# EAST-J/Dynhor

Hardware: AMD Instinct MI355X
Metric: training rays/sec (higher is better)
Workload: dtype f32; 1 GPU; custom_shoes-shaped synthetic seq, 512x512, 2048 rays x (64+64) samples per rank, NeuS SDF(8x256, skip 4, softplus100) + colour(4x256) MLP, full training iteration; family=neus, frames=64, rays_per_rank=2048, samples_per_ray=128, parallelism=dp1, loss=rgb L1 + 0.1 eikonal + 0.1 mask BCE + 0.05 mono-normal

## Files before the change

dynhor_amd/_lib.py:

```python
import ctypes
import os

import torch

_HERE = os.path.dirname(os.path.abspath(__file__))
LIB_PATH = os.path.join(_HERE, "libdynhor_hip.so")
_LIB = None

_vp, _i64, _i32, _f32 = ctypes.c_void_p, ctypes.c_int64, ctypes.c_int, ctypes.c_float

SIGNATURES = {
    "dh_version": (_i32, []),
    "dh_strerror": (ctypes.c_char_p, [_i32]),
    "dh_set_arithmetic": (_i32, [_i32]),
    "dh_get_arithmetic": (_i32, []),
    "dh_hash_set_scatter_mode": (_i32, [_i32]),
    "dh_num_params": (_i64, []),
    "dh_packed_floats": (_i64, []),
    "dh_param_layout": (_i32, [_i32, _i32, ctypes.POINTER(_i64), ctypes.POINTER(_i64), ctypes.POINTER(_i64),
                               ctypes.POINTER(_i32), ctypes.POINTER(_i32)]),
    "dh_packed_section": (_i32, [_i32, ctypes.POINTER(_i64), ctypes.POINTER(_i64)]),
    "dh_pack_weights": (_i32, [_vp, _vp, _vp]),
    "dh_pack_weights_ex": (_i32, [_i32, _vp, _vp, _vp]),
    "dh_sdf_nograd": (_i32, [_vp, _vp, _i64, _vp, _vp]),
    "dh_workspace_floats": (_i32, [_i64, ctypes.POINTER(_i64), ctypes.POINTER(_i64), ctypes.POINTER(_i64)]),
    "dh_range_words": (_i32, [ctypes.POINTER(_i64), ctypes.POINTER(_i64), ctypes.POINTER(_f32)]),
    "dh_mlp_forward": (_i32, [_vp, _vp, _vp, _i32, _i64, _vp, _vp, _vp, _vp, _vp]),
    "dh_sdf_forward": (_i32, [_vp, _vp, _i64, _vp, _vp, _vp]),
    "dh_sdf_gradient": (_i32, [_vp, _vp, _i64, _vp, _vp, _i32, _vp]),
    "dh_color_forward": (_i32, [_vp, _vp, _vp, _i32, _vp, _i64, _vp, _vp, _i32, _vp]),
    "dh_color_backward": (_i32, [_vp, _vp, _vp, _i64, _vp, _vp, _vp]),
    "dh_sdf_tangent": (_i32, [_vp, _vp, _vp, _i64, _vp, _vp]),
    "dh_sdf_backward": (_i32, [_vp, _vp, _i64, _vp, _vp]),
    "dh_color_backward_rays": (_i32, [_vp, _vp, _vp, _vp, _i32, _i64, _vp, _vp, _vp, _vp, _vp]),
    "dh_sdf_backward_rays": (_i32, [_vp, _vp, _vp, _vp, _i64, _vp, _vp, _vp]),
    "dh_weight_grads_gemm": (_i32, [_i64, _vp, _vp]),
    "dh_weight_grads_fold": (_i32, [_vp, _vp, _i64, _vp, _vp, _vp]),
    "dh_mlp_backward": (_i32, [_vp, _vp, _vp, _i64] + [_vp] * 7),
    "dh_sdf_nograd_ex": (_i32, [_i32, _vp, _vp, _i64, _vp, _vp]),
    "dh_mlp_forward_ex": (_i32, [_i32, _vp, _vp, _vp, _i32, _i64, _vp, _vp, _vp, _vp, _vp]),
    "dh_sdf_forward_ex": (_i32, [_i32, _vp, _vp, _i64, _vp, _vp, _vp]),
    "dh_sdf_gradient_ex": (_i32, [_i32, _vp, _vp, _i64, _vp, _vp, _i32, _vp]),
    "dh_color_forward_ex": (_i32, [_i32, _vp, _vp, _vp, _i32, _vp, _i64, _vp, _vp, _i32, _vp]),
    "dh_color_backward_ex": (_i32, [_i32, _vp, _vp, _vp, _i64, _vp, _vp, _vp]),
    "dh_sdf_tangent_ex": (_i32, [_i32, _vp, _vp, _vp, _i64, _vp, _vp]),
    "dh_sdf_backward_ex": (_i32, [_i32, _vp, _vp, _i64, _vp, _vp]),
    "dh_color_backward_rays_ex": (_i32, [_i32, _vp, _vp, _vp, _vp, _i32, _i64, _vp, _vp, _vp, _vp, _vp]),
    "dh_sdf_backward_rays_ex": (_i32, [_i32, _vp, _vp, _vp, _vp, _i64, _vp, _vp, _vp]),
    "dh_weight_grads_gemm_ex": (_i32, [_i32, _i64, _vp, _vp]),
    "dh_mlp_backward_ex": (_i32, [_i32, _vp, _vp, _vp, _i64] + [_vp] * 7),
    "dh_adam_step": (_i32, [_vp, _vp, _vp, _vp, _i64, _f32, _f32, _f32, _f32, _i64, _f32, _vp]),
    "dh_hashgrid_entries": (_i64, []),
    "dh_hashgrid_level": (_i32, [_i32, ctypes.POINTER(_f32), ctypes.POINTER(ctypes.c_uint32), ctypes.POINTER(ctypes.c_uint32),
                                 ctypes.POINTER(ctypes.c_uint32)]),
    "dh_hashgrid_encode": (_i32, [_vp, _vp, _i64, _vp, _vp]),
    "dh_hashgrid_encode_backward": (_i32, [_vp, _vp, _i64, _vp, _vp]),
    "dh_hash_num_params": (_i64, []),
    "dh_hash_packed_floats": (_i64, []),
    "dh_hash_param_layout": (_i32, [_i32, _i32, ctypes.POINTER(_i64), ctypes.POINTER(_i64), ctypes.POINTER(_i64),
                                    ctypes.POINTER(_i32), ctypes.POINTER(_i32)]),
    "dh_hash_pack_weights": (_i32, [_vp, _vp, _vp]),
    "dh_hash_workspace_floats": (_i32, [_i64, ctypes.POINTER(_i64), ctypes.POINTER(_i64)]),
    "dh_hash_sdf_nograd": (_i32, [_vp, _vp, _vp, _i64, _f32, _vp, _vp]),
    "dh_hash_geo_forward": (_i32, [_vp, _vp, _vp, _i64, _f32, _f32, _vp, _i32, _vp, _vp, _vp, _vp, _vp]),
    "dh_hash_color_forward": (_i32, [_vp, _vp, _vp, _vp, _i32, _i64, _vp, _vp, _vp]),
    "dh_hash_color_backward": (_i32, [_vp, _vp, _vp, _vp, _vp, _i32, _i64, _vp, _vp, _vp, _vp, _vp]),
    "dh_hash_geo_backward": (_i32, [_vp, _vp, _vp, _vp, _vp, _vp, _i64, _f32, _f32, _vp, _vp, _vp]),
    "dh_hash_weight_grads": (_i32, [_vp, _vp, _i64, _vp, _vp, _vp, _vp]),
    "dh_hash_weight_grads_parts": (_i32, [_vp, _vp, _i64, _vp, _vp, _vp, _i32, _vp]),
    "dh_gen_rays": (_i32, [_vp] * 6 + [_i32, _i32, _i32, _i32, _vp, _vp, _i64, _vp, _vp, _vp, _vp]),
    "dh_coarse_samples": (_i32, [_vp] * 5 + [_i64, _i32, _vp, _vp, _vp]),
    "dh_upsample_step": (_i32, [_vp] * 4 + [_i64, _i32, _i32, _f32, _vp, _vp, _vp]),
    "dh_merge_samples": (_i32, [_vp] * 4 + [_i64, _i32, _i32, _vp, _vp, _vp]),
    "dh_midpoints": (_i32, [_vp] * 3 + [_i64, _i32, _f32, _vp, _vp]),
    "dh_render_scan_fwd": (_i32, [_vp] * 7 + [_f32, _f32, _vp, _i64, _i32] + [_vp] * 9),
    "dh_render_scan_bwd": (_i32, [_vp] * 7 + [_f32, _f32, _vp, _i64, _i32] + [_vp] * 11),
    "dh_render_scan_bwd_rays": (_i32, [_vp] * 7 + [_f32, _f32, _vp, _i64, _i32] + [_vp] * 12),
    "dh_march_count": (_i32, [_vp] * 6 + [_i32, _f32, _f32, _f32, _i32, _i64, _vp, _vp]),
# ... 85 lines not shown


def roctx():
    global _ROCTX
    if _ROCTX is False:
        _ROCTX = None
        for name in ("librocprofiler-sdk-roctx.so", "libroctx64.so"):
            try:
                L = ctypes.CDLL(name)
                L.roctxRangePushA.argtypes = [ctypes.c_char_p]
                L.roctxRangePushA.restype = ctypes.c_int
                L.roctxRangePop.restype = ctypes.c_int
                _ROCTX = L
                break
            except (OSError, AttributeError):
                continue
    return _ROCTX


def check(status: int):
    if status != 0:
        raise DynhorHipError(f"dynhor_hip status {status}: {lib().dh_strerror(status).decode()}")


def ptr(t: torch.Tensor):
    assert t.is_cuda and t.is_contiguous(), "device-resident contiguous tensor required"
    return ctypes.c_void_p(t.data_ptr())


def stream():
    return ctypes.c_void_p(torch.cuda.current_stream().cuda_stream)


def param_layout(net: int, layer: int):
    b, g, v = _i64(), _i64(), _i64()
    o, i = _i32(), _i32()
    check(lib().dh_param_layout(net, layer, ctypes.byref(b), ctypes.byref(g), ctypes.byref(v),
                                ctypes.byref(o), ctypes.byref(i)))
    return b.value, g.value, v.value, o.value, i.value


def packed_section(section: int):
    o, n = _i64(), _i64()
    check(lib().dh_packed_section(int(section), ctypes.byref(o), ctypes.byref(n)))
    return o.value, n.value


def range_words():
    a, t, lim = _i64(), _i64(), _f32()
    check(lib().dh_range_words(ctypes.byref(a), ctypes.byref(t), ctypes.byref(lim)))
    return a.value, t.value, lim.value


def workspace_floats(npts: int):
    i, f, t = _i64(), _i64(), _i64()
    check(lib().dh_workspace_floats(npts, ctypes.byref(i), ctypes.byref(f), ctypes.byref(t)))
    return i.value, f.value, t.value
```

dynhor_amd/csrc/api.hip:

```cpp
#include "../../include/dynhor_hip.h"
#include "kernels.h"
#include "hash_layout.h"
#include "layout.h"
#include "workspace.h"

using namespace dh;

namespace dh {
static int g_arith = DH_ARITH_SPLIT_F16;
static int g_hash_scatter = 0;
int hash_scatter_mode() { return __atomic_load_n(&g_hash_scatter, __ATOMIC_RELAXED); }
}

namespace {
inline bool misaligned16(const void* p) { return (reinterpret_cast<uintptr_t>(p) & 15u) != 0; }
inline bool bad_arith(int a) { return a != DH_ARITH_SPLIT_BF16 && a != DH_ARITH_FP32_MFMA && a != DH_ARITH_SPLIT_F16; }
inline bool bad_arith_form(int a) {
    const int form = a & ~0xff;
    return bad_arith(a & 0xff) || (form != 0 && form != DH_CHAIN_FORM_TILE && form != DH_CHAIN_FORM_PAIR) ||
           (form != 0 && (a & 0xff) != DH_ARITH_SPLIT_F16);
}
inline int cur_arith() { return __atomic_load_n(&dh::g_arith, __ATOMIC_RELAXED); }
#ifndef DH_GRID_DIV
#define DH_GRID_DIV 1
// ... 37 lines not shown
        case 0: *offset_floats = PACKT.stream; *n_floats = PACKT_STREAM_FLOATS; break;
        case 1: *offset_floats = PACKT.bias10; *n_floats = 10 * 256; break;
        case 2: *offset_floats = PACKH.stream; *n_floats = PACKTH_STREAM_FLOATS; break;
        case 3: *offset_floats = PACKH.bias11; *n_floats = 11 * 256; break;
        case 4: *offset_floats = PACKH.wabs; *n_floats = 16; break;
        default: return DH_ERR_BAD_ARG;
    }
    return DH_OK;
}

int dh_param_layout(int net, int layer, int64_t* bias_off, int64_t* g_off, int64_t* v_off, int* out_dim, int* in_dim) {
    if (!bias_off || !g_off || !v_off || !out_dim || !in_dim) return DH_ERR_BAD_ARG;
    if (net == 0) {
        if (layer < 0 || layer >= N_SDF) return DH_ERR_BAD_ARG;
        const LinOff o = sdf_off(layer);
        *bias_off = o.bias; *g_off = o.g; *v_off = o.v; *out_dim = SDF_DIMS[layer].out; *in_dim = SDF_DIMS[layer].in;
    } else if (net == 1) {
        *bias_off = *g_off = *v_off = VARIANCE_OFF; *out_dim = 1; *in_dim = 1;
    } else if (net == 2) {
        if (layer < 0 || layer >= N_COL) return DH_ERR_BAD_ARG;
        const LinOff o = col_off(layer);
        *bias_off = o.bias; *g_off = o.g; *v_off = o.v; *out_dim = COL_DIMS[layer].out; *in_dim = COL_DIMS[layer].in;
    } else {
        return DH_ERR_BAD_ARG;
    }
    return DH_OK;
}

int dh_pack_weights(const float* params, float* packed, void* stream) {
    if (!params || !packed || misaligned16(packed)) return DH_ERR_BAD_ARG;
    return launch_pack_weights(params, packed, 7, static_cast<hipStream_t>(stream));
}
int dh_pack_weights_ex(int arithmetic, const float* params, float* packed, void* stream) {
    if (!params || !packed || misaligned16(packed) || bad_arith(arithmetic)) return DH_ERR_BAD_ARG;
    return launch_pack_weights(params, packed, 1 << arithmetic, static_cast<hipStream_t>(stream));
}

int dh_sdf_nograd_ex(int arithmetic, const float* packed, const float* pts, int64_t npts, float* sdf, void* stream) {
    if (npts < 0 || bad_arith(arithmetic)) return DH_ERR_BAD_ARG;
    if (npts == 0) return DH_OK;
    if (!packed || !pts || !sdf || misaligned16(packed)) return DH_ERR_BAD_ARG;
    return launch_sdf_nograd(packed, pts, npts, sdf, DEFAULT_GRID, arithmetic, static_cast<hipStream_t>(stream));
}

int dh_workspace_floats(int64_t npts, int64_t* infer_floats, int64_t* fwd_floats, int64_t* total_floats) {
    if (npts < 0 || !infer_floats || !fwd_floats || !total_floats) return DH_ERR_BAD_ARG;
    const Workspace w = carve_workspace(nullptr, npts);
    *infer_floats = w.infer_floats;
    *fwd_floats = w.fwd_floats;
    *total_floats = w.total_floats;
    return DH_OK;
}

int dh_range_words(int64_t* act_max_off, int64_t* tag_off, float* limit) {
    if (!act_max_off || !tag_off || !limit) return DH_ERR_BAD_ARG;
    *act_max_off = (int64_t)ABSMAX_ACT * ABSMAX_STRIDE;
    *tag_off = (int64_t)ABSMAX_TAG * ABSMAX_STRIDE;
    *limit = H2_RANGE / H2_XS;
    return DH_OK;
}

int dh_sdf_forward_ex(int arithmetic, const float* packed, const float* pts, int64_t npts, float* ws, float* sdf, void* stream) {
    if (bad_arith(arithmetic)) return DH_ERR_BAD_ARG;
    if (npts <= 0) return npts == 0 ? DH_OK : DH_ERR_BAD_ARG;
    if (!packed || !pts || !ws || !sdf || misaligned16(packed) || misaligned16(ws)) return DH_ERR_BAD_ARG;
    const Workspace w = carve_workspace(ws, npts);
    return launch_sdf_fwd_train(packed, pts, npts, sdf, w.feat, w.act, w.eaux, w.absmax, DEFAULT_GRID, arithmetic, static_cast<hipStream_t>(stream));
}

int dh_sdf_gradient_ex(int arithmetic, const float* packed, const float* pts, int64_t npts, float* ws, float* normals, int save,
                       void* stream) {
    if (bad_arith_form(arithmetic)) return DH_ERR_BAD_ARG;
    if (npts <= 0) return npts == 0 ? DH_OK : DH_ERR_BAD_ARG;
    if (!packed || !pts || !ws || !normals || misaligned16(packed) || misaligned16(ws)) return DH_ERR_BAD_ARG;
    const Workspace w = carve_workspace(ws, npts);
    if (save < 0 || save > 2) return DH_ERR_BAD_ARG;
    return launch_sdf_grad(packed, pts, npts, w.act, w.asave, normals, save, w.gesave, w.absmax, DEFAULT_GRID, arithmetic,
                           static_cast<hipStream_t>(stream));
}

int dh_color_forward_ex(int arithmetic, const float* packed, const float* pts, const float* dirs, int n_per_ray, const float* normals,
                        int64_t npts, float* ws, float* color, int save, void* stream) {
    if (npts < 0 || n_per_ray <= 0 || bad_arith_form(arithmetic)) return DH_ERR_BAD_ARG;
    if (npts == 0) return DH_OK;
    if (!packed || !pts || !dirs || !normals || !ws || !color || misaligned16(packed) || misaligned16(ws)) return DH_ERR_BAD_ARG;
    const Workspace w = carve_workspace(ws, npts);
    return launch_color_fwd(packed, pts, dirs, n_per_ray, normals, w.feat, npts, color, w.cact, w.caux, save, w.absmax, DEFAULT_GRID,
                            arithmetic, static_cast<hipStream_t>(stream));
}

int dh_mlp_forward_ex(int arithmetic, const float* packed, const float* pts, const float* dirs, int n_per_ray, int64_t npts, float* ws,
                      float* sdf, float* normals, float* color, void* stream) {
    int rc = dh_sdf_forward_ex(arithmetic, packed, pts, npts, ws, sdf, stream);
    if (rc) return rc;
    rc = dh_sdf_gradient_ex(arithmetic, packed, pts, npts, ws, normals, 1, stream);
    if (rc) return rc;
    return dh_color_forward_ex(arithmetic, packed, pts, dirs, n_per_ray, normals, npts, ws, color, 1, stream);
}

int dh_color_backward_ex(int arithmetic, const float* packed, const float* colors, const float* d_colors, int64_t npts, float* ws,
                         float* d_normals, void* stream) {
    if (npts <= 0 || bad_arith_form(arithmetic)) return DH_ERR_BAD_ARG;
    if (!packed || !colors || !d_colors || !ws || !d_normals || misaligned16(packed) || misaligned16(ws)) return DH_ERR_BAD_ARG;
    const Workspace w = carve_workspace(ws, npts);
    return launch_color_bwd(packed, colors, d_colors, npts, w.cact, w.czbar, w.featbar, d_normals, w.tpart, w.absmax, DEFAULT_GRID,
                            arithmetic, static_cast<hipStream_t>(stream));
}

int dh_sdf_tangent_ex(int arithmetic, const float* packed, const float* pts, const float* d_normals, int64_t npts, float* ws,
                      void* stream) {
    if (npts <= 0 || bad_arith(arithmetic)) return DH_ERR_BAD_ARG;
    if (!packed || !pts || !d_normals || !ws || misaligned16(packed) || misaligned16(ws)) return DH_ERR_BAD_ARG;
    const Workspace w = carve_workspace(ws, npts);
    return launch_sdf_tangent(packed, pts, d_normals, npts, w.act, w.asave, w.t0aux, w.tsave, w.rsave, w.tpart, w.absmax, DEFAULT_GRID,
                              arithmetic, static_cast<hipStream_t>(stream));
}

int dh_sdf_backward_ex(int arithmetic, const float* packed, const float* d_sdf, int64_t npts, float* ws, void* stream) {
    if (npts <= 0 || bad_arith(arithmetic)) return DH_ERR_BAD_ARG;
    if (!packed || !d_sdf || !ws || misaligned16(packed) || misaligned16(ws)) return DH_ERR_BAD_ARG;
    const Workspace w = carve_workspace(ws, npts);
    return launch_sdf_bwd(packed, d_sdf, npts, w.act, w.rsave, w.featbar, w.zbar, w.tpart, w.absmax, DEFAULT_GRID, arithmetic,
                          static_cast<hipStream_t>(stream));
}

int dh_color_backward_rays_ex(int arithmetic, const float* packed, const float* colors, const float* d_colors, const float* dirs,
                              int n_per_ray, int64_t npts, float* ws, float* d_normals, float* d_pts, float* d_dirs_pts, void* stream) {
    if (npts <= 0 || n_per_ray <= 0 || bad_arith(arithmetic)) return DH_ERR_BAD_ARG;
    if (!packed || !colors || !d_colors || !dirs || !ws || !d_normals || !d_pts || !d_dirs_pts || misaligned16(packed) || misaligned16(ws))
        return DH_ERR_BAD_ARG;
    const Workspace w = carve_workspace(ws, npts);
    return launch_color_bwd_rays(packed, colors, d_colors, dirs, n_per_ray, npts, w.cact, w.czbar, w.featbar, d_normals, w.tpart,
                                 d_pts, d_dirs_pts, w.absmax, DEFAULT_GRID, arithmetic, static_cast<hipStream_t>(stream));
}

int dh_sdf_backward_rays_ex(int arithmetic, const float* packed, const float* d_sdf, const float* pts, const float* d_normals,
                            int64_t npts, float* ws, float* d_pts, void* stream) {
    if (npts <= 0 || bad_arith(arithmetic)) return DH_ERR_BAD_ARG;
    if (!packed || !d_sdf || !pts || !d_normals || !ws || !d_pts || misaligned16(packed) || misaligned16(ws)) return DH_ERR_BAD_ARG;
    const Workspace w = carve_workspace(ws, npts);
    return launch_sdf_bwd_rays(packed, d_sdf, pts, d_normals, npts, w.act, w.rsave, w.featbar, w.gesave, w.zbar, w.tpart, d_pts,
                               w.absmax, DEFAULT_GRID, arithmetic, static_cast<hipStream_t>(stream));
}

int dh_weight_grads_gemm_ex(int arithmetic, int64_t npts, float* ws, void* stream) {
    if (npts <= 0 || bad_arith(arithmetic)) return DH_ERR_BAD_ARG;
    if (!ws || misaligned16(ws)) return DH_ERR_BAD_ARG;
    const Workspace w = carve_workspace(ws, npts);
    return launch_weight_grads_gemm(w, w.slabs, DW_G, arithmetic, static_cast<hipStream_t>(stream));
}

int dh_weight_grads_fold(const float* packed, const float* params, int64_t npts, float* ws, float* grad_flat, void* stream) {
    if (npts <= 0) return DH_ERR_BAD_ARG;
    if (!packed || !params || !ws || !grad_flat || misaligned16(packed) || misaligned16(ws)) return DH_ERR_BAD_ARG;
    const Workspace w = carve_workspace(ws, npts);
    return launch_weight_grads_fold(w, w.slabs, w.tred, DW_G, DW_NS, params, packed, grad_flat, static_cast<hipStream_t>(stream));
}

int dh_mlp_backward_ex(int arithmetic, const float* packed, const float* params, const float* pts, int64_t npts, float* ws,
                       const float* colors, const float* d_sdf, float* d_normals, const float* d_colors, float* grad_flat,
                       void* stream) {
    int rc = dh_color_backward_ex(arithmetic, packed, colors, d_colors, npts, ws, d_normals, stream);
    if (rc) return rc;
    rc = dh_sdf_tangent_ex(arithmetic, packed, pts, d_normals, npts, ws, stream);
    if (rc) return rc;
    rc = dh_sdf_backward_ex(arithmetic, packed, d_sdf, npts, ws, stream);
    if (rc) return rc;
    rc = dh_weight_grads_gemm_ex(arithmetic, npts, ws, stream);
    if (rc) return rc;
    return dh_weight_grads_fold(packed, params, npts, ws, grad_flat, stream);
}

int dh_sdf_nograd(const float* packed, const float* pts, int64_t npts, float* sdf, void* stream) {
    return dh_sdf_nograd_ex(cur_arith(), packed, pts, npts, sdf, stream);
}
int dh_sdf_forward(const float* packed, const float* pts, int64_t npts, float* ws, float* sdf, void* stream) {
    return dh_sdf_forward_ex(cur_arith(), packed, pts, npts, ws, sdf, stream);
}
int dh_sdf_gradient(const float* packed, const float* pts, int64_t npts, float* ws, float* normals, int save, void* stream) {
    return dh_sdf_gradient_ex(cur_arith(), packed, pts, npts, ws, normals, save, stream);
}
int dh_color_forward(const float* packed, const float* pts, const float* dirs, int n_per_ray, const float* normals,
                     int64_t npts, float* ws, float* color, int save, void* stream) {
    return dh_color_forward_ex(cur_arith(), packed, pts, dirs, n_per_ray, normals, npts, ws, color, save, stream);
}
// ... 529 lines not shown
```

dynhor_amd/csrc/chain_pair.hip:

```cpp
#include "tile.h"
#include "kernels.h"
#include "mlp_common.h"
#include "tile16h.h"
#include "pair16h.h"
#include "workspace.h"

namespace dh {

struct HScratchP { float sred[4]; float sred2[4]; float lmax[12]; };
struct ColHPtrs;
struct ColPPtrs {
    const u32x4* main0;
    const u32x4* aux;
    const float* bias0;
    const float* w4;
    const float* b4;
    const unsigned* wabs;
};
constexpr int64_t COL_MAIN_STRIDE = (PACKH.col_fwd_main[1] - PACKH.col_fwd_main[0]) / 4;
constexpr int64_t COL_BIAS_STRIDE = PACK.col_bias[1] - PACK.col_bias[0];
static_assert(PACKH.col_fwd_main[2] - PACKH.col_fwd_main[1] == PACKH.col_fwd_main[1] - PACKH.col_fwd_main[0] &&
              PACKH.col_fwd_main[3] - PACKH.col_fwd_main[2] == PACKH.col_fwd_main[1] - PACKH.col_fwd_main[0] &&
              (PACKH.col_fwd_main[1] - PACKH.col_fwd_main[0]) % 4 == 0, "colour forward weights: one stride");
static_assert(PACK.col_bias[2] - PACK.col_bias[1] == COL_BIAS_STRIDE && PACK.col_bias[3] - PACK.col_bias[2] == COL_BIAS_STRIDE, "colour biases: one stride");
static inline ColPPtrs make_colp_ptrs(const float* packed) {
    ColPPtrs C;
    C.main0 = reinterpret_cast<const u32x4*>(packed + PACKH.col_fwd_main[0]);
    C.aux = reinterpret_cast<const u32x4*>(packed + PACKH.col_fwd_aux0);
    C.bias0 = packed + PACK.col_bias[0];
    C.w4 = packed + PACK.col_w4;
    C.b4 = packed + PACK.col_b4;
    C.wabs = reinterpret_cast<const unsigned*>(packed + PACKH.wabs) + N_SDF;
    return C;
}

template <bool SAVE>
struct ColFwdEpi : PEpi<ColFwdEpi<SAVE>, 3, 4> {
    f32x16 (&acc)[MT][2];
    HScratchP& hs;
    float* lmax;
    const int wave, lane, tid;
    const float inv, b0, b1;
    const rsrc_t st;
    const int loff;
    __device__ __forceinline__ ColFwdEpi(f32x16 (&acc_)[MT][2], _Float16* img_, HScratchP& hs_, float* lmax_, int wave_, int lane_, int tid_,
                                         float inv_, float b0_, float b1_, rsrc_t st_, int loff_, bool)
        : acc(acc_), hs(hs_), lmax(lmax_), wave(wave_), lane(lane_), tid(tid_), inv(inv_), b0(b0_), b1(b1_), st(st_), loff(loff_) {
        this->handoff_init(img_, wave_, lane_);
    }
    template <int G, int SUB>
    __device__ __forceinline__ void elem() {
        constexpr int m = G / 8, t = (G / 4) % 2, r4 = G % 4;
        const float b = t ? b1 : b0;
        if constexpr (SUB == 0 || SUB == 1) {
            constexpr int r = 4 * r4 + 2 * SUB;
            acc[m][t][r] = fmaxf(fmaf(acc[m][t][r], inv, b), 0.f);
            acc[m][t][r + 1] = fmaxf(fmaf(acc[m][t][r + 1], inv, b), 0.f);
        } else {
            if constexpr (SAVE) {
                f32x4 v;
                v[0] = acc[m][t][4 * r4 + 0]; v[1] = acc[m][t][4 * r4 + 1]; v[2] = acc[m][t][4 * r4 + 2]; v[3] = acc[m][t][4 * r4 + 3];
                tile_st(st, loff, G, v);
            }
            this->m0 = fmaxf(this->m0, fmaxf(fabsf(acc[m][t][4 * r4 + 0]), fabsf(acc[m][t][4 * r4 + 1])));
            this->m1 = fmaxf(this->m1, fmaxf(fabsf(acc[m][t][4 * r4 + 2]), fabsf(acc[m][t][4 * r4 + 3])));
        }
    }
    __device__ __forceinline__ void publish(float wm) { tile_max_publish(hs.sred, wave, lane, wm); }
    __device__ __forceinline__ float read_tile_max() { return tile_max_read(hs.sred); }
    __device__ __forceinline__ void on_tile_max(float m) { if (tid == 0 && lmax) *lmax = fmaxf(*lmax, m); }
};

__device__ __forceinline__ void row_dot256x3_hp(const _Float16* img, const float* sw4, int tid, float (&out)[3]) {
    constexpr int TPP_ = 256 / TM, SEG = 256 / TPP_;
    const int p = tid / TPP_, part = tid % TPP_;
    const f16x8* xh = reinterpret_cast<const f16x8*>(img + p * LDH + part * SEG);
    const f16x8* xl = reinterpret_cast<const f16x8*>(img + PLANE_H + p * LDH + part * SEG);
    float s[3] = {0.f, 0.f, 0.f};
    DH_UNROLL for (int i = 0; i < SEG / 8; ++i) {
        const f16x8 h = xh[i], l = xl[i];
        float x[8];
        DH_UNROLL for (int k = 0; k < 8; ++k) x[k] = (float)h[k] + (float)l[k];
        DH_UNROLL for (int j = 0; j < 3; ++j) {
            const f32x4* wr = reinterpret_cast<const f32x4*>(sw4 + j * 256 + part * SEG);
            const f32x4 b0 = wr[2 * i], b1 = wr[2 * i + 1];
            DH_UNROLL for (int k = 0; k < 4; ++k) s[j] = fmaf(x[k], b0[k], s[j]);
            DH_UNROLL for (int k = 0; k < 4; ++k) s[j] = fmaf(x[4 + k], b1[k], s[j]);
        }
    }
    DH_UNROLL for (int j = 0; j < 3; ++j) {
        DH_UNROLL for (int off = 1; off < TPP_; off <<= 1) s[j] += __shfl_xor(s[j], off);
        out[j] = s[j];
    }
}

__device__ __forceinline__ TileScale pair_handoff_exposed(const f32x16 (&acc)[MT][2], _Float16* img, HScratchP& hs, float* lmax, int tid,
                                                          int wave, int lane, const float* extra_lds) {
    tile_max_publish(hs.sred, wave, lane, acc_absmax(acc));
    __syncthreads();
    const float m = tile_max_read(hs.sred);
    if (tid == 0 && lmax) *lmax = fmaxf(*lmax, m);
    const TileScale ts = scale_for_max(fmaxf(m, *extra_lds));
    acc_to_lds_split(acc, img, wave, lane, ts.S);
    __syncthreads();
    return ts;
}

template <bool SAVE>
__global__ __launch_bounds__(256, 1) void color_fwd_p_kernel(ColPPtrs C, const float* __restrict__ pts, const float* __restrict__ dirs,
                                                            int n_per_ray, const float* __restrict__ normals,
                                                            const float* __restrict__ feat, int64_t npts, float* __restrict__ color,
                                                            float* __restrict__ cact, float* __restrict__ caux,
                                                            unsigned* __restrict__ absmax) {
    __shared__ __attribute__((aligned(16))) _Float16 simg[2][IMG_H];
    __shared__ __attribute__((aligned(16))) float saux[2][TM * LDA];
    __shared__ HScratchP hs;
    __shared__ float sfb[64];
    const int tid = threadIdx.x, wave = tid >> 6, lane = tid & 63;
    const int loff = tile_loff(wave, lane);
    const int64_t ntiles = (npts + TM - 1) / TM, npairs = (ntiles + 1) / 2;
    if (tid < 12) hs.lmax[tid] = 0.f;
    float winv0 = winv_from_bits(C.wabs[0]), winv1 = winv_from_bits(C.wabs[1]), winv2 = winv_from_bits(C.wabs[2]), winv3 = winv_from_bits(C.wabs[3]);
    float bs[4][2];
    DH_UNROLL for (int l = 0; l < 4; ++l)
        DH_UNROLL for (int t = 0; t < 2; ++t) bs[l][t] = C.bias0[l * COL_BIAS_STRIDE + acc_col(wave, t, lane)];
    PW<P_NKC> W;
    _Float16* imgA = simg[0];
    _Float16* imgB = simg[1];
    int pit = 0;
    for (int64_t pr = blockIdx.x; pr < npairs; pr += gridDim.x, ++pit) {
        const bool son = pit == 2;
        (void)son;
        PSTAMP(son, 0);
        const int64_t tileA = 2 * pr;
        const bool okB = tileA + 1 < ntiles;
        const int64_t tileB = okB ? tileA + 1 : tileA;
        f32x16 accA[MT][2], accB[MT][2];
        acc_load_native_b(accA, tile_rsrc(feat + tileA * TILE_F), loff);
        acc_load_native_b(accB, tile_rsrc(feat + tileB * TILE_F), loff);
        {
            const int which = tid >> 7, half = (tid >> 6) & 1, p = tid & 63;
            const int64_t t0 = (which ? tileB : tileA) * TM;
            const int64_t gp = t0 + p;
            auto single_ray = [&](int64_t first) {
                const int64_t last = first + TM - 1 < npts ? first + TM - 1 : npts - 1;
                return first / n_per_ray == last / n_per_ray;
            };
            const bool oneA = single_ray(tileA * TM), oneB = single_ray(tileB * TM);
            const bool one_ray = which ? oneB : oneA;
            float* row = saux[which] + p * LDA;
            float* emb = sfb + which * 32;
            if (one_ray && half == 0 && lane < 12) {
                const int c = lane % 3, k = lane / 3;
                float sn, co; sincosf(dirs[(t0 / n_per_ray) * 3 + c] * (float)(1 << k), &sn, &co);
                emb[6 * k + c] = sn;
                emb[6 * k + 3 + c] = co;
            }
            float mx = 1.f;
            if (gp < npts) {
                const int64_t ray = gp / n_per_ray;
                DH_UNROLL for (int c = 0; c < 3; ++c) {
                    const float d = dirs[ray * 3 + c];
                    if (!one_ray) {
                        DH_UNROLL for (int kk = 0; kk < 2; ++kk) {
                            const int k = 2 * half + kk;
                            float sn, co; sincosf(d * (float)(1 << k), &sn, &co);
// ... 2 lines not shown
                        }
                    }
                    if (half == 0) {
                        const float x = pts[gp * 3 + c], nn = normals[gp * 3 + c];
                        row[c] = x;
                        row[3 + c] = d;
                        row[30 + c] = nn;
                        mx = fmaxf(mx, fmaxf(fabsf(x), fmaxf(fabsf(d), fabsf(nn))));
                    }
                }
            } else {
                DH_UNROLL for (int c = 0; c < 3; ++c) {
                    DH_UNROLL for (int kk = 0; kk < 2; ++kk) { row[6 + 6 * (2 * half + kk) + c] = 0.f; row[6 + 6 * (2 * half + kk) + 3 + c] = 0.f; }
                    if (half == 0) { row[c] = 0.f; row[3 + c] = 0.f; row[30 + c] = 0.f; }
                }
            }
            if (half == 0) {
                DH_UNROLL for (int c = CAUX; c < LDA; ++c) row[c] = 0.f;
                mx = wave_max(mx);
                if (lane == 0) hs.sred2[which] = mx;
            }
            if (oneA || oneB) {
                pair_barrier();
                if (one_ray && gp < npts) { DH_UNROLL for (int j = 0; j < 12; ++j) row[6 + 12 * half + j] = emb[12 * half + j]; }
            }
        }
        PSTAMP(son, 88);
        TileScale tsA = pair_handoff_exposed(accA, imgA, hs, SAVE ? &hs.lmax[4] : nullptr, tid, wave, lane, &hs.sred2[0]);
        PSTAMP(son, 89);
        TileScale tsB = pair_handoff_exposed(accB, imgB, hs, SAVE ? &hs.lmax[4] : nullptr, tid, wave, lane, &hs.sred2[1]);
        PSTAMP(son, 90);
        if (SAVE && tid == 0) hs.lmax[5] = fmaxf(hs.lmax[5], fmaxf(hs.sred2[0], hs.sred2[1]));
        if (SAVE) {
            aux_lds_to_native(saux[0], caux + tileA * AUXT_F, wave, lane);
            if (okB) aux_lds_to_native(saux[1], caux + tileB * AUXT_F, wave, lane);
        }
        PSTAMP(son, 91);
        pw_load_all(W, C.main0, wave, lane);
        PSTAMP(son, 1);
        _Pragma("unroll 1") for (int l = 0; l < 4; ++l) {
            const float wl = l == 0 ? winv0 : l == 1 ? winv1 : l == 2 ? winv2 : winv3;
            const float wp = l == 1 ? winv0 : l == 2 ? winv1 : winv2;
            const float c0 = l == 0 ? bs[0][0] : l == 1 ? bs[1][0] : l == 2 ? bs[2][0] : bs[3][0];
            const float c1 = l == 0 ? bs[0][1] : l == 1 ? bs[1][1] : l == 2 ? bs[2][1] : bs[3][1];
            const float p0 = l == 1 ? bs[0][0] : l == 2 ? bs[1][0] : bs[2][0];
            const float p1 = l == 1 ? bs[0][1] : l == 2 ? bs[1][1] : bs[2][1];
            acc_zero(accA);
            if (l == 0) {
                PNoEpi e;
                pair_phase<false>(accA, imgA, W, C.main0, C.main0, wave, lane, e);
                gemm_rows_aux_h(accA, saux[0], C.aux, wave, lane, tsA.S);
            } else {
                ColFwdEpi<SAVE> e(accB, imgB, hs, SAVE ? &hs.lmax[l - 1] : nullptr, wave, lane, tid, tsB.inv * wp, p0, p1,
                                  tile_rsrc_if(cact + ((int64_t)(l - 1) * ntiles + tileB) * TILE_F, okB), loff, okB);
                if (son && l == 2) e.stamp = 18;
                pair_phase<false>(accA, imgA, W, C.main0 + (int64_t)l * COL_MAIN_STRIDE, C.main0, wave, lane, e);
                tsB.S = e.S; tsB.inv = e.inv_S;
            }
            PSTAMP(son, 2 + 4 * l);
            pair_barrier();
            PSTAMP(son, 3 + 4 * l);
            acc_zero(accB);
            {
                ColFwdEpi<SAVE> e(accA, imgA, hs, SAVE ? &hs.lmax[l] : nullptr, wave, lane, tid, tsA.inv * wl, c0, c1,
                                  tile_rsrc(cact + ((int64_t)l * ntiles + tileA) * TILE_F), loff, true);
                if (son && l == 2) e.stamp = 52;
                pair_phase<true>(accB, imgB, W, C.main0 + (int64_t)l * COL_MAIN_STRIDE, C.main0 + (int64_t)(l < 3 ? l + 1 : 3) * COL_MAIN_STRIDE, wave, lane, e, l < 3);
                if (l == 0) gemm_rows_aux_h(accB, saux[1], C.aux, wave, lane, tsB.S);
                tsA.S = e.S; tsA.inv = e.inv_S;
            }
            PSTAMP(son, 4 + 4 * l);
            pair_barrier();
            PSTAMP(son, 5 + 4 * l);
        }
        const float w4a = C.w4[tid], w4b = C.w4[256 + tid], w4c = C.w4[512 + tid];
        {
            ColFwdEpi<SAVE> e(accB, imgB, hs, SAVE ? &hs.lmax[3] : nullptr, wave, lane, tid, tsB.inv * winv3, bs[3][0], bs[3][1],
                              tile_rsrc_if(cact + ((int64_t)3 * ntiles + tileB) * TILE_F, okB), loff, okB);
            pair_epi_alone_from<0>(e);
            tsB.S = e.S; tsB.inv = e.inv_S;
        }
        float* sw4 = saux[0];
        sw4[tid] = w4a; sw4[256 + tid] = w4b; sw4[512 + tid] = w4c;
        pair_barrier();
        PSTAMP(son, 86);
        DH_UNROLL for (int which = 0; which < 2; ++which) {
            const int64_t gp = (which ? tileB : tileA) * TM + tid / TPP;
            const float sinv = which ? tsB.inv : tsA.inv;
            float dots[3];
            row_dot256x3_hp(which ? imgB : imgA, sw4, tid, dots);
            DH_UNROLL for (int j = 0; j < 3; ++j) {
                const float raw = fmaf(dots[j], sinv, C.b4[j]);
                if (tid % TPP == 0 && gp < npts && (which == 0 || okB)) color[gp * 3 + j] = 1.f / (1.f + __expf(-raw));
            }
        }
        pair_barrier();
        PSTAMP(son, 87);
    }
    if (SAVE && absmax) {
        if (tid < 4) post_class_max(absmax, ABSMAX_CACT + tid, hs.lmax[tid]);
        if (tid == 4) post_class_max(absmax, ABSMAX_FEAT, hs.lmax[4]);
        if (tid == 5) post_class_max(absmax, ABSMAX_CAUX, hs.lmax[5]);
    }
}

struct SdfGradPPtrs {
    const u32x4 *rev1, *rev2, *rev3, *rev4, *rev5, *rev6, *rev7;
    const u32x4 *revaux0, *revaux4;
    const float* w8row0;
    const unsigned* wabs;
};
static inline SdfGradPPtrs make_sdfgradp_ptrs(const float* packed) {
    SdfGradPPtrs P;
    auto rv = [&](int l) { return reinterpret_cast<const u32x4*>(packed + PACKH.sdf_rev_main[l]); };
    P.rev1 = rv(1); P.rev2 = rv(2); P.rev3 = rv(3); P.rev4 = rv(4); P.rev5 = rv(5); P.rev6 = rv(6); P.rev7 = rv(7);
    P.revaux0 = reinterpret_cast<const u32x4*>(packed + PACKH.sdf_rev_aux[0]);
    P.revaux4 = reinterpret_cast<const u32x4*>(packed + PACKH.sdf_rev_aux[4]);
    P.w8row0 = packed + PACK.sdf_w8row0;
    P.wabs = reinterpret_cast<const unsigned*>(packed + PACKH.wabs);
    return P;
}
template <bool SAVE>
struct SdfGradEpi : PEpi<SdfGradEpi<SAVE>, 5, 3> {
    static constexpr int RING = 5;
    f32x16 (&acc)[MT][2];
    HScratchP& hs;
    float* lmax;
    const int wave, lane, tid;
    const float inv;
    const rsrc_t hr, st;
    const int loff;
// ... 151 lines not shown
                        float* q = &saux[which][aux_row(wave, r, lane) * LDA + col];
                        *q = fmaf(g0[tt][r], inv, *q);
                    }
                }
            }
        }
        __syncthreads();
        if (tid < 2 * TM) {
            const int which = tid >> 6, p = tid & 63;
            const int64_t gp = (which ? tileB : tileA) * TM + p;
            if (gp < npts && (which == 0 || okB)) {
                const float* g = saux[which] + p * LDA;
                float n[3];
                DH_UNROLL for (int c = 0; c < 3; ++c) {
                    const float x = pts[gp * 3 + c];
                    float v = g[c];
                    DH_UNROLL for (int k = 0; k < 6; ++k) {
                        const float f = (float)(1 << k);
                        float sn, co; sincosf(x * f, &sn, &co);
                        v += f * (co * g[3 + 6 * k + c] - sn * g[3 + 6 * k + 3 + c]);
                    }
                    n[c] = v;
                }
                normals[gp * 3 + 0] = n[0]; normals[gp * 3 + 1] = n[1]; normals[gp * 3 + 2] = n[2];
                if (save == 2) { for (int c = 0; c < 40; ++c) gesave[gp * 40 + c] = c < EMB ? g[c] : 0.f; }
            }
        }
        __syncthreads();
        PSTAMP(son, 31);
    }
    if (SAVE && absmax && tid < 8) post_class_max(absmax, ABSMAX_ASAVE + tid, hs.lmax[tid]);
    if (absmax) {
        const float m = wave_max(watch_close(hmax));
        if (lane == 0) post_class_max(absmax, ABSMAX_ACT, m);
    }
}

enum : int { PTP_COL_B0 = 12, PTP_COL_W4 = 16, PTP_COL_B4 = 19 };
struct ColBwdPPtrs {
    const u32x4 *rev0, *rev1, *rev2, *rev3;
    const u32x4* revaux;
    const float* w4;
    const unsigned* wabs;
};
static inline ColBwdPPtrs make_colbwdp_ptrs(const float* packed) {
    ColBwdPPtrs C;
    auto rv = [&](int l) { return reinterpret_cast<const u32x4*>(packed + PACKH.col_rev_main[l]); };
    C.rev0 = rv(0); C.rev1 = rv(1); C.rev2 = rv(2); C.rev3 = rv(3);
    C.revaux = reinterpret_cast<const u32x4*>(packed + PACKH.col_rev_aux0);
    C.w4 = packed + PACK.col_w4;
    C.wabs = reinterpret_cast<const unsigned*>(packed + PACKH.wabs) + N_SDF;
    return C;
}
template <bool LAST>
struct ColBwdEpi : PEpi<ColBwdEpi<LAST>, 4, 3, !LAST> {
    static constexpr int RING = 5;
    f32x16 (&acc)[MT][2];
    HScratchP& hs;
    float* lmax;
    unsigned* tslot;
    float* csum;
    const int wave, lane, tid;
    const float inv;
    const rsrc_t hr, st;
    const int loff;
    const bool store;
    float cs0 = 0.f, cs1 = 0.f;
    f32x4 hq[RING];
    __device__ __forceinline__ ColBwdEpi(f32x16 (&acc_)[MT][2], _Float16* img_, HScratchP& hs_, float* lmax_, unsigned* tslot_, float* csum_,
                                         int wave_, int lane_, int tid_, float inv_, rsrc_t hr_, rsrc_t st_, int loff_, bool store_)
        : acc(acc_), hs(hs_), lmax(lmax_), tslot(tslot_), csum(csum_), wave(wave_), lane(lane_), tid(tid_), inv(inv_), hr(hr_),
          st(st_), loff(loff_), store(store_) {
        if constexpr (!LAST) {
            this->handoff_init(img_, wave_, lane_);
            DH_UNROLL for (int g = 0; g < RING; ++g) hq[g] = tile_ld(hr, loff, g);
        }
    }
    template <int G, int SUB>
    __device__ __forceinline__ void elem() {
        constexpr int m = G / 8, t = (G / 4) % 2, r4 = G % 4;
        if constexpr (SUB == 0 || SUB == 1) {
            constexpr int i = 2 * SUB, r = 4 * r4 + i;
            if constexpr (LAST) {
                acc[m][t][r] *= inv;
                acc[m][t][r + 1] *= inv;
            } else {
                const f32x4& h = hq[G % RING];
                acc[m][t][r] = h[i] > 0.f ? acc[m][t][r] * inv : 0.f;
                acc[m][t][r + 1] = h[i + 1] > 0.f ? acc[m][t][r + 1] * inv : 0.f;
            }
        } else if constexpr (SUB == 2) {
            f32x4 v;
            v[0] = acc[m][t][4 * r4 + 0]; v[1] = acc[m][t][4 * r4 + 1]; v[2] = acc[m][t][4 * r4 + 2]; v[3] = acc[m][t][4 * r4 + 3];
            tile_st(st, loff, G, v);
            if constexpr (!LAST && G + RING < 16) hq[G % RING] = tile_ld(hr, loff, G + RING);
            if constexpr (!LAST) {
                float& cs = t ? cs1 : cs0;
                cs += acc[m][t][4 * r4 + 0]; cs += acc[m][t][4 * r4 + 1]; cs += acc[m][t][4 * r4 + 2]; cs += acc[m][t][4 * r4 + 3];
            }
        } else {
            this->m0 = fmaxf(this->m0, fmaxf(fabsf(acc[m][t][4 * r4 + 0]), fabsf(acc[m][t][4 * r4 + 1])));
            this->m1 = fmaxf(this->m1, fmaxf(fabsf(acc[m][t][4 * r4 + 2]), fabsf(acc[m][t][4 * r4 + 3])));
        }
    }
    __device__ __forceinline__ void publish(float wm) {
        if constexpr (LAST) {
            tile_max_publish(hs.sred2, wave, lane, wm);
        } else {
            cs0 += __shfl_xor(cs0, 32); cs1 += __shfl_xor(cs1, 32);
            if (lane < 32 && store) { csum[64 * wave + lane] = cs0; csum[64 * wave + 32 + lane] = cs1; }
            tile_max_publish(hs.sred, wave, lane, wm);
        }
    }
    __device__ __forceinline__ float read_tile_max() { return tile_max_read(hs.sred); }
    __device__ __forceinline__ void on_tile_max(float m) {
        if (tid == 0) {
            *lmax = fmaxf(*lmax, m);
            if (store) *tslot = __builtin_bit_cast(unsigned, m);
        }
    }
};

#ifndef COLBWD_NREG
#define COLBWD_NREG 8
#endif
__global__ __launch_bounds__(256, 1) void color_bwd_p_kernel(ColBwdPPtrs C, const float* __restrict__ colors, const float* __restrict__ d_colors,
                                                            int64_t npts, const float* __restrict__ cact, float* __restrict__ czbar,
                                                            float* __restrict__ featbar, float* __restrict__ d_normals,
                                                            float* __restrict__ tpart, unsigned* __restrict__ absmax,
                                                            unsigned* __restrict__ tmax) {
    __shared__ __attribute__((aligned(16))) _Float16 simg[2][IMG_H];
    __shared__ __attribute__((aligned(16))) float scraw[2][TM * 4];
    __shared__ HScratchP hs;
    __shared__ float sfb[2][4];
    const int tid = threadIdx.x, wave = tid >> 6, lane = tid & 63;
    const int loff = tile_loff(wave, lane);
    const int64_t ntiles = (npts + TM - 1) / TM, npairs = (ntiles + 1) / 2;
    if (tid < 12) hs.lmax[tid] = 0.f;
    const float wi0 = winv_from_bits(C.wabs[0]), wi1 = winv_from_bits(C.wabs[1]), wi2 = winv_from_bits(C.wabs[2]), wi3 = winv_from_bits(C.wabs[3]);
    auto winv = [&](int l) { return l == 0 ? wi0 : l == 1 ? wi1 : l == 2 ? wi2 : wi3; };
    auto rev = [&](int l) { return l == 0 ? C.rev0 : l == 1 ? C.rev1 : l == 2 ? C.rev2 : C.rev3; };
    PW<COLBWD_NREG> W;
    _Float16* imgA = simg[0];
    _Float16* imgB = simg[1];
    for (int64_t pr = blockIdx.x; pr < npairs; pr += gridDim.x) {
        const int64_t tileA = 2 * pr;
        const bool okB = tileA + 1 < ntiles;
        const int64_t tileB = okB ? tileA + 1 : tileA;
        float* tpA = tpart + tileA * N_TILE_PART * 256;
        float* tpB = tpart + tileB * N_TILE_PART * 256;
        if (tid < 2 * TM) {
            const int which = tid >> 6, p = tid & 63;
            const int64_t gp = (which ? tileB : tileA) * TM + p;
            DH_UNROLL for (int j = 0; j < 3; ++j) {
                float v = 0.f;
                if (gp < npts) { const float c = colors[gp * 3 + j]; v = d_colors[gp * 3 + j] * c * (1.f - c); }
                scraw[which][p * 4 + j] = v;
            }
            scraw[which][p * 4 + 3] = 0.f;
        }
        __syncthreads();
        if (tid < 3 || (tid >= 64 && tid < 67)) {
            const int which = tid >> 6, j = tid & 63;
            float sum = 0.f;
            for (int r = 0; r < TM; ++r) sum += scraw[which][r * 4 + j];
            if (which == 0 || okB) (which ? tpB : tpA)[PTP_COL_B4 * 256 + j] = sum;
        }
        f32x16 accA[MT][2], accB[MT][2];
        TileScale tsA, tsB;
        DH_UNROLL for (int which = 0; which < 2; ++which) {
            f32x16 (&acc)[MT][2] = which ? accB : accA;
            const int64_t tile = which ? tileB : tileA;
            float* tp = which ? tpB : tpA;
            const bool on = which == 0 || okB;
            acc_load_native_b(acc, tile_rsrc(cact + ((int64_t)3 * ntiles + tile) * TILE_F), loff);
            {
                const int col0 = acc_col(wave, 0, lane), col1 = acc_col(wave, 1, lane);
                float w4[3][2];
                DH_UNROLL for (int j = 0; j < 3; ++j) { w4[j][0] = C.w4[j * 256 + col0]; w4[j][1] = C.w4[j * 256 + col1]; }
                float dw[3][2] = {{0.f, 0.f}, {0.f, 0.f}, {0.f, 0.f}};
                DH_UNROLL for (int m = 0; m < MT; ++m)
                    DH_UNROLL for (int r = 0; r < 16; ++r) {
                        const f32x4 cr = *reinterpret_cast<const f32x4*>(scraw[which] + acc_row(m, r, lane) * 4);
                        DH_UNROLL for (int t = 0; t < 2; ++t) {
                            const float h = acc[m][t][r];
                            DH_UNROLL for (int j = 0; j < 3; ++j) dw[j][t] = fmaf(cr[j], h, dw[j][t]);
                            const float hb = cr[0] * w4[0][t] + cr[1] * w4[1][t] + cr[2] * w4[2][t];
                            acc[m][t][r] = h > 0.f ? hb : 0.f;
                        }
                    }
                DH_UNROLL for (int j = 0; j < 3; ++j)
                    DH_UNROLL for (int t = 0; t < 2; ++t) {
                        float sum = dw[j][t];
                        sum += __shfl_xor(sum, 32);
                        if (lane < 32 && on) tp[(PTP_COL_W4 + j) * 256 + 64 * wave + 32 * t + lane] = sum;
                    }
            }
            if (on) {
                acc_store_native_b(acc, tile_rsrc(czbar + ((int64_t)3 * ntiles + tile) * TILE_F), loff);
                tile_colsum(acc, tp + (PTP_COL_B0 + 3) * 256, wave, lane);
            }
            tile_max_publish(hs.sred, wave, lane, acc_absmax(acc));
            __syncthreads();
            const float mx = tile_max_read(hs.sred);
            if (tid == 0) {
                hs.lmax[3] = fmaxf(hs.lmax[3], mx);
                if (on) tmax[(TMAX_CZBAR + 3) * ntiles + tile] = __builtin_bit_cast(unsigned, mx);
            }
            const TileScale ts = scale_for_max(mx);
            acc_to_lds_split(acc, which ? imgB : imgA, wave, lane, ts.S);
            __syncthreads();
            if (which) tsB = ts; else tsA = ts;
        }
        pw_load_all(W, C.rev3, wave, lane);
        _Pragma("unroll 1") for (int l = 3; l >= 1; --l) {
            acc_zero(accA);
            if (l == 3) {
                PNoEpi e;
                pair_phase<false>(accA, imgA, W, C.rev3, C.rev3, wave, lane, e);
            } else {
                ColBwdEpi<false> e(accB, imgB, hs, &hs.lmax[l], tmax + (TMAX_CZBAR + l) * ntiles + tileB, tpB + (PTP_COL_B0 + l) * 256, wave, lane, tid,
                                   tsB.inv * winv(l + 1), tile_rsrc(cact + ((int64_t)l * ntiles + tileB) * TILE_F),
                                   tile_rsrc_if(czbar + ((int64_t)l * ntiles + tileB) * TILE_F, okB), loff, okB);
                pair_phase<false>(accA, imgA, W, rev(l), C.rev3, wave, lane, e);
                tsB.S = e.S; tsB.inv = e.inv_S;
            }
            pair_barrier();
            acc_zero(accB);
            {
                ColBwdEpi<false> e(accA, imgA, hs, &hs.lmax[l - 1], tmax + (TMAX_CZBAR + l - 1) * ntiles + tileA, tpA + (PTP_COL_B0 + l - 1) * 256, wave,
                                   lane, tid, tsA.inv * winv(l), tile_rsrc(cact + ((int64_t)(l - 1) * ntiles + tileA) * TILE_F),
                                   tile_rsrc(czbar + ((int64_t)(l - 1) * ntiles + tileA) * TILE_F), loff, true);
                pair_phase<true>(accB, imgB, W, rev(l), rev(l - 1), wave, lane, e);
                tsA.S = e.S; tsA.inv = e.inv_S;
            }
            pair_barrier();
        }
        acc_zero(accA);
        {
            ColBwdEpi<false> e(accB, imgB, hs, &hs.lmax[0], tmax + TMAX_CZBAR * ntiles + tileB, tpB + PTP_COL_B0 * 256, wave, lane, tid,
                               tsB.inv * wi1, tile_rsrc(cact + tileB * TILE_F), tile_rsrc_if(czbar + tileB * TILE_F, okB), loff, okB);
            pair_phase<false>(accA, imgA, W, C.rev0, C.rev0, wave, lane, e);
            tsB.S = e.S; tsB.inv = e.inv_S;
        }
        pair_barrier();
        acc_zero(accB);
        {
            ColBwdEpi<true> e(accA, imgA, hs, nullptr, nullptr, nullptr, wave, lane, tid, tsA.inv * wi0, tile_rsrc(featbar + tileA * TILE_F),
                              tile_rsrc(featbar + tileA * TILE_F), loff, true);
            pair_phase<false>(accB, imgB, W, C.rev0, C.rev0, wave, lane, e);
            if (lane == 0) sfb[0][wave] = hs.sred2[wave];
        }
        pair_barrier();
        {
            ColBwdEpi<true> e(accB, imgB, hs, nullptr, nullptr, nullptr, wave, lane, tid, tsB.inv * wi0, tile_rsrc(featbar + tileB * TILE_F),
                              tile_rsrc_if(featbar + tileB * TILE_F, okB), loff, okB);
            pair_epi_alone_from<0>(e);
            if (lane == 0) sfb[1][wave] = hs.sred2[wave];
        }
        DH_UNROLL for (int which = 0; which < 2; ++which) {
            f32x16 a2[AUX_NTW];
            aux_zero(a2);
            gemm_auxout_hp(a2, which ? imgB : imgA, 16, C.revaux, wave, lane);
            const float inv0 = (which ? tsB.inv : tsA.inv) * wi0;
            DH_UNROLL for (int tt = 0; tt < AUX_NTW; ++tt) {
                const int col = aux_col(wave, tt, lane);
                if (col >= 30 && col < 33 && (which == 0 || okB)) {
                    DH_UNROLL for (int r = 0; r < 16; ++r) {
                        const int64_t gp = (which ? tileB : tileA) * TM + aux_row(wave, r, lane);
                        if (gp < npts) d_normals[gp * 3 + (col - 30)] += a2[tt][r] * inv0;
                    }
                }
            }
        }
        __syncthreads();
        if (tid < 2) {
            const float m = fmaxf(fmaxf(sfb[tid][0], sfb[tid][1]), fmaxf(sfb[tid][2], sfb[tid][3]));
            if (tid == 0 || okB) {
                atomicMax(reinterpret_cast<unsigned*>(&hs.lmax[4]), __builtin_bit_cast(unsigned, m));
                tmax[TMAX_FEATBAR * ntiles + (tid ? tileB : tileA)] = __builtin_bit_cast(unsigned, m);
            }
        }
        __syncthreads();
    }
    if (absmax) {
        if (tid < 4) post_class_max(absmax, ABSMAX_CZBAR + tid, hs.lmax[tid]);
        if (tid == 4) post_class_max(absmax, ABSMAX_FEATBAR, hs.lmax[4]);
    }
}

}
#ifdef DH_STAMPS
extern "C" int dh_dev_read_stamps_p(unsigned long long* host, long long n) {
    const long long total = (long long)(sizeof(dh::dh_pstamps) / sizeof(unsigned long long));
    if (n > total) n = total;
    return hipMemcpyFromSymbol(host, HIP_SYMBOL(dh::dh_pstamps), (size_t)n * sizeof(unsigned long long)) == hipSuccess ? 0 : -3;
}
#endif
namespace dh {
static inline int okp() { return hipGetLastError() == hipSuccess ? 0 : -3; }
static int pair_cus() {
    static int cache[16] = {};
    int dev = 0;
    if (hipGetDevice(&dev) != hipSuccess || dev < 0 || dev >= 16) return 0;
    if (cache[dev] == 0) {
        int cus = 0, lds = 0;
        if (hipDeviceGetAttribute(&cus, hipDeviceAttributeMultiprocessorCount, dev) != hipSuccess) cus = 0;
        if (hipDeviceGetAttribute(&lds, hipDeviceAttributeMaxSharedMemoryPerMultiprocessor, dev) != hipSuccess) lds = 0;
        cache[dev] = (lds >= PAIR_LDS_BYTES && cus > 0) ? cus : -1;
    }
    return cache[dev] > 0 ? cache[dev] : 0;
}
bool pair_form_available() { return pair_cus() > 0; }
int pair_form_cus() { return pair_cus(); }
int launch_color_fwd_p(const float* packed, const float* pts, const float* dirs, int n_per_ray, const float* normals,
                       const float* feat, int64_t npts, float* color, float* cact, float* caux, int save, unsigned* absmax,
                       hipStream_t stream) {
    const int cus = pair_cus();
    if (cus <= 0) return -2;
    const int64_t ntiles = (npts + TM - 1) / TM, npairs = (ntiles + 1) / 2;
    const int g = (int)(npairs < cus ? npairs : cus);
    if (save) hipLaunchKernelGGL(color_fwd_p_kernel<true>, dim3(g), dim3(256), 0, stream, make_colp_ptrs(packed), pts, dirs, n_per_ray, normals,
                                 feat, npts, color, cact, caux, absmax);
    else hipLaunchKernelGGL(color_fwd_p_kernel<false>, dim3(g), dim3(256), 0, stream, make_colp_ptrs(packed), pts, dirs, n_per_ray, normals,
                            feat, npts, color, cact, caux, absmax);
    return okp();
}

}

namespace dh {
int launch_sdf_grad_p(const float* packed, const float* pts, int64_t npts, const float* act, float* asave, float* normals, int save,
                      float* gesave, unsigned* absmax, hipStream_t stream) {
    const int cus = pair_cus();
    if (cus <= 0) return -2;
    const int64_t ntiles = (npts + TM - 1) / TM, npairs = (ntiles + 1) / 2;
    const int g = (int)(npairs < cus ? npairs : cus);
    if (save) hipLaunchKernelGGL(sdf_grad_p_kernel<true>, dim3(g), dim3(256), 0, stream, make_sdfgradp_ptrs(packed), pts, npts, act, asave,
                                 normals, save, gesave, absmax);
    else hipLaunchKernelGGL(sdf_grad_p_kernel<false>, dim3(g), dim3(256), 0, stream, make_sdfgradp_ptrs(packed), pts, npts, act, asave,
                            normals, save, gesave, absmax);
    return okp();
}
}

namespace dh {
int launch_color_bwd_p(const float* packed, const float* colors, const float* d_colors, int64_t npts, const float* cact, float* czbar,
                       float* featbar, float* d_normals, float* tpart, unsigned* absmax, unsigned* tmax, hipStream_t stream) {
    const int cus = pair_cus();
    if (cus <= 0) return -2;
    const int64_t ntiles = (npts + TM - 1) / TM, npairs = (ntiles + 1) / 2;
    const int g = (int)(npairs < cus ? npairs : cus);
    hipLaunchKernelGGL(color_bwd_p_kernel, dim3(g), dim3(256), 0, stream, make_colbwdp_ptrs(packed), colors, d_colors, npts, cact, czbar,
                       featbar, d_normals, tpart, absmax, tmax);
    return okp();
}
}
```

dynhor_amd/csrc/kernels.h:

```cpp
#pragma once
#include <hip/hip_runtime.h>
#include <stdint.h>
#include "layout.h"

namespace dh {

enum : int { ARITH_BF16 = 0, ARITH_FP32 = 1, ARITH_F16 = 2 };
int hash_scatter_mode();

int launch_pack_weights(const float* params, float* packed, int arith_mask, hipStream_t stream);

inline int ok() { return hipGetLastError() == hipSuccess ? 0 : -3; }
inline int grid_for(int64_t npts, int grid) {
    const int64_t ntiles = (npts + TM - 1) / TM;
    return (int)(ntiles < grid ? ntiles : grid);
}

int launch_sdf_nograd(const float* packed, const float* pts, int64_t npts, float* sdf, int grid, int arith, hipStream_t stream);
int launch_sdf_nograd_t(const float* packed, const float* pts, int64_t npts, float* sdf, bool h2, hipStream_t stream);
int launch_sdf_fwd_train_t(const float* packed, const float* pts, int64_t npts, float* sdf, float* feat, float* act, float* eaux,
                           unsigned* absmax, bool h2, hipStream_t stream);

int launch_sdf_fwd_train(const float* packed, const float* pts, int64_t npts, float* sdf, float* feat, float* act,
                         float* eaux, float* absmax, int grid, int arith, hipStream_t stream);
int launch_sdf_grad(const float* packed, const float* pts, int64_t npts, const float* act, float* asave, float* normals,
                    int save, float* gesave, float* absmax, int grid, int arith, hipStream_t stream);
int launch_color_fwd(const float* packed, const float* pts, const float* dirs, int n_per_ray, const float* normals,
                     const float* feat, int64_t npts, float* color, float* cact, float* caux, int save, float* absmax, int grid,
                     int arith, hipStream_t stream);
int launch_sdf_grad_h(const float* packed, const float* pts, int64_t npts, const float* act, float* asave, float* normals,
                      int save, float* gesave, unsigned* absmax, int grid, hipStream_t stream);
int launch_color_fwd_h(const float* packed, const float* pts, const float* dirs, int n_per_ray, const float* normals,
                       const float* feat, int64_t npts, float* color, float* cact, float* caux, int save, unsigned* absmax,
                       int grid, hipStream_t stream);
int launch_color_bwd_h(const float* packed, const float* colors, const float* d_colors, const float* dirs, int n_per_ray,
                       int64_t npts, const float* cact, float* czbar, float* featbar, float* d_normals, float* tpart,
                       float* d_pts, float* d_dirs_pts, unsigned* absmax, unsigned* tmax, int grid, hipStream_t st);
int launch_sdf_tangent_h(const float* packed, const float* pts, const float* d_normals, int64_t npts, const float* act,
                         const float* asave, float* t0aux, float* tsave, float* rsave, float* tpart, unsigned* absmax, unsigned* tmax,
                         int grid, hipStream_t st);
int launch_sdf_bwd_h(const float* packed, const float* d_sdf, const float* pts, const float* d_normals, int64_t npts,
                     const float* act, const float* rsave, const float* featbar, const float* gesave, float* zbar, float* tpart,
                     float* d_pts, unsigned* absmax, unsigned* tmax, int grid, hipStream_t st);

enum : int { CHAIN_FORM_AUTO = 0, CHAIN_FORM_TILE = 1, CHAIN_FORM_PAIR = 2 };
bool pair_form_available();
int pair_form_cus();
inline bool use_pair_form(int form, int64_t npts, bool auto_pair) {
    if (form == CHAIN_FORM_PAIR) return true;
    if (form == CHAIN_FORM_TILE || !auto_pair) return false;
    const int cus = pair_form_cus();
    return cus > 0 && (npts + TM - 1) / TM >= 2 * (int64_t)cus;
}
int launch_color_fwd_p(const float* packed, const float* pts, const float* dirs, int n_per_ray, const float* normals,
                       const float* feat, int64_t npts, float* color, float* cact, float* caux, int save, unsigned* absmax,
                       hipStream_t stream);

int launch_sdf_grad_p(const float* packed, const float* pts, int64_t npts, const float* act, float* asave, float* normals, int save,
                      float* gesave, unsigned* absmax, hipStream_t stream);

int launch_color_bwd_p(const float* packed, const float* colors, const float* d_colors, int64_t npts, const float* cact, float* czbar,
                       float* featbar, float* d_normals, float* tpart, unsigned* absmax, unsigned* tmax, hipStream_t stream);

int launch_gen_rays(const uint8_t* rgb, const int8_t* label, const uint8_t* normal, const float* R, const float* T,
                    const float* Kinv, int H, int W, int frame, const int64_t* px, const int64_t* py, int64_t B,
                    float* rays, float* near, float* far, hipStream_t st);
int launch_coarse_samples(const float* o, const float* d, const float* near, const float* far, const float* t_rand,
                          int64_t B, int n, float* z, float* pts, hipStream_t st);
int launch_upsample(const float* o, const float* d, const float* z, const float* sdf, int64_t B, int n, int n_new,
                    float inv_s, float* z_new, float* pts_new, hipStream_t st);
int launch_merge(const float* z, const float* z_new, const float* sdf, const float* sdf_new, int64_t B, int n, int n_new,
                 float* z_out, float* sdf_out, hipStream_t st);
int launch_midpoints(const float* o, const float* d, const float* z, int64_t B, int n, float sample_dist, float* pts,
                     hipStream_t st);
int launch_render_fwd(const float* o, const float* d, const float* z, const float* sdf, const float* normals,
                      const float* colors, const float* inv_s, float car, float sample_dist, const float* bg, int64_t B,
                      int n, float* weights, float* color, float* wsum, float* wmax, float* cdf, float* inside, float* eik,
                      float* nmap, const int64_t* seg_off, const int32_t* seg_cnt, hipStream_t st);
int launch_render_bwd(const float* o, const float* d, const float* z, const float* sdf, const float* normals,
                      const float* colors, const float* inv_s, float car, float sample_dist, const float* bg, int64_t B,
                      int n, const float* d_color, const float* d_wsum, const float* d_weights, const float* d_gradients,
                      const float* d_nmap, const float* eik_coef, float* d_sdf, float* d_normals, float* d_colors,
                      float* d_inv_s, float* d_rays_d, const int64_t* seg_off, const int32_t* seg_cnt, hipStream_t st);
int launch_march_count(const float* o, const float* d, const float* near, const float* far, const float* u, const uint8_t* occ,
                       int res, float radius, float step, float half_step, int max_samples, int64_t B, int32_t* cnt,
                       hipStream_t st);
int launch_march_emit(const float* o, const float* d, const float* near, const float* far, const float* u, const uint8_t* occ,
                      int res, float radius, float step, float half_step, int max_samples, int64_t B, const int64_t* off,
                      const int32_t* keep, float* t_start, float* pts, float* dirs_pts, int32_t* ray_idx, hipStream_t st);
int launch_loss(const float* color, const float* wsum, const float* nmap, const float* eik, const float* rays,
                const float* R, int64_t B, float igr_w, float mask_w, float normal_w, float* stats, float* d_color,
                float* d_wsum, float* d_nmap, float* eik_coef, hipStream_t st);

int launch_corr_loss(const float* rays_o, const float* rays_d, const float* z, const float* weights, const float* corr,
                     const float* R_all, const float* T_all, int n_frames, const float* K, int64_t B, int n, float sample_dist,
                     float delta_px, float corr_w, float* stats, float* residual_px, float* d_weights, float* pose_adj,
                     hipStream_t st);

int launch_color_bwd(const float* packed, const float* colors, const float* d_colors, int64_t npts, const float* cact,
                     float* czbar, float* featbar, float* d_normals, float* tpart, float* absmax, int grid, int arith, hipStream_t st);
int launch_color_bwd_rays(const float* packed, const float* colors, const float* d_colors, const float* dirs, int n_per_ray,
                          int64_t npts, const float* cact, float* czbar, float* featbar, float* d_normals, float* tpart,
                          float* d_pts, float* d_dirs_pts, float* absmax, int grid, int arith, hipStream_t st);
int launch_sdf_bwd_rays(const float* packed, const float* d_sdf, const float* pts, const float* d_normals, int64_t npts,
                        const float* act, const float* rsave, const float* featbar, const float* gesave, float* zbar,
                        float* tpart, float* d_pts, float* absmax, int grid, int arith, hipStream_t st);
int launch_sdf_tangent(const float* packed, const float* pts, const float* d_normals, int64_t npts, const float* act,
                       const float* asave, float* t0aux, float* tsave, float* rsave, float* tpart, float* absmax, int grid, int arith,
                       hipStream_t st);
int launch_sdf_bwd(const float* packed, const float* d_sdf, int64_t npts, const float* act, const float* rsave,
                   const float* featbar, float* zbar, float* tpart, float* absmax, int grid, int arith, hipStream_t st);
struct Workspace;
int launch_weight_grads_gemm(const Workspace& w, float* slabs, int G, int arith, hipStream_t st);
int launch_weight_grads_fold(const Workspace& w, float* slabs, float* tred, int G, int nS, const float* params,
                             const float* packed, float* grad, hipStream_t st);

int launch_adam(float* p, const float* g, float* m, float* v, int64_t n, float lr, float b1, float b2, float eps,
                int64_t step, float grad_scale, hipStream_t st);

int64_t hashgrid_entries();
int hashgrid_level(int l, float* scale, uint32_t* res, uint32_t* offset, uint32_t* dense);
int launch_hashgrid_fwd(const float* table, const float* x01, int64_t n, float* out, hipStream_t st);
int launch_hashgrid_bwd(const float* x01, const float* d_out, int64_t n, float* d_table, hipStream_t st);

int64_t hash_num_params();
int64_t hash_workspace_floats(int64_t n);
int launch_hash_pack(const float* params, float* hp, hipStream_t st);
int launch_hash_sdf_nograd(const float* params, const float* hp, const float* pts, int64_t n, float radius, float* sdf,
                           hipStream_t st);
int64_t hash_infer_workspace_floats(int64_t n);
int launch_hash_geo_fwd(const float* params, const float* hp, const float* pts, int64_t n, float radius, float eps,
                        float* ws, int save, float* sdf, float* feat, float* grad, const int64_t* n_act, hipStream_t st);
int launch_sh_color_fwd(const float* hp, const float* feat, const float* normals, const float* dirs, int n_per_ray,
                        int64_t n, float* color, const int64_t* n_act, hipStream_t st);
int launch_sh_color_bwd(const float* hp, const float* feat, const float* normals, const float* dirs, const float* d_color,
                        int n_per_ray, int64_t n, float* ws, float* d_feat, float* d_normals, const int64_t* n_act, hipStream_t st);
int launch_hash_geo_bwd(const float* params, const float* hp, const float* pts, const float* d_sdf, const float* d_feat,
                        const float* d_grad, int64_t n, float radius, float eps, float* ws, const int64_t* n_act, hipStream_t st);
int launch_hash_weight_grads(const float* params, const float* hp, int64_t n, float* ws, float* grad, const int64_t* n_act,
                             int parts, hipStream_t st);

int64_t nearest_sqdist_workspace(int64_t nq, int64_t nr);
int launch_nearest_sqdist(const float* q, int64_t nq, const float* ref, int64_t nr, float* d2, int32_t* idx, void* ws, hipStream_t st);

int64_t icp_correspond_workspace(int64_t n, int64_t m, int64_t h);
int launch_icp_correspond(const float* src, int64_t n, const float* tgt, int64_t m, const float* xf, int64_t h, float* d2, int32_t* idx,
                          void* ws, hipStream_t st);
int icp_moments_sums(int plane);
int64_t icp_moments_workspace(int64_t n, int64_t h, int plane);
int launch_icp_moments(const float* src, const float* tgt, const float* nrm, const float* xf, const int32_t* idx, const float* d2,
                       const float* thr, const float* osrc, const float* otgt, int64_t n, int64_t m, int64_t h, double* out, void* ws,
                       hipStream_t st);

int launch_label_dilate(const int8_t* label, int64_t n_frames, int H, int W, int radius, uint8_t* tmp, uint8_t* keep, hipStream_t st);
int launch_mesh_mask_votes(const float* verts, int64_t nv, const uint8_t* keep, const float* R, const float* T, const float* K,
// ... 31 lines not shown
```

dynhor_amd/csrc/kernels_mlp.hip:

```cpp
#include "tile.h"
#include "kernels.h"
#include "mlp_common.h"
#include "tile16.h"
#include "workspace.h"


namespace dh {

__global__ __launch_bounds__(256, 2) void sdf_nograd_kernel(SdfPtrs P, const float* __restrict__ pts, int64_t npts,
                                                             float* __restrict__ sdf_out) {
    __shared__ __attribute__((aligned(16))) float smain[TM * LDX];
    __shared__ __attribute__((aligned(16))) float saux[TM * LDA];
    const int tid = threadIdx.x, wave = tid >> 6, lane = tid & 63;
    const int64_t ntiles = (npts + TM - 1) / TM;
    for (int64_t tile = blockIdx.x; tile < ntiles; tile += gridDim.x) {
        embed_tile(pts, tile * TM, npts, saux, tid);
        __syncthreads();
        f32x16 acc[MT][2];
        BFrag pre = gemm_b_prefetch(P.fwd_main[1], wave, lane);
        for (int l = 0; l < 8; ++l) {
            acc_zero(acc);
            if (l > 0) gemm_rows(acc, smain, LDX, l == 4 ? 28 : 32, P.fwd_main[l], wave, lane, pre);
            if (l == 0 || l == 4) gemm_rows(acc, saux, LDA, 5, P.fwd_aux[l], wave, lane);
            pre = gemm_b_prefetch(P.fwd_main[l + 1], wave, lane);
// ... 64 lines not shown
            acc_map(acc, [&](int, int t, int, float h) { float s, em; softplus_deriv_from_h(h, s, em); return (t ? w1 : w0) * s; });
            if (save) acc_store_native(acc, asave + ((int64_t)7 * ntiles + tile) * TILE_F, wave, lane);
            acc_to_lds(acc, smain, wave, lane);
            __syncthreads();
        }
        typename Core::Pre pre = Core::prefetch(P.rev_main[7], wave, lane);
        for (int l = 7; l >= 1; --l) {
            acc_zero(acc);
            Core::rows(acc, smain, LDX, Core::K_MAIN, P.rev_main[l], wave, lane, pre);
            if (l > 1) pre = Core::prefetch(P.rev_main[l - 1], wave, lane);
            if (l == 4) Core::auxout(ge, smain, P.rev_aux[4], wave, lane);
            const f32x4* hp = reinterpret_cast<const f32x4*>(act + ((int64_t)(l - 1) * ntiles + tile) * TILE_F) + (size_t)wave * MT * 8 * 64 + lane;
            DH_UNROLL for (int m = 0; m < MT; ++m) {
                DH_UNROLL for (int t = 0; t < 2; ++t)
                    DH_UNROLL for (int r4 = 0; r4 < 4; ++r4) {
                        const f32x4 h = DH_TILE_LD(hp + ((m * 2 + t) * 4 + r4) * 64);
                        DH_UNROLL for (int rr = 0; rr < 4; ++rr) {
                            float s, em; softplus_deriv_from_h(h[rr], s, em);
                            acc[m][t][4 * r4 + rr] *= s;
                        }
                    }
                __builtin_amdgcn_sched_barrier(0);
            }
            if (save) acc_store_native(acc, asave + ((int64_t)(l - 1) * ntiles + tile) * TILE_F, wave, lane);
            __syncthreads();
            acc_to_lds(acc, smain, wave, lane);
            __syncthreads();
        }
        Core::auxout(ge, smain, P.rev_aux[0], wave, lane);
        aux_acc_to_lds(ge, saux, AUXW, wave, lane);
        __syncthreads();
        if (tid < TM) {
            const int64_t gp = tile * TM + tid;
            if (gp < npts) point_normal(saux + tid * LDA, pts, gp, normals, save, gesave);
        }
        __syncthreads();
    }
}
__global__ __launch_bounds__(256, 2) void sdf_grad_kernel(SdfPtrs P, const float* __restrict__ pts, int64_t npts,
                                                           const float* __restrict__ act, float* __restrict__ asave,
                                                           float* __restrict__ normals, int save, float* __restrict__ gesave) {
    sdf_grad_body<CoreF32>(P, pts, npts, act, asave, normals, save, gesave);
}
__global__ __launch_bounds__(256, 2) void sdf_grad_s_kernel(Sdf16Ptrs P, const float* __restrict__ pts, int64_t npts,
                                                           const float* __restrict__ act, float* __restrict__ asave,
                                                           float* __restrict__ normals, int save, float* __restrict__ gesave) {
    sdf_grad_body<CoreBf16>(P, pts, npts, act, asave, normals, save, gesave);
}


template <class Core>
__device__ __forceinline__ void color_fwd_body(const typename Core::Col& C, const float* pts, const float* dirs, int n_per_ray,
                                               const float* normals, const float* feat, int64_t npts, float* color, float* cact,
                                               float* caux, int save) {
    __shared__ __attribute__((aligned(16))) float smain[TM * LDX];
    __shared__ __attribute__((aligned(16))) float saux[TM * LDA];
    const int tid = threadIdx.x, wave = tid >> 6, lane = tid & 63;
    const int64_t ntiles = (npts + TM - 1) / TM;
    for (int64_t tile = blockIdx.x; tile < ntiles; tile += gridDim.x) {
        if (tid < TM) {
            const int64_t gp = tile * TM + tid;
            float* row = saux + tid * LDA;
            if (gp < npts) {
                const int64_t ray = gp / n_per_ray;
                DH_UNROLL for (int c = 0; c < 3; ++c) {
                    const float d = dirs[ray * 3 + c];
                    row[c] = pts[gp * 3 + c];
                    row[3 + c] = d;
                    DH_UNROLL for (int k = 0; k < 4; ++k) {
                        float s, co; sincosf(d * (float)(1 << k), &s, &co);
                        row[6 + 6 * k + c] = s;
                        row[6 + 6 * k + 3 + c] = co;
                    }
                    row[30 + c] = normals[gp * 3 + c];
                }
            } else {
                DH_UNROLL for (int c = 0; c < CAUX; ++c) row[c] = 0.f;
            }
            DH_UNROLL for (int c = CAUX; c < LDA; ++c) row[c] = 0.f;
        }
        f32x16 acc[MT][2];
        acc_load_native(acc, feat + tile * TILE_F, wave, lane);
        acc_to_lds(acc, smain, wave, lane);
        __syncthreads();
        if (save) aux_lds_to_native(saux, caux + tile * AUXT_F, wave, lane);
        typename Core::Pre pre = Core::prefetch(C.fwd_main[0], wave, lane);
        for (int l = 0; l < 4; ++l) {
            acc_zero(acc);
            Core::rows(acc, smain, LDX, Core::K_MAIN, C.fwd_main[l], wave, lane, pre);
            if (l == 0) Core::rows(acc, saux, LDA, Core::K_AUX, C.fwd_aux0, wave, lane);
            if (l < 3) pre = Core::prefetch(C.fwd_main[l + 1], wave, lane);
            const float b0 = C.bias[l][acc_col(wave, 0, lane)], b1 = C.bias[l][acc_col(wave, 1, lane)];
            acc_map(acc, [&](int, int t, int, float v) { return fmaxf(v + (t ? b1 : b0), 0.f); });
            if (save) acc_store_native(acc, cact + ((int64_t)l * ntiles + tile) * TILE_F, wave, lane);
            __syncthreads();
            acc_to_lds(acc, smain, wave, lane);
            __syncthreads();
        }
        const int64_t gp = tile * TM + tid / TPP;
        DH_UNROLL for (int j = 0; j < 3; ++j) {
            const float raw = row_dot256(smain, C.w4 + j * 256, tid) + C.b4[j];
            if (tid % TPP == 0 && gp < npts) color[gp * 3 + j] = 1.f / (1.f + __expf(-raw));
        }
        __syncthreads();
    }
}
__global__ __launch_bounds__(256, 2) void color_fwd_kernel(ColPtrs C, const float* __restrict__ pts, const float* __restrict__ dirs,
                                                            int n_per_ray, const float* __restrict__ normals,
                                                            const float* __restrict__ feat, int64_t npts,
                                                            float* __restrict__ color, float* __restrict__ cact,
                                                            float* __restrict__ caux, int save) {
    color_fwd_body<CoreF32>(C, pts, dirs, n_per_ray, normals, feat, npts, color, cact, caux, save);
}
__global__ __launch_bounds__(256, 2) void color_fwd_s_kernel(Col16Ptrs C, const float* __restrict__ pts, const float* __restrict__ dirs,
                                                            int n_per_ray, const float* __restrict__ normals,
                                                            const float* __restrict__ feat, int64_t npts,
                                                            float* __restrict__ color, float* __restrict__ cact,
                                                            float* __restrict__ caux, int save) {
    color_fwd_body<CoreBf16>(C, pts, dirs, n_per_ray, normals, feat, npts, color, cact, caux, save);
}

int launch_sdf_fwd_train(const float* packed, const float* pts, int64_t npts, float* sdf, float* feat, float* act,
                         float* eaux, float* absmax, int grid, int arith, hipStream_t stream) {
    if (absmax) (void)hipMemsetAsync(absmax, 0, ABSMAX_FLOATS * sizeof(float), stream);
    if (arith != ARITH_FP32) return launch_sdf_fwd_train_t(packed, pts, npts, sdf, feat, act, eaux, reinterpret_cast<unsigned*>(absmax),
                                                           arith == ARITH_F16, stream);
    hipLaunchKernelGGL(sdf_fwd_train_kernel, dim3(grid_for(npts, grid)), dim3(256), 0, stream, make_sdf_ptrs(packed), pts, npts, sdf, feat, act, eaux);
    return ok();
}
int launch_sdf_grad(const float* packed, const float* pts, int64_t npts, const float* act, float* asave, float* normals,
                    int save, float* gesave, float* absmax, int grid, int arith, hipStream_t stream) {
    const int form = arith >> 8;
    arith &= 0xff;
    if (arith == ARITH_F16) {
        if (use_pair_form(form, npts, false)) return launch_sdf_grad_p(packed, pts, npts, act, asave, normals, save, gesave, reinterpret_cast<unsigned*>(absmax), stream);
        return launch_sdf_grad_h(packed, pts, npts, act, asave, normals, save, gesave, reinterpret_cast<unsigned*>(absmax), grid, stream);
    }
    if (arith == ARITH_FP32) hipLaunchKernelGGL(sdf_grad_kernel, dim3(grid_for(npts, grid)), dim3(256), 0, stream, make_sdf_ptrs(packed), pts, npts, act, asave, normals, save, gesave);
    else hipLaunchKernelGGL(sdf_grad_s_kernel, dim3(grid_for(npts, grid)), dim3(256), 0, stream, make_sdf16_ptrs(packed), pts, npts, act, asave, normals, save, gesave);
    return ok();
}
int launch_color_fwd(const float* packed, const float* pts, const float* dirs, int n_per_ray, const float* normals,
                     const float* feat, int64_t npts, float* color, float* cact, float* caux, int save, float* absmax, int grid,
                     int arith, hipStream_t stream) {
    const int form = arith >> 8;
    arith &= 0xff;
    if (arith == ARITH_F16) {
        if (use_pair_form(form, npts, true)) return launch_color_fwd_p(packed, pts, dirs, n_per_ray, normals, feat, npts, color, cact, caux, save,
                                                                 reinterpret_cast<unsigned*>(absmax), stream);
        return launch_color_fwd_h(packed, pts, dirs, n_per_ray, normals, feat, npts, color, cact, caux, save,
                                  reinterpret_cast<unsigned*>(absmax), grid, stream);
    }
    const int g = grid_for(npts, grid);
    if (arith == ARITH_FP32) hipLaunchKernelGGL(color_fwd_kernel, dim3(g), dim3(256), 0, stream, make_col_ptrs(packed), pts, dirs, n_per_ray, normals,
                                                feat, npts, color, cact, caux, save);
    else hipLaunchKernelGGL(color_fwd_s_kernel, dim3(g), dim3(256), 0, stream, make_col16_ptrs(packed), pts, dirs, n_per_ray, normals,
                            feat, npts, color, cact, caux, save);
    return ok();
}

int launch_sdf_nograd(const float* packed, const float* pts, int64_t npts, float* sdf, int grid, int arith, hipStream_t stream) {
    if (npts <= 0) return 0;
    if (arith != ARITH_FP32) return launch_sdf_nograd_t(packed, pts, npts, sdf, arith == ARITH_F16, stream);
    hipLaunchKernelGGL(sdf_nograd_kernel, dim3(grid_for(npts, grid)), dim3(256), 0, stream, make_sdf_ptrs(packed), pts, npts, sdf);
    return ok();
}

}
```

dynhor_amd/csrc/kernels_mlp_bwd.hip:

```cpp
#include "tile.h"
#include "kernels.h"
#include "mlp_common.h"
#include "workspace.h"
#include "stamps.h"

DH_STAMP_READER(dh_dev_read_stamps_bwd)

namespace dh {

enum : int { TP_SDF_B0 = 0, TP_SDF_B8 = 8, TP_W8ROW0_T = 9, TP_W8ROW0_S = 10, TP_SCAL = 11, TP_COL_B0 = 12,
             TP_COL_W4 = 16, TP_COL_B4 = 19 };

template <class Core, bool RAYS>
__device__ __forceinline__ void color_bwd_body(const typename Core::Col& C, const float* colors, const float* d_colors, int64_t npts,
                                               const float* cact, float* czbar, float* featbar, float* d_normals, float* tpart,
                                               const float* dirs, int n_per_ray, float* d_pts, float* d_dirs_pts) {
    __shared__ __attribute__((aligned(16))) float smain[TM * LDX];
    __shared__ __attribute__((aligned(16))) float saux[TM * LDA];
    const int tid = threadIdx.x, wave = tid >> 6, lane = tid & 63;
    const int64_t ntiles = (npts + TM - 1) / TM;
    for (int64_t tile = blockIdx.x; tile < ntiles; tile += gridDim.x) {
        float* tp = tpart + tile * N_TILE_PART * 256;
        if (tid < TM) {
            const int64_t gp = tile * TM + tid;
            DH_UNROLL for (int j = 0; j < 3; ++j) {
                float v = 0.f;
                if (gp < npts) { const float c = colors[gp * 3 + j]; v = d_colors[gp * 3 + j] * c * (1.f - c); }
                saux[tid * 4 + j] = v;
            }
            saux[tid * 4 + 3] = 0.f;
        }
        __syncthreads();
        if (tid < 3) {
            float s = 0.f;
            for (int r = 0; r < TM; ++r) s += saux[r * 4 + tid];
            tp[TP_COL_B4 * 256 + tid] = s;
        }
        f32x16 acc[MT][2];
        acc_load_native(acc, cact + ((int64_t)3 * ntiles + tile) * TILE_F, wave, lane);
        {
            const int col0 = acc_col(wave, 0, lane), col1 = acc_col(wave, 1, lane);
            float w4[3][2];
            DH_UNROLL for (int j = 0; j < 3; ++j) { w4[j][0] = C.w4[j * 256 + col0]; w4[j][1] = C.w4[j * 256 + col1]; }
            float dw[3][2] = {{0.f, 0.f}, {0.f, 0.f}, {0.f, 0.f}};
            DH_UNROLL for (int m = 0; m < MT; ++m)
                DH_UNROLL for (int r = 0; r < 16; ++r) {
                    const f32x4 cr = *reinterpret_cast<const f32x4*>(saux + acc_row(m, r, lane) * 4);
                    DH_UNROLL for (int t = 0; t < 2; ++t) {
                        const float h = acc[m][t][r];
                        DH_UNROLL for (int j = 0; j < 3; ++j) dw[j][t] = fmaf(cr[j], h, dw[j][t]);
                        const float hb = cr[0] * w4[0][t] + cr[1] * w4[1][t] + cr[2] * w4[2][t];
                        acc[m][t][r] = h > 0.f ? hb : 0.f;
                    }
                }
            DH_UNROLL for (int j = 0; j < 3; ++j)
                DH_UNROLL for (int t = 0; t < 2; ++t) {
                    float s = dw[j][t];
                    s += __shfl_xor(s, 32);
                    if (lane < 32) tp[(TP_COL_W4 + j) * 256 + 64 * wave + 32 * t + lane] = s;
                }
        }
        acc_store_native(acc, czbar + ((int64_t)3 * ntiles + tile) * TILE_F, wave, lane);
        tile_colsum(acc, tp + (TP_COL_B0 + 3) * 256, wave, lane);
        acc_to_lds(acc, smain, wave, lane);
        __syncthreads();
        typename Core::Pre pre = Core::prefetch(C.rev_main[3], wave, lane);
        for (int l = 3; l >= 1; --l) {
            acc_zero(acc);
            Core::rows(acc, smain, LDX, Core::K_MAIN, C.rev_main[l], wave, lane, pre);
            pre = Core::prefetch(C.rev_main[l - 1], wave, lane);
            const f32x4* hp = reinterpret_cast<const f32x4*>(cact + ((int64_t)(l - 1) * ntiles + tile) * TILE_F) + (size_t)wave * MT * 8 * 64 + lane;
            DH_UNROLL for (int m = 0; m < MT; ++m) {
                DH_UNROLL for (int t = 0; t < 2; ++t)
                    DH_UNROLL for (int r4 = 0; r4 < 4; ++r4) {
                        const f32x4 h = DH_TILE_LD(hp + ((m * 2 + t) * 4 + r4) * 64);
                        DH_UNROLL for (int rr = 0; rr < 4; ++rr)
                            if (!(h[rr] > 0.f)) acc[m][t][4 * r4 + rr] = 0.f;
                    }
                __builtin_amdgcn_sched_barrier(0);
            }
            acc_store_native(acc, czbar + ((int64_t)(l - 1) * ntiles + tile) * TILE_F, wave, lane);
            tile_colsum(acc, tp + (TP_COL_B0 + l - 1) * 256, wave, lane);
            __syncthreads();
            acc_to_lds(acc, smain, wave, lane);
            __syncthreads();
        }
        acc_zero(acc);
        Core::rows(acc, smain, LDX, Core::K_MAIN, C.rev_main[0], wave, lane, pre);
        acc_store_native(acc, featbar + tile * TILE_F, wave, lane);
        f32x16 a2[AUX_NTW];
        aux_zero(a2);
        Core::auxout(a2, smain, C.rev_aux0, wave, lane);
        DH_UNROLL for (int tt = 0; tt < AUX_NTW; ++tt) {
            const int col = aux_col(wave, tt, lane);
            if (col >= 30 && col < 33) {
                DH_UNROLL for (int r = 0; r < 16; ++r) {
                    const int64_t gp = tile * TM + aux_row(wave, r, lane);
                    if (gp < npts) d_normals[gp * 3 + (col - 30)] += a2[tt][r];
                }
            }
        }
        if (RAYS) {
            __syncthreads();
            aux_acc_to_lds(a2, saux, CAUX, wave, lane);
            __syncthreads();
            if (tid < TM) {
                const int64_t gp = tile * TM + tid;
                if (gp < npts) point_view_adjoint(saux + tid * LDA, dirs, n_per_ray, gp, d_pts, d_dirs_pts);
            }
        }
        __syncthreads();
    }
}
template <bool RAYS>
__global__ __launch_bounds__(256, 2) void color_bwd_kernel(ColPtrs C, const float* __restrict__ colors,
                                                            const float* __restrict__ d_colors, int64_t npts,
                                                            const float* __restrict__ cact, float* __restrict__ czbar,
                                                            float* __restrict__ featbar, float* __restrict__ d_normals,
                                                            float* __restrict__ tpart, const float* __restrict__ dirs,
                                                            int n_per_ray, float* __restrict__ d_pts,
                                                            float* __restrict__ d_dirs_pts) {
    color_bwd_body<CoreF32, RAYS>(C, colors, d_colors, npts, cact, czbar, featbar, d_normals, tpart, dirs, n_per_ray, d_pts, d_dirs_pts);
}
template <bool RAYS>
__global__ __launch_bounds__(256, 2) void color_bwd_s_kernel(Col16Ptrs C, const float* __restrict__ colors,
                                                            const float* __restrict__ d_colors, int64_t npts,
                                                            const float* __restrict__ cact, float* __restrict__ czbar,
                                                            float* __restrict__ featbar, float* __restrict__ d_normals,
                                                            float* __restrict__ tpart, const float* __restrict__ dirs,
                                                            int n_per_ray, float* __restrict__ d_pts,
                                                            float* __restrict__ d_dirs_pts) {
    color_bwd_body<CoreBf16, RAYS>(C, colors, d_colors, npts, cact, czbar, featbar, d_normals, tpart, dirs, n_per_ray, d_pts, d_dirs_pts);
}


template <class Core>
__device__ __forceinline__ void sdf_tangent_body(const typename Core::Sdf& P, const float* pts, const float* d_normals, int64_t npts,
                                                 const float* act, const float* asave, float* t0aux, float* tsave, float* rsave,
                                                 float* tpart) {
    __shared__ __attribute__((aligned(16))) float smain[TM * LDX];
    __shared__ __attribute__((aligned(16))) float saux[TM * LDA];
    const int tid = threadIdx.x, wave = tid >> 6, lane = tid & 63;
    const int64_t ntiles = (npts + TM - 1) / TM;
    int it = 0;
    for (int64_t tile = blockIdx.x; tile < ntiles; tile += gridDim.x, ++it) {
        float* tp = tpart + tile * N_TILE_PART * 256;
        {
            const int p = tid & (TM - 1), part = tid / TM;
            const int64_t gp = tile * TM + p;
            float x[3] = {0.f, 0.f, 0.f}, nb[3] = {0.f, 0.f, 0.f};
            if (gp < npts) {
                DH_UNROLL for (int c = 0; c < 3; ++c) { x[c] = pts[gp * 3 + c]; nb[c] = d_normals[gp * 3 + c]; }
            }
            float* row = saux + p * LDA;
            if (part == 0) { row[0] = nb[0]; row[1] = nb[1]; row[2] = nb[2]; }
            if (part == 1) { for (int c = 39; c < LDA; ++c) row[c] = 0.f; }
            for (int k = part; k < 6; k += TPP) {
                const float f = (float)(1 << k);
                DH_UNROLL for (int c = 0; c < 3; ++c) {
                    float s, co;
                    sincosf(x[c] * f, &s, &co);
                    row[3 + 6 * k + c] = f * co * nb[c];
                    row[3 + 6 * k + 3 + c] = -f * s * nb[c];
                }
            }
        }
        __syncthreads();
        aux_lds_to_native(saux, t0aux + tile * AUXT_F, wave, lane);
        f32x16 acc[MT][2];
        typename Core::Pre pre = Core::prefetch(P.fwd_main[1], wave, lane);
        for (int l = 0; l < 8; ++l) {
            if constexpr (Core::STAMPS) DH_STAMP(it, l, 0);
            acc_zero(acc);
            if (l > 0) Core::rows(acc, smain, LDX, l == 4 ? Core::K_L4 : Core::K_MAIN, P.fwd_main[l], wave, lane, pre);
            if (l == 0 || l == 4) Core::rows(acc, saux, LDA, Core::K_AUX, P.fwd_aux[l], wave, lane);
            if (l < 7) pre = Core::prefetch(P.fwd_main[l + 1], wave, lane);
            if constexpr (Core::STAMPS) DH_STAMP(it, l, 1);
            const size_t woff = (size_t)wave * MT * 8 * 64 + lane;
            const f32x4* hp = reinterpret_cast<const f32x4*>(act + ((int64_t)l * ntiles + tile) * TILE_F) + woff;
            const f32x4* ap = reinterpret_cast<const f32x4*>(asave + ((int64_t)l * ntiles + tile) * TILE_F) + woff;
            f32x4* rp = reinterpret_cast<f32x4*>(rsave + ((int64_t)l * ntiles + tile) * TILE_F) + woff;
            DH_UNROLL for (int m = 0; m < MT; ++m) {
                DH_UNROLL for (int t = 0; t < 2; ++t)
                    DH_UNROLL for (int r4 = 0; r4 < 4; ++r4) {
                        const int idx = ((m * 2 + t) * 4 + r4) * 64;
// ... 101 lines not shown
            }
            if (l == 7) {
                ws0 += __shfl_xor(ws0, 32); ws1 += __shfl_xor(ws1, 32);
                if (lane < 32) {
                    tp[TP_W8ROW0_S * 256 + 64 * wave + lane] = ws0;
                    tp[TP_W8ROW0_S * 256 + 64 * wave + 32 + lane] = ws1;
                }
            }
            acc_store_native(acc, zbar + ((int64_t)l * ntiles + tile) * TILE_F, wave, lane);
            tile_colsum(acc, tp + (TP_SDF_B0 + l) * 256, wave, lane);
            if (l > 0) {
                __syncthreads();
                acc_to_lds(acc, smain, wave, lane);
                __syncthreads();
                if (RAYS && l == 4) Core::auxout(eb, smain, P.rev_aux[4], wave, lane);
                acc_zero(acc);
                Core::rows(acc, smain, LDX, Core::K_MAIN, P.rev_main[l], wave, lane, pre);
                if (l > 1) pre = Core::prefetch(P.rev_main[l - 1], wave, lane);
            } else if (RAYS) {
                __syncthreads();
                acc_to_lds(acc, smain, wave, lane);
                __syncthreads();
                Core::auxout(eb, smain, P.rev_aux[0], wave, lane);
                aux_acc_to_lds(eb, saux, AUXW, wave, lane);
                __syncthreads();
                if (tid < TM) {
                    const int64_t gp = tile * TM + tid;
                    if (gp < npts) point_sdf_adjoint(saux + tid * LDA, pts, d_normals, gesave, gp, d_pts);
                }
            }
        }
        __syncthreads();
    }
}
template <bool RAYS>
__global__ __launch_bounds__(256, 2) void sdf_bwd_kernel(SdfPtrs P, const float* __restrict__ d_sdf, int64_t npts,
                                                          const float* __restrict__ act, const float* __restrict__ rsave,
                                                          const float* __restrict__ featbar, float* __restrict__ zbar,
                                                          float* __restrict__ tpart, const float* __restrict__ pts,
                                                          const float* __restrict__ d_normals, const float* __restrict__ gesave,
                                                          float* __restrict__ d_pts) {
    sdf_bwd_body<CoreF32, RAYS>(P, d_sdf, npts, act, rsave, featbar, zbar, tpart, pts, d_normals, gesave, d_pts);
}
template <bool RAYS>
__global__ __launch_bounds__(256, 2) void sdf_bwd_s_kernel(Sdf16Ptrs P, const float* __restrict__ d_sdf, int64_t npts,
                                                          const float* __restrict__ act, const float* __restrict__ rsave,
                                                          const float* __restrict__ featbar, float* __restrict__ zbar,
                                                          float* __restrict__ tpart, const float* __restrict__ pts,
                                                          const float* __restrict__ d_normals, const float* __restrict__ gesave,
                                                          float* __restrict__ d_pts) {
    sdf_bwd_body<CoreBf16, RAYS>(P, d_sdf, npts, act, rsave, featbar, zbar, tpart, pts, d_normals, gesave, d_pts);
}

int launch_color_bwd(const float* packed, const float* colors, const float* d_colors, int64_t npts, const float* cact,
                     float* czbar, float* featbar, float* d_normals, float* tpart, float* absmax, int grid, int arith, hipStream_t st) {
    const int form = arith >> 8;
    arith &= 0xff;
    if (arith == ARITH_F16) {
        unsigned* am = reinterpret_cast<unsigned*>(absmax);
        if (use_pair_form(form, npts, false)) return launch_color_bwd_p(packed, colors, d_colors, npts, cact, czbar, featbar, d_normals, tpart, am,
                                                                 am + ABSMAX_FLOATS, st);
        return launch_color_bwd_h(packed, colors, d_colors, nullptr, 1, npts, cact, czbar, featbar, d_normals, tpart, nullptr, nullptr, am,
                                  am + ABSMAX_FLOATS, grid, st);
    }
    if (arith == ARITH_FP32) hipLaunchKernelGGL(color_bwd_kernel<false>, dim3(grid_for(npts, grid)), dim3(256), 0, st, make_col_ptrs(packed), colors,
                                                d_colors, npts, cact, czbar, featbar, d_normals, tpart, nullptr, 1, nullptr, nullptr);
    else hipLaunchKernelGGL(color_bwd_s_kernel<false>, dim3(grid_for(npts, grid)), dim3(256), 0, st, make_col16_ptrs(packed), colors,
                            d_colors, npts, cact, czbar, featbar, d_normals, tpart, nullptr, 1, nullptr, nullptr);
    return ok();
}
int launch_color_bwd_rays(const float* packed, const float* colors, const float* d_colors, const float* dirs, int n_per_ray,
                          int64_t npts, const float* cact, float* czbar, float* featbar, float* d_normals, float* tpart,
                          float* d_pts, float* d_dirs_pts, float* absmax, int grid, int arith, hipStream_t st) {
    if (arith == ARITH_F16) return launch_color_bwd_h(packed, colors, d_colors, dirs, n_per_ray, npts, cact, czbar, featbar, d_normals, tpart, d_pts,
                                                     d_dirs_pts, reinterpret_cast<unsigned*>(absmax), reinterpret_cast<unsigned*>(absmax) + ABSMAX_FLOATS, grid, st);
    if (arith == ARITH_FP32) hipLaunchKernelGGL(color_bwd_kernel<true>, dim3(grid_for(npts, grid)), dim3(256), 0, st, make_col_ptrs(packed), colors,
                                                d_colors, npts, cact, czbar, featbar, d_normals, tpart, dirs, n_per_ray, d_pts, d_dirs_pts);
    else hipLaunchKernelGGL(color_bwd_s_kernel<true>, dim3(grid_for(npts, grid)), dim3(256), 0, st, make_col16_ptrs(packed), colors,
                            d_colors, npts, cact, czbar, featbar, d_normals, tpart, dirs, n_per_ray, d_pts, d_dirs_pts);
    return ok();
}
int launch_sdf_tangent(const float* packed, const float* pts, const float* d_normals, int64_t npts, const float* act,
                       const float* asave, float* t0aux, float* tsave, float* rsave, float* tpart, float* absmax, int grid, int arith,
                       hipStream_t st) {
    if (arith == ARITH_F16) return launch_sdf_tangent_h(packed, pts, d_normals, npts, act, asave, t0aux, tsave, rsave, tpart,
                                                       reinterpret_cast<unsigned*>(absmax), reinterpret_cast<unsigned*>(absmax) + ABSMAX_FLOATS, grid, st);
    if (arith == ARITH_FP32) hipLaunchKernelGGL(sdf_tangent_kernel, dim3(grid_for(npts, grid)), dim3(256), 0, st, make_sdf_ptrs(packed), pts,
                                                d_normals, npts, act, asave, t0aux, tsave, rsave, tpart);
    else hipLaunchKernelGGL(sdf_tangent_s_kernel, dim3(grid_for(npts, grid)), dim3(256), 0, st, make_sdf16_ptrs(packed), pts, d_normals,
                            npts, act, asave, t0aux, tsave, rsave, tpart);
    return ok();
}
int launch_sdf_bwd(const float* packed, const float* d_sdf, int64_t npts, const float* act, const float* rsave,
                   const float* featbar, float* zbar, float* tpart, float* absmax, int grid, int arith, hipStream_t st) {
    if (arith == ARITH_F16) return launch_sdf_bwd_h(packed, d_sdf, nullptr, nullptr, npts, act, rsave, featbar, nullptr, zbar, tpart, nullptr,
                                                   reinterpret_cast<unsigned*>(absmax), reinterpret_cast<unsigned*>(absmax) + ABSMAX_FLOATS, grid, st);
    if (arith == ARITH_FP32) hipLaunchKernelGGL(sdf_bwd_kernel<false>, dim3(grid_for(npts, grid)), dim3(256), 0, st, make_sdf_ptrs(packed), d_sdf, npts,
                                                act, rsave, featbar, zbar, tpart, nullptr, nullptr, nullptr, nullptr);
    else hipLaunchKernelGGL(sdf_bwd_s_kernel<false>, dim3(grid_for(npts, grid)), dim3(256), 0, st, make_sdf16_ptrs(packed), d_sdf, npts,
                            act, rsave, featbar, zbar, tpart, nullptr, nullptr, nullptr, nullptr);
    return ok();
}
int launch_sdf_bwd_rays(const float* packed, const float* d_sdf, const float* pts, const float* d_normals, int64_t npts,
                        const float* act, const float* rsave, const float* featbar, const float* gesave, float* zbar,
                        float* tpart, float* d_pts, float* absmax, int grid, int arith, hipStream_t st) {
    if (arith == ARITH_F16) return launch_sdf_bwd_h(packed, d_sdf, pts, d_normals, npts, act, rsave, featbar, gesave, zbar, tpart, d_pts,
                                                   reinterpret_cast<unsigned*>(absmax), reinterpret_cast<unsigned*>(absmax) + ABSMAX_FLOATS, grid, st);
    if (arith == ARITH_FP32) hipLaunchKernelGGL(sdf_bwd_kernel<true>, dim3(grid_for(npts, grid)), dim3(256), 0, st, make_sdf_ptrs(packed), d_sdf, npts,
                                                act, rsave, featbar, zbar, tpart, pts, d_normals, gesave, d_pts);
    else hipLaunchKernelGGL(sdf_bwd_s_kernel<true>, dim3(grid_for(npts, grid)), dim3(256), 0, st, make_sdf16_ptrs(packed), d_sdf, npts, act,
                            rsave, featbar, zbar, tpart, pts, d_normals, gesave, d_pts);
    return ok();
}

}
```

dynhor_amd/csrc/kernels_mlp_h.hip:

```cpp
#include "tile.h"
#include "kernels.h"
#include "mlp_common.h"
#include "tile16h.h"
#include "workspace.h"
#include "stamps.h"

DH_STAMP_READER(dh_dev_read_stamps_h)

namespace dh {

#ifndef H2_LEAN2
#define H2_LEAN2 true
#endif

enum : int { TP_SDF_B0 = 0, TP_SDF_B8 = 8, TP_W8ROW0_T = 9, TP_W8ROW0_S = 10, TP_SCAL = 11, TP_COL_B0 = 12,
             TP_COL_W4 = 16, TP_COL_B4 = 19 };

struct SdfHPtrs {
    const u32x4* main[N_SDF];
    const u32x4* aux[N_SDF];
    const u32x4* rev[N_SDF];
    const u32x4* revaux[N_SDF];
    const float* bias[N_SDF];
    const float* w8row0;
// ... 55 lines not shown
        if (tslot) *tslot = __builtin_bit_cast(unsigned, m);
    }
    if (extra_lds) extra_max = fmaxf(extra_max, *extra_lds);
    const TileScale ts = scale_for_max(fmaxf(m, extra_max));
    acc_to_lds_split(acc, smain, wave, lane, ts.S);
    DH_STAMP(sit, slayer, 5);
    __syncthreads();
    DH_STAMP(sit, slayer, 6);
    return ts;
}

#ifdef DH_STAMPS
template <int KC>
__device__ __forceinline__ void gemm_stamped_steps(f32x16 (&acc)[MT][2], H2 (&a)[2][MT], H2 (&b)[4][2], const _Float16* xrow, rsrc_t wr, int woff, int it, int wave,
                                                   int lane, bool on) {
    if constexpr (KC < 16) {
        if (on) DH_STAMP(it, 5 + (KC >> 3), KC & 7);
        if constexpr (KC + 3 < 16) {
            DH_UNROLL for (int t = 0; t < 2; ++t)
                DH_UNROLL for (int p = 0; p < 2; ++p)
                    b[(KC + 3) & 3][t].p[p] = __builtin_amdgcn_raw_buffer_load_b128(wr, woff + (t * 2 + p) * 1024, (KC + 3) * (8 * 2 * 64 * 16), 0);
        }
        if constexpr (KC + 1 < 16) {
            DH_UNROLL for (int m = 0; m < MT; ++m)
                DH_UNROLL for (int p = 0; p < 2; ++p)
                    a[(KC + 1) & 1][m].p[p] = *reinterpret_cast<const u32x4*>(xrow + p * PLANE_H + m * 32 * LDH + (KC + 1) * 16);
        }
        __builtin_amdgcn_sched_barrier(0);
        mfma_only_h<0, 12>(acc, a[KC & 1], b[KC & 3]);
        __builtin_amdgcn_sched_barrier(0);
        gemm_stamped_steps<KC + 1>(acc, a, b, xrow, wr, woff, it, wave, lane, on);
    }
}
__device__ __forceinline__ void gemm_rows_stamped(f32x16 (&acc)[MT][2], const _Float16* img, const u32x4* __restrict__ wp, int wave, int lane, int it, bool on) {
    const _Float16* xrow = img + (lane & 31) * LDH + 8 * (lane >> 5);
    const rsrc_t wr = weight_rsrc(wp);
    const int woff = ((2 * wave) * 2 * 64 + lane) * 16;
    H2 a[2][MT], b[4][2];
    DH_UNROLL for (int kc = 0; kc < 3; ++kc)
        DH_UNROLL for (int t = 0; t < 2; ++t)
            DH_UNROLL for (int p = 0; p < 2; ++p)
                b[kc][t].p[p] = __builtin_amdgcn_raw_buffer_load_b128(wr, woff + (t * 2 + p) * 1024, kc * (8 * 2 * 64 * 16), 0);
    DH_UNROLL for (int m = 0; m < MT; ++m)
        DH_UNROLL for (int p = 0; p < 2; ++p) a[0][m].p[p] = *reinterpret_cast<const u32x4*>(xrow + p * PLANE_H + m * 32 * LDH);
    gemm_stamped_steps<0>(acc, a, b, xrow, wr, woff, it, wave, lane, on);
    if (on) DH_STAMP(it, 7, 0);
}
#endif

__global__ __launch_bounds__(256, 2) void color_fwd_h_kernel(ColHPtrs C, const float* __restrict__ pts, const float* __restrict__ dirs,
                                                            int n_per_ray, const float* __restrict__ normals,
                                                            const float* __restrict__ feat, int64_t npts,
                                                            float* __restrict__ color, float* __restrict__ cact,
                                                            float* __restrict__ caux, int save, unsigned* __restrict__ absmax) {
    __shared__ __attribute__((aligned(16))) _Float16 smain[IMG_H];
    __shared__ __attribute__((aligned(16))) float saux[TM * LDA];
    __shared__ HScratch hs;
    const int tid = threadIdx.x, wave = tid >> 6, lane = tid & 63;
    const int loff = tile_loff(wave, lane);
    const int64_t ntiles = (npts + TM - 1) / TM;
    hs_init(hs, tid);
    float winv[4];
    DH_UNROLL for (int l = 0; l < 4; ++l) winv[l] = winv_from_bits(C.wabs[l]);
    int it = 0;
    for (int64_t tile = blockIdx.x; tile < ntiles; tile += gridDim.x, ++it) {
        (void)it;
        if (tid < TM) {
            const int64_t gp = tile * TM + tid;
            float* row = saux + tid * LDA;
            float mx = 1.f;
            const int64_t first = tile * TM, last = first + TM - 1 < npts ? first + TM - 1 : npts - 1;
            const bool one_ray = first / n_per_ray == last / n_per_ray;
            float esin = 0.f, ecos = 0.f;
            if (one_ray && lane < 12) sincosf(dirs[(first / n_per_ray) * 3 + lane % 3] * (float)(1 << (lane / 3)), &esin, &ecos);
            if (gp < npts) {
                const int64_t ray = gp / n_per_ray;
                DH_UNROLL for (int c = 0; c < 3; ++c) {
                    const float d = dirs[ray * 3 + c], x = pts[gp * 3 + c], nn = normals[gp * 3 + c];
                    row[c] = x;
                    row[3 + c] = d;
                    DH_UNROLL for (int k = 0; k < 4; ++k) {
                        float s, co;
                        if (one_ray) {
                            s = __builtin_bit_cast(float, __builtin_amdgcn_readlane(__builtin_bit_cast(int, esin), 3 * k + c));
                            co = __builtin_bit_cast(float, __builtin_amdgcn_readlane(__builtin_bit_cast(int, ecos), 3 * k + c));
                        } else {
                            sincosf(d * (float)(1 << k), &s, &co);
                        }
                        row[6 + 6 * k + c] = s;
                        row[6 + 6 * k + 3 + c] = co;
                    }
                    row[30 + c] = nn;
                    mx = fmaxf(mx, fmaxf(fabsf(x), fmaxf(fabsf(d), fabsf(nn))));
                }
            } else {
                DH_UNROLL for (int c = 0; c < CAUX; ++c) row[c] = 0.f;
            }
            DH_UNROLL for (int c = CAUX; c < LDA; ++c) row[c] = 0.f;
            mx = wave_max(mx);
            if (lane == 0) hs.sred2[0] = mx;
        }
        f32x16 acc[MT][2];
        acc_load_native_b(acc, tile_rsrc(feat + tile * TILE_F), loff);
        TileScale ts = lds_handoff(acc, smain, hs, save ? &hs.lmax[4] : nullptr, tid, wave, lane, 0.f, &hs.sred2[0]);
        if (save && tid == 0) hs.lmax[5] = fmaxf(hs.lmax[5], hs.sred2[0]);
        if (save) aux_lds_to_native(saux, caux + tile * AUXT_F, wave, lane);
        for (int l = 0; l < 4; ++l) {
            DH_STAMP(it, l, 0);
            acc_zero(acc);
#ifdef DH_STAMPS
            gemm_rows_stamped(acc, smain, C.main[l], wave, lane, it, l == 1);
#else
            gemm_rows_hp(acc, smain, 16, C.main[l], wave, lane);
#endif
            const float inv = ts.inv * winv[l];
            if (l == 0) gemm_rows_aux_h(acc, saux, C.aux, wave, lane, ts.S);
            DH_STAMP(it, l, 1);
            const float b0 = C.bias[l][acc_col(wave, 0, lane)], b1 = C.bias[l][acc_col(wave, 1, lane)];
            acc_map(acc, [&](int, int t, int, float v) { return fmaxf(fmaf(v, inv, t ? b1 : b0), 0.f); });
            if (save) acc_store_native_b(acc, tile_rsrc(cact + ((int64_t)l * ntiles + tile) * TILE_F), loff);
            DH_STAMP(it, l, 2);
            ts = lds_handoff(acc, smain, hs, save ? &hs.lmax[l] : nullptr, tid, wave, lane, 0.f, nullptr, nullptr, it, l);
        }
        DH_STAMP(it, 4, 0);
        const int64_t gp = tile * TM + tid / TPP;
        DH_UNROLL for (int j = 0; j < 3; ++j) {
            const float raw = fmaf(row_dot256_hp(smain, C.w4 + j * 256, tid), ts.inv, C.b4[j]);
            if (tid % TPP == 0 && gp < npts) color[gp * 3 + j] = 1.f / (1.f + __expf(-raw));
        }
        __syncthreads();
    }
    if (save && absmax) {
        if (tid < 4) post_class_max(absmax, ABSMAX_CACT + tid, hs.lmax[tid]);
        if (tid == 4) post_class_max(absmax, ABSMAX_FEAT, hs.lmax[4]);
        if (tid == 5) post_class_max(absmax, ABSMAX_CAUX, hs.lmax[5]);
    }
}

__global__ __launch_bounds__(256, 2) void sdf_grad_h_kernel(SdfHPtrs P, const float* __restrict__ pts, int64_t npts,
                                                           const float* __restrict__ act, float* __restrict__ asave,
                                                           float* __restrict__ normals, int save, float* __restrict__ gesave,
                                                           unsigned* __restrict__ absmax) {
    __shared__ __attribute__((aligned(16))) _Float16 smain[IMG_H];
    __shared__ __attribute__((aligned(16))) float saux[TM * LDA];
    __shared__ HScratch hs;
    const int tid = threadIdx.x, wave = tid >> 6, lane = tid & 63;
    const int loff = tile_loff(wave, lane);
    const int64_t ntiles = (npts + TM - 1) / TM;
    hs_init(hs, tid);
    unsigned hmax = 0u;
    int it = 0;
    for (int64_t tile = blockIdx.x; tile < ntiles; tile += gridDim.x, ++it) {
        (void)it;
        f32x16 acc[MT][2];
        f32x16 ge[AUX_NTW];
        aux_zero(ge);
        TileScale ts;
        {
            const float w0 = P.w8row0[acc_col(wave, 0, lane)], w1 = P.w8row0[acc_col(wave, 1, lane)];
            acc_load_native_b(acc, tile_rsrc(act + ((int64_t)7 * ntiles + tile) * TILE_F), loff);
            DH_UNROLL for (int m = 0; m < MT; ++m) DH_UNROLL for (int t = 0; t < 2; ++t)
                DH_UNROLL for (int r = 0; r < 16; r += 2) hmax = watch_max3(hmax, acc[m][t][r], acc[m][t][r + 1]);
            acc_map(acc, [&](int, int t, int, float h) { float s, em; softplus_deriv_from_h(h, s, em); return (t ? w1 : w0) * s; });
            if (save) acc_store_native_b(acc, tile_rsrc(asave + ((int64_t)7 * ntiles + tile) * TILE_F), loff);
            ts = lds_handoff(acc, smain, hs, &hs.lmax[7], tid, wave, lane);
        }
        for (int l = 7; l >= 1; --l) {
            DH_STAMP(it, l, 0);
            acc_zero(acc);
            const rsrc_t hr = tile_rsrc(act + ((int64_t)(l - 1) * ntiles + tile) * TILE_F);
            Slab h0, h1;
            gemm_rows_hp<false>(acc, smain, 16, P.rev[l], wave, lane, [&] { slab_ld(h0, hr, loff, 0); });
            DH_STAMP(it, l, 1);
// ... 17 lines not shown
                    }
                __builtin_amdgcn_sched_barrier(0);
            }
            if (save) acc_store_native_b(acc, tile_rsrc(asave + ((int64_t)(l - 1) * ntiles + tile) * TILE_F), loff);
            DH_STAMP(it, l, 2);
            ts = lds_handoff(acc, smain, hs, &hs.lmax[l - 1], tid, wave, lane, 0.f, nullptr, nullptr, it, l);
        }
        DH_STAMP(it, 0, 0);
        {
            f32x16 g0[AUX_NTW];
            aux_zero(g0);
            gemm_auxout_hp(g0, smain, 16, P.revaux[0], wave, lane);
            const float inv = ts.inv * winv_from_bits(P.wabs[0]);
            DH_UNROLL for (int tt = 0; tt < AUX_NTW; ++tt) DH_UNROLL for (int r = 0; r < 16; ++r) ge[tt][r] = fmaf(g0[tt][r], inv, ge[tt][r]);
        }
        DH_UNROLL for (int tt = 0; tt < AUX_NTW; ++tt) {
            const int col = aux_col(wave, tt, lane);
            if (col < AUXW) {
                DH_UNROLL for (int r = 0; r < 16; ++r) saux[aux_row(wave, r, lane) * LDA + col] = ge[tt][r];
            }
        }
        __syncthreads();
        if (tid < TM) {
            const int64_t gp = tile * TM + tid;
            if (gp < npts) {
                const float* g = saux + tid * LDA;
                float n[3];
                DH_UNROLL for (int c = 0; c < 3; ++c) {
                    const float x = pts[gp * 3 + c];
                    float v = g[c];
                    DH_UNROLL for (int k = 0; k < 6; ++k) {
                        const float f = (float)(1 << k);
                        float s, co; sincosf(x * f, &s, &co);
                        v += f * (co * g[3 + 6 * k + c] - s * g[3 + 6 * k + 3 + c]);
                    }
                    n[c] = v;
                }
                normals[gp * 3 + 0] = n[0]; normals[gp * 3 + 1] = n[1]; normals[gp * 3 + 2] = n[2];
                if (save == 2) { for (int c = 0; c < 40; ++c) gesave[gp * 40 + c] = c < EMB ? g[c] : 0.f; }
            }
        }
        __syncthreads();
    }
    if (save && absmax && tid < 8) post_class_max(absmax, ABSMAX_ASAVE + tid, hs.lmax[tid]);
    if (absmax) {
        const float m = wave_max(watch_close(hmax));
        if (lane == 0) post_class_max(absmax, ABSMAX_ACT, m);
    }
}

template <bool RAYS>
__global__ __launch_bounds__(256, 2) void color_bwd_h_kernel(ColHPtrs C, const float* __restrict__ colors,
                                                            const float* __restrict__ d_colors, int64_t npts,
                                                            const float* __restrict__ cact, float* __restrict__ czbar,
                                                            float* __restrict__ featbar, float* __restrict__ d_normals,
                                                            float* __restrict__ tpart, const float* __restrict__ dirs,
                                                            int n_per_ray, float* __restrict__ d_pts,
                                                            float* __restrict__ d_dirs_pts, unsigned* __restrict__ absmax,
                                                            unsigned* __restrict__ tmax) {
    __shared__ __attribute__((aligned(16))) _Float16 smain[IMG_H];
    __shared__ __attribute__((aligned(16))) float saux[TM * LDA];
    __shared__ HScratch hs;
    const int tid = threadIdx.x, wave = tid >> 6, lane = tid & 63;
    const int loff = tile_loff(wave, lane);
    const int64_t ntiles = (npts + TM - 1) / TM;
    hs_init(hs, tid);
    for (int64_t tile = blockIdx.x; tile < ntiles; tile += gridDim.x) {
        float* tp = tpart + tile * N_TILE_PART * 256;
        if (tid < TM) {
            const int64_t gp = tile * TM + tid;
            DH_UNROLL for (int j = 0; j < 3; ++j) {
                float v = 0.f;
                if (gp < npts) { const float c = colors[gp * 3 + j]; v = d_colors[gp * 3 + j] * c * (1.f - c); }
                saux[tid * 4 + j] = v;
            }
            saux[tid * 4 + 3] = 0.f;
        }
        __syncthreads();
        if (tid < 3) {
            float s = 0.f;
            for (int r = 0; r < TM; ++r) s += saux[r * 4 + tid];
            tp[TP_COL_B4 * 256 + tid] = s;
        }
        f32x16 acc[MT][2];
        acc_load_native_b(acc, tile_rsrc(cact + ((int64_t)3 * ntiles + tile) * TILE_F), loff);
        {
            const int col0 = acc_col(wave, 0, lane), col1 = acc_col(wave, 1, lane);
            float w4[3][2];
            DH_UNROLL for (int j = 0; j < 3; ++j) { w4[j][0] = C.w4[j * 256 + col0]; w4[j][1] = C.w4[j * 256 + col1]; }
            float dw[3][2] = {{0.f, 0.f}, {0.f, 0.f}, {0.f, 0.f}};
            DH_UNROLL for (int m = 0; m < MT; ++m)
                DH_UNROLL for (int r = 0; r < 16; ++r) {
                    const f32x4 cr = *reinterpret_cast<const f32x4*>(saux + acc_row(m, r, lane) * 4);
                    DH_UNROLL for (int t = 0; t < 2; ++t) {
                        const float h = acc[m][t][r];
                        DH_UNROLL for (int j = 0; j < 3; ++j) dw[j][t] = fmaf(cr[j], h, dw[j][t]);
                        const float hb = cr[0] * w4[0][t] + cr[1] * w4[1][t] + cr[2] * w4[2][t];
                        acc[m][t][r] = h > 0.f ? hb : 0.f;
                    }
                }
            DH_UNROLL for (int j = 0; j < 3; ++j)
                DH_UNROLL for (int t = 0; t < 2; ++t) {
                    float s = dw[j][t];
                    s += __shfl_xor(s, 32);
                    if (lane < 32) tp[(TP_COL_W4 + j) * 256 + 64 * wave + 32 * t + lane] = s;
                }
        }
        acc_store_native_b(acc, tile_rsrc(czbar + ((int64_t)3 * ntiles + tile) * TILE_F), loff);
        tile_colsum(acc, tp + (TP_COL_B0 + 3) * 256, wave, lane);
        TileScale ts = lds_handoff(acc, smain, hs, &hs.lmax[3], tid, wave, lane, 0.f, nullptr, tmax + (TMAX_CZBAR + 3) * ntiles + tile);
        for (int l = 3; l >= 1; --l) {
            acc_zero(acc);
            const rsrc_t hr = tile_rsrc(cact + ((int64_t)(l - 1) * ntiles + tile) * TILE_F);
            Slab h0, h1;
            gemm_rows_hp<false>(acc, smain, 16, C.rev[l], wave, lane, [&] { slab_ld(h0, hr, loff, 0); });
            slab_ld(h1, hr, loff, 1);
            const float inv = ts.inv * winv_from_bits(C.wabs[l]);
            DH_UNROLL for (int m = 0; m < MT; ++m) {
                const Slab& hs_ = m ? h1 : h0;
                DH_UNROLL for (int t = 0; t < 2; ++t)
                    DH_UNROLL for (int r4 = 0; r4 < 4; ++r4) {
                        const f32x4 h = hs_.v[t * 4 + r4];
                        DH_UNROLL for (int rr = 0; rr < 4; ++rr)
                            acc[m][t][4 * r4 + rr] = h[rr] > 0.f ? acc[m][t][4 * r4 + rr] * inv : 0.f;
                    }
                __builtin_amdgcn_sched_barrier(0);
            }
            acc_store_native_b(acc, tile_rsrc(czbar + ((int64_t)(l - 1) * ntiles + tile) * TILE_F), loff);
            tile_colsum(acc, tp + (TP_COL_B0 + l - 1) * 256, wave, lane);
            ts = lds_handoff(acc, smain, hs, &hs.lmax[l - 1], tid, wave, lane, 0.f, nullptr, tmax + (TMAX_CZBAR + l - 1) * ntiles + tile);
        }
        const float inv0 = ts.inv * winv_from_bits(C.wabs[0]);
        acc_zero(acc);
        gemm_rows_hp(acc, smain, 16, C.rev[0], wave, lane);
        acc_map(acc, [&](int, int, int, float v) { return v * inv0; });
        acc_store_native_b(acc, tile_rsrc(featbar + tile * TILE_F), loff);
        tile_max_publish(hs.sred2, wave, lane, acc_absmax(acc));
        f32x16 a2[AUX_NTW];
        aux_zero(a2);
        gemm_auxout_hp(a2, smain, 16, C.revaux, wave, lane);
        DH_UNROLL for (int tt = 0; tt < AUX_NTW; ++tt) DH_UNROLL for (int r = 0; r < 16; ++r) a2[tt][r] *= inv0;
        DH_UNROLL for (int tt = 0; tt < AUX_NTW; ++tt) {
            const int col = aux_col(wave, tt, lane);
            if (col >= 30 && col < 33) {
                DH_UNROLL for (int r = 0; r < 16; ++r) {
                    const int64_t gp = tile * TM + aux_row(wave, r, lane);
                    if (gp < npts) d_normals[gp * 3 + (col - 30)] += a2[tt][r];
                }
            }
        }
        if (RAYS) {
            __syncthreads();
            DH_UNROLL for (int tt = 0; tt < AUX_NTW; ++tt) {
                const int col = aux_col(wave, tt, lane);
                if (col < CAUX) {
                    DH_UNROLL for (int r = 0; r < 16; ++r) saux[aux_row(wave, r, lane) * LDA + col] = a2[tt][r];
                }
            }
            __syncthreads();
            if (tid < TM) {
                const int64_t gp = tile * TM + tid;
                if (gp < npts) {
                    const float* row = saux + tid * LDA;
                    const int64_t ray = gp / n_per_ray;
                    DH_UNROLL for (int c = 0; c < 3; ++c) {
                        d_pts[gp * 3 + c] = row[c];
                        const float dv = dirs[ray * 3 + c];
                        float v = row[3 + c];
                        DH_UNROLL for (int kf = 0; kf < 4; ++kf) {
                            const float f = (float)(1 << kf);
                            float sn, co; sincosf(dv * f, &sn, &co);
                            v += f * (co * row[6 + 6 * kf + c] - sn * row[6 + 6 * kf + 3 + c]);
                        }
                        d_dirs_pts[gp * 3 + c] = v;
                    }
                }
            }
        }
        __syncthreads();
        if (tid == 0) {
            const float m = tile_max_read(hs.sred2);
            hs.lmax[4] = fmaxf(hs.lmax[4], m);
            tmax[TMAX_FEATBAR * ntiles + tile] = __builtin_bit_cast(unsigned, m);
        }
    }
    if (absmax) {
        if (tid < 4) post_class_max(absmax, ABSMAX_CZBAR + tid, hs.lmax[tid]);
        if (tid == 4) post_class_max(absmax, ABSMAX_FEATBAR, hs.lmax[4]);
    }
}

__global__ __launch_bounds__(256, 2) void sdf_tangent_h_kernel(SdfHPtrs P, const float* __restrict__ pts,
                                                              const float* __restrict__ d_normals, int64_t npts,
                                                              const float* __restrict__ act, const float* __restrict__ asave,
                                                              float* __restrict__ t0aux, float* __restrict__ tsave,
                                                              float* __restrict__ rsave, float* __restrict__ tpart,
                                                              unsigned* __restrict__ absmax, unsigned* __restrict__ tmax) {
    __shared__ __attribute__((aligned(16))) _Float16 smain[IMG_H];
    __shared__ __attribute__((aligned(16))) float saux[TM * LDA];
    __shared__ HScratch hs;
    const int tid = threadIdx.x, wave = tid >> 6, lane = tid & 63;
    const int loff = tile_loff(wave, lane);
    const int64_t ntiles = (npts + TM - 1) / TM;
    hs_init(hs, tid);
    for (int64_t tile = blockIdx.x; tile < ntiles; tile += gridDim.x) {
        float* tp = tpart + tile * N_TILE_PART * 256;
        {
            const int p = tid & (TM - 1), part = tid / TM;
            const int64_t gp = tile * TM + p;
// ... 154 lines not shown
                {
                    f32x16 e0[AUX_NTW];
                    aux_zero(e0);
                    gemm_auxout_hp(e0, smain, 16, P.revaux[0], wave, lane);
                    const float inv = ts.inv * winv_from_bits(P.wabs[0]);
                    DH_UNROLL for (int tt = 0; tt < AUX_NTW; ++tt) DH_UNROLL for (int r = 0; r < 16; ++r) eb[tt][r] = fmaf(e0[tt][r], inv, eb[tt][r]);
                }
                DH_UNROLL for (int tt = 0; tt < AUX_NTW; ++tt) {
                    const int col = aux_col(wave, tt, lane);
                    if (col < AUXW) {
                        DH_UNROLL for (int r = 0; r < 16; ++r) saux[aux_row(wave, r, lane) * LDA + col] = eb[tt][r];
                    }
                }
                __syncthreads();
                if (tid < TM) {
                    const int64_t gp = tile * TM + tid;
                    if (gp < npts) {
                        const float* e = saux + tid * LDA;
                        const float* ge = gesave + gp * 40;
                        DH_UNROLL for (int c = 0; c < 3; ++c) {
                            const float x = pts[gp * 3 + c], nb = d_normals[gp * 3 + c];
                            float v = e[c], dn = 0.f;
                            DH_UNROLL for (int k = 0; k < 6; ++k) {
                                const float f = (float)(1 << k);
                                float sn, co; sincosf(x * f, &sn, &co);
                                v += f * (co * e[3 + 6 * k + c] - sn * e[3 + 6 * k + 3 + c]);
                                dn -= f * f * (sn * ge[3 + 6 * k + c] + co * ge[3 + 6 * k + 3 + c]);
                            }
                            d_pts[gp * 3 + c] += v + nb * dn;
                        }
                    }
                }
            } else {
                tile_max_publish(hs.sred2, wave, lane, acc_absmax(acc));
            }
        }
        __syncthreads();
        if (!RAYS && tid == 0) {
            const float m = tile_max_read(hs.sred2);
            hs.lmax[0] = fmaxf(hs.lmax[0], m);
            tmax[TMAX_ZBAR * ntiles + tile] = __builtin_bit_cast(unsigned, m);
        }
    }
    if (absmax && tid < 8) post_class_max(absmax, ABSMAX_ZBAR + tid, hs.lmax[tid]);
}

int launch_sdf_grad_h(const float* packed, const float* pts, int64_t npts, const float* act, float* asave, float* normals,
                      int save, float* gesave, unsigned* absmax, int grid, hipStream_t stream) {
    hipLaunchKernelGGL(sdf_grad_h_kernel, dim3(grid_for(npts, grid)), dim3(256), 0, stream, make_sdfh_ptrs(packed), pts, npts, act,
                       asave, normals, save, gesave, absmax);
    return ok();
}
int launch_color_fwd_h(const float* packed, const float* pts, const float* dirs, int n_per_ray, const float* normals,
                       const float* feat, int64_t npts, float* color, float* cact, float* caux, int save, unsigned* absmax,
                       int grid, hipStream_t stream) {
    hipLaunchKernelGGL(color_fwd_h_kernel, dim3(grid_for(npts, grid)), dim3(256), 0, stream, make_colh_ptrs(packed), pts, dirs,
                       n_per_ray, normals, feat, npts, color, cact, caux, save, absmax);
    return ok();
}
int launch_color_bwd_h(const float* packed, const float* colors, const float* d_colors, const float* dirs, int n_per_ray,
                       int64_t npts, const float* cact, float* czbar, float* featbar, float* d_normals, float* tpart,
                       float* d_pts, float* d_dirs_pts, unsigned* absmax, unsigned* tmax, int grid, hipStream_t st) {
    if (d_pts) hipLaunchKernelGGL(color_bwd_h_kernel<true>, dim3(grid_for(npts, grid)), dim3(256), 0, st, make_colh_ptrs(packed), colors,
                                  d_colors, npts, cact, czbar, featbar, d_normals, tpart, dirs, n_per_ray, d_pts, d_dirs_pts, absmax, tmax);
    else hipLaunchKernelGGL(color_bwd_h_kernel<false>, dim3(grid_for(npts, grid)), dim3(256), 0, st, make_colh_ptrs(packed), colors,
                            d_colors, npts, cact, czbar, featbar, d_normals, tpart, nullptr, 1, nullptr, nullptr, absmax, tmax);
    return ok();
}
int launch_sdf_tangent_h(const float* packed, const float* pts, const float* d_normals, int64_t npts, const float* act,
                         const float* asave, float* t0aux, float* tsave, float* rsave, float* tpart, unsigned* absmax, unsigned* tmax,
                         int grid, hipStream_t st) {
    hipLaunchKernelGGL(sdf_tangent_h_kernel, dim3(grid_for(npts, grid)), dim3(256), 0, st, make_sdfh_ptrs(packed), pts, d_normals,
                       npts, act, asave, t0aux, tsave, rsave, tpart, absmax, tmax);
    return ok();
}
int launch_sdf_bwd_h(const float* packed, const float* d_sdf, const float* pts, const float* d_normals, int64_t npts,
                     const float* act, const float* rsave, const float* featbar, const float* gesave, float* zbar, float* tpart,
                     float* d_pts, unsigned* absmax, unsigned* tmax, int grid, hipStream_t st) {
    if (d_pts) hipLaunchKernelGGL(sdf_bwd_h_kernel<true>, dim3(grid_for(npts, grid)), dim3(256), 0, st, make_sdfh_ptrs(packed), d_sdf, npts,
                                  act, rsave, featbar, zbar, tpart, pts, d_normals, gesave, d_pts, absmax, tmax);
    else hipLaunchKernelGGL(sdf_bwd_h_kernel<false>, dim3(grid_for(npts, grid)), dim3(256), 0, st, make_sdfh_ptrs(packed), d_sdf, npts,
                            act, rsave, featbar, zbar, tpart, nullptr, nullptr, nullptr, nullptr, absmax, tmax);
    return ok();
}

}
```

dynhor_amd/csrc/tile.h:

```cpp
#pragma once
#include <hip/hip_runtime.h>
#include "layout.h"

namespace dh {

typedef float f32x16 __attribute__((ext_vector_type(16)));
typedef float f32x4 __attribute__((ext_vector_type(4)));

#define DH_UNROLL _Pragma("unroll")

__device__ __forceinline__ void acc_zero(f32x16 (&acc)[MT][2]) {
    DH_UNROLL for (int m = 0; m < MT; ++m)
        DH_UNROLL for (int t = 0; t < 2; ++t)
            DH_UNROLL for (int r = 0; r < 16; ++r) acc[m][t][r] = 0.f;
}

__device__ __forceinline__ void mfma_block(f32x16 (&acc)[MT][2], const f32x4 (&a)[MT], const f32x4 (&b)[2]) {
    DH_UNROLL for (int s = 0; s < 4; ++s)
        DH_UNROLL for (int m = 0; m < MT; ++m)
            DH_UNROLL for (int t = 0; t < 2; ++t)
                acc[m][t] = __builtin_amdgcn_mfma_f32_32x32x2f32(a[m][s], b[t][s], acc[m][t], 0, 0, 0);
}
struct BFrag { f32x4 b[2]; };
__device__ __forceinline__ BFrag gemm_b_prefetch(const f32x4* __restrict__ wp, const int wave, const int lane) {
// ... 12 lines not shown
    _Pragma("unroll 1") for (int kg = 0; kg < nkg; kg += 2) {
        const int k1 = (kg + 1 < nkg) ? kg + 1 : kg;
        DH_UNROLL for (int t = 0; t < 2; ++t) b1[t] = wl[(k1 * 8 + t) * 64];
        DH_UNROLL for (int m = 0; m < MT; ++m) a1[m] = *reinterpret_cast<const f32x4*>(xrow + m * 32 * ldx + k1 * 8);
        __builtin_amdgcn_sched_barrier(0);
        mfma_block(acc, a0, b0);
        __builtin_amdgcn_sched_barrier(0);
        if (kg + 1 < nkg) {
            const int k2 = (kg + 2 < nkg) ? kg + 2 : kg + 1;
            DH_UNROLL for (int t = 0; t < 2; ++t) b0[t] = wl[(k2 * 8 + t) * 64];
            DH_UNROLL for (int m = 0; m < MT; ++m) a0[m] = *reinterpret_cast<const f32x4*>(xrow + m * 32 * ldx + k2 * 8);
            __builtin_amdgcn_sched_barrier(0);
            mfma_block(acc, a1, b1);
            __builtin_amdgcn_sched_barrier(0);
        }
    }
}
__device__ __forceinline__ void gemm_rows(f32x16 (&acc)[MT][2], const float* xs, const int ldx, const int nkg,
                                          const f32x4* __restrict__ wp, const int wave, const int lane) {
    gemm_rows(acc, xs, ldx, nkg, wp, wave, lane, gemm_b_prefetch(wp, wave, lane));
}

constexpr int AUX_WPM = 4 / MT;
constexpr int AUX_NTW = 2 / AUX_WPM;
__device__ __forceinline__ int aux_mtile(int wave) { return wave / AUX_WPM; }
__device__ __forceinline__ int aux_ntile(int wave, int tt) { return (wave % AUX_WPM) * AUX_NTW + tt; }
__device__ __forceinline__ void gemm_auxout(f32x16 (&acc2)[AUX_NTW], const float* xs, const int nkg,
                                            const f32x4* __restrict__ wp, const int wave, const int lane) {
    const float* xrow = xs + (32 * aux_mtile(wave) + (lane & 31)) * LDX + 4 * (lane >> 5);
    const f32x4* wl = wp + aux_ntile(wave, 0) * 64 + lane;
    f32x4 a = *reinterpret_cast<const f32x4*>(xrow);
    f32x4 b[AUX_NTW];
    DH_UNROLL for (int t = 0; t < AUX_NTW; ++t) b[t] = wl[t * 64];
    _Pragma("unroll 2") for (int kg = 0; kg < nkg; ++kg) {
        const int kn = (kg + 1 < nkg) ? kg + 1 : kg;
        f32x4 an = *reinterpret_cast<const f32x4*>(xrow + kn * 8);
        f32x4 bn[AUX_NTW];
        DH_UNROLL for (int t = 0; t < AUX_NTW; ++t) bn[t] = wl[(kn * 2 + t) * 64];
        __builtin_amdgcn_sched_barrier(0);
        DH_UNROLL for (int s = 0; s < 4; ++s)
            DH_UNROLL for (int t = 0; t < AUX_NTW; ++t)
                acc2[t] = __builtin_amdgcn_mfma_f32_32x32x2f32(a[s], b[t][s], acc2[t], 0, 0, 0);
        __builtin_amdgcn_sched_barrier(0);
        a = an;
        DH_UNROLL for (int t = 0; t < AUX_NTW; ++t) b[t] = bn[t];
    }
}
__device__ __forceinline__ void aux_zero(f32x16 (&a2)[AUX_NTW]) {
    DH_UNROLL for (int t = 0; t < AUX_NTW; ++t) DH_UNROLL for (int r = 0; r < 16; ++r) a2[t][r] = 0.f;
}
__device__ __forceinline__ int aux_row(int wave, int r, int lane) { return 32 * aux_mtile(wave) + (r & 3) + 8 * (r >> 2) + 4 * (lane >> 5); }
__device__ __forceinline__ int aux_col(int wave, int tt, int lane) { return 32 * aux_ntile(wave, tt) + (lane & 31); }

__device__ __forceinline__ int acc_row(int m, int r, int lane) { return m * 32 + (r & 3) + 8 * (r >> 2) + 4 * (lane >> 5); }
__device__ __forceinline__ int acc_col(int wave, int t, int lane) { return 64 * wave + 32 * t + (lane & 31); }

__device__ __forceinline__ void acc_to_lds(const f32x16 (&acc)[MT][2], float* xs, int wave, int lane) {
    DH_UNROLL for (int m = 0; m < MT; ++m)
        DH_UNROLL for (int t = 0; t < 2; ++t) {
            float* base = xs + (m * 32 + 4 * (lane >> 5)) * LDX + acc_col(wave, t, lane);
            DH_UNROLL for (int r = 0; r < 16; ++r) base[((r & 3) + 8 * (r >> 2)) * LDX] = acc[m][t][r];
        }
}

#define DH_TILE_LD(ptr) __builtin_nontemporal_load(ptr)
#define DH_TILE_ST(ptr, v) __builtin_nontemporal_store(v, ptr)
__device__ __forceinline__ void acc_store_native(const f32x16 (&acc)[MT][2], float* __restrict__ tile, int wave, int lane) {
    f32x4* p = reinterpret_cast<f32x4*>(tile) + (size_t)wave * MT * 8 * 64 + lane;
    DH_UNROLL for (int m = 0; m < MT; ++m)
        DH_UNROLL for (int t = 0; t < 2; ++t)
            DH_UNROLL for (int r4 = 0; r4 < 4; ++r4) {
                f32x4 v;
                v[0] = acc[m][t][4 * r4 + 0]; v[1] = acc[m][t][4 * r4 + 1];
                v[2] = acc[m][t][4 * r4 + 2]; v[3] = acc[m][t][4 * r4 + 3];
                DH_TILE_ST(&p[((m * 2 + t) * 4 + r4) * 64], v);
            }
}
__device__ __forceinline__ void acc_load_native(f32x16 (&acc)[MT][2], const float* __restrict__ tile, int wave, int lane) {
    const f32x4* p = reinterpret_cast<const f32x4*>(tile) + (size_t)wave * MT * 8 * 64 + lane;
    DH_UNROLL for (int m = 0; m < MT; ++m)
        DH_UNROLL for (int t = 0; t < 2; ++t)
            DH_UNROLL for (int r4 = 0; r4 < 4; ++r4) {
                f32x4 v = DH_TILE_LD(&p[((m * 2 + t) * 4 + r4) * 64]);
                acc[m][t][4 * r4 + 0] = v[0]; acc[m][t][4 * r4 + 1] = v[1];
                acc[m][t][4 * r4 + 2] = v[2]; acc[m][t][4 * r4 + 3] = v[3];
            }
}

__device__ __forceinline__ void aux_store_native(const f32x16 (&a2)[AUX_NTW], float* __restrict__ tile, int wave, int lane) {
    f32x4* p = reinterpret_cast<f32x4*>(tile) + lane;
    DH_UNROLL for (int tt = 0; tt < AUX_NTW; ++tt)
        DH_UNROLL for (int r4 = 0; r4 < 4; ++r4) {
            f32x4 v;
            v[0] = a2[tt][4 * r4 + 0]; v[1] = a2[tt][4 * r4 + 1]; v[2] = a2[tt][4 * r4 + 2]; v[3] = a2[tt][4 * r4 + 3];
            p[((aux_mtile(wave) * 2 + aux_ntile(wave, tt)) * 4 + r4) * 64] = v;
        }
}
__device__ __forceinline__ void aux_lds_to_native(const float* aux, float* __restrict__ tile, int wave, int lane) {
    f32x16 a2[AUX_NTW];
    DH_UNROLL for (int tt = 0; tt < AUX_NTW; ++tt) {
        const int col = aux_col(wave, tt, lane);
        DH_UNROLL for (int r = 0; r < 16; ++r)
            a2[tt][r] = (col < AUXW) ? aux[aux_row(wave, r, lane) * LDA + col] : 0.f;
    }
    aux_store_native(a2, tile, wave, lane);
}

__device__ __forceinline__ float softplus100(float z) {
    const float e = __builtin_amdgcn_exp2f(-fabsf(z) * (SOFTPLUS_BETA * 1.44269504088896f));
    const float l = __builtin_amdgcn_logf(1.f + e);
    return fmaf(l, 0.69314718055995f / SOFTPLUS_BETA, fmaxf(z, 0.f));
}
__device__ __forceinline__ void softplus_deriv_from_h(float h, float& s, float& em) {
    em = __builtin_amdgcn_exp2f(h * (-SOFTPLUS_BETA * 1.44269504088896f));
    s = 1.f - em;
}

}
```

dynhor_amd/csrc/tile16h.h:

```cpp
#pragma once
#include "tile16.h"
#include "workspace.h"

namespace dh {

typedef _Float16 f16x8 __attribute__((ext_vector_type(8)));
typedef _Float16 f16x2v __attribute__((ext_vector_type(2)));
struct H2 { u32x4 p[2]; };
__device__ __forceinline__ unsigned pack_f16x2(f32x2 v) { return __builtin_bit_cast(unsigned, __builtin_convertvector(v, f16x2v)); }
__device__ __forceinline__ f32x2 resid_f16x2(f32x2 v, unsigned h) {
    f32x2 r;
#ifdef H2_VISIBLE_RESID
    const f16x2v hv = __builtin_bit_cast(f16x2v, h);
    r[0] = v[0] - (float)hv[0];
    r[1] = v[1] - (float)hv[1];
#else
    asm("v_fma_mix_f32 %0, -%1, 1.0, %2 op_sel_hi:[1,0,0]" : "=v"(r[0]) : "v"(h), "v"(v[0]));
    asm("v_fma_mix_f32 %0, -%1, 1.0, %2 op_sel:[1,0,0] op_sel_hi:[1,0,0]" : "=v"(r[1]) : "v"(h), "v"(v[1]));
#endif
    return r;
}
__device__ __forceinline__ f32x16 mfma_h(const u32x4& a, const u32x4& b, const f32x16& c) {
    return __builtin_amdgcn_mfma_f32_32x32x16_f16(__builtin_bit_cast(f16x8, a), __builtin_bit_cast(f16x8, b), c, 0, 0, 0);
}
// ... 107 lines not shown
        f32x2 x;
        x[0] = q < 2 ? raw.lo[m][2 * q] : raw.hi[m][2 * q - 4];
        x[1] = q < 2 ? raw.lo[m][2 * q + 1] : raw.hi[m][2 * q - 3];
        if constexpr (SC) { x[0] *= st.sc; x[1] *= st.sc; }
        a[m].p[0][q] = pack_f16x2(x);
        st.r[j] = x;
    } else if constexpr (s == 1) {
        st.r[j] = resid_f16x2(st.r[j], a[m].p[0][q]);
    } else {
        a[m].p[1][q] = pack_f16x2(st.r[j]);
    }
}

template <int I>
__device__ __forceinline__ void mfma_step_h(f32x16 (&acc)[MT][2], const H2 (&a)[MT], const H2 (&b)[2]) {
    constexpr int pa[3] = {0, 1, 0}, pb[3] = {1, 0, 0};
    constexpr int p = I / (2 * MT), mt = I % (2 * MT), m = mt / 2, t = mt % 2;
    acc[m][t] = mfma_h(a[m].p[pa[p]], b[t].p[pb[p]], acc[m][t]);
}
template <int I, int N>
__device__ __forceinline__ void mfma_only_h(f32x16 (&acc)[MT][2], const H2 (&ac)[MT], const H2 (&bc)[2]) {
    if constexpr (I < N) { mfma_step_h<I>(acc, ac, bc); mfma_only_h<I + 1, N>(acc, ac, bc); }
}

typedef __amdgpu_buffer_rsrc_t rsrc_t;
__device__ __forceinline__ rsrc_t tile_rsrc(const float* tile) {
    return __builtin_amdgcn_make_buffer_rsrc(const_cast<float*>(tile), 0, TILE_F * 4, 0x00020000);
}
__device__ __forceinline__ int tile_loff(int wave, int lane) { return (wave * MT * 8 * 64 + lane) * 16; }
__device__ __forceinline__ f32x4 tile_ld(rsrc_t r, int loff, int idx) {
    const int off = idx * 1024;
    return __builtin_bit_cast(f32x4, __builtin_amdgcn_raw_buffer_load_b128(r, loff + (off & 4095), off & ~4095, 2));
}
__device__ __forceinline__ void tile_st(rsrc_t r, int loff, int idx, const f32x4& v) {
    __builtin_amdgcn_raw_buffer_store_b128(__builtin_bit_cast(u32x4, v), r, loff + idx * 1024, 0, 2);
}
__device__ __forceinline__ void acc_store_native_b(const f32x16 (&acc)[MT][2], rsrc_t r, int loff) {
    DH_UNROLL for (int m = 0; m < MT; ++m)
        DH_UNROLL for (int t = 0; t < 2; ++t)
            DH_UNROLL for (int r4 = 0; r4 < 4; ++r4) {
                f32x4 v;
                v[0] = acc[m][t][4 * r4 + 0]; v[1] = acc[m][t][4 * r4 + 1]; v[2] = acc[m][t][4 * r4 + 2]; v[3] = acc[m][t][4 * r4 + 3];
                tile_st(r, loff, (m * 2 + t) * 4 + r4, v);
            }
}
__device__ __forceinline__ void acc_load_native_b(f32x16 (&acc)[MT][2], rsrc_t r, int loff) {
    DH_UNROLL for (int m = 0; m < MT; ++m)
        DH_UNROLL for (int t = 0; t < 2; ++t)
            DH_UNROLL for (int r4 = 0; r4 < 4; ++r4) {
                const f32x4 v = tile_ld(r, loff, (m * 2 + t) * 4 + r4);
                acc[m][t][4 * r4 + 0] = v[0]; acc[m][t][4 * r4 + 1] = v[1]; acc[m][t][4 * r4 + 2] = v[2]; acc[m][t][4 * r4 + 3] = v[3];
            }
}
struct Slab { f32x4 v[8]; };
__device__ __forceinline__ void slab_ld(Slab& s, rsrc_t r, int loff, int m) {
    DH_UNROLL for (int i = 0; i < 8; ++i) s.v[i] = tile_ld(r, loff, m * 8 + i);
}
__device__ __forceinline__ rsrc_t weight_rsrc(const u32x4* wp) {
    return __builtin_amdgcn_make_buffer_rsrc(const_cast<u32x4*>(wp), 0, 0x40000000, 0x00020000);
}

struct NoPre { __device__ __forceinline__ void operator()() const {} };
template <bool LEAN = false, class Pre = NoPre>
__device__ __forceinline__ void gemm_rows_hp(f32x16 (&acc)[MT][2], const _Float16* img, const int nkc,
                                             const u32x4* __restrict__ wp, const int wave, const int lane, Pre&& pre = Pre()) {
    static_assert(MT == 2, "");
    const _Float16* xrow = img + (lane & 31) * LDH + 8 * (lane >> 5);
    const rsrc_t wr = weight_rsrc(wp);
    const int woff = ((2 * wave) * 2 * 64 + lane) * 16;
    auto loadb = [&](H2 (&b)[2], int kc) {
        DH_UNROLL for (int t = 0; t < 2; ++t)
            DH_UNROLL for (int p = 0; p < 2; ++p)
                b[t].p[p] = __builtin_amdgcn_raw_buffer_load_b128(wr, woff + (t * 2 + p) * 1024, kc * (8 * 2 * 64 * 16), 0);
    };
    auto loada = [&](H2 (&a)[MT], int kc) {
        DH_UNROLL for (int m = 0; m < MT; ++m)
            DH_UNROLL for (int p = 0; p < 2; ++p)
                a[m].p[p] = *reinterpret_cast<const u32x4*>(xrow + p * PLANE_H + m * 32 * LDH + kc * 16);
    };
    H2 a0[MT], a1[MT];
    if constexpr (LEAN) {
        H2 b0[2], b1[2];
        loadb(b0, 0); loada(a0, 0);
        _Pragma("unroll 1") for (int kc = 0; kc < nkc; kc += 2) {
            loadb(b1, kc + 1); loada(a1, kc + 1);
            __builtin_amdgcn_sched_barrier(0);
            mfma_only_h<0, 12>(acc, a0, b0);
            __builtin_amdgcn_sched_barrier(0);
            if (kc + 2 < nkc) { loadb(b0, kc + 2); loada(a0, kc + 2); }
            else pre();
            __builtin_amdgcn_sched_barrier(0);
            mfma_only_h<0, 12>(acc, a1, b1);
            __builtin_amdgcn_sched_barrier(0);
        }
        return;
    }
    H2 bA[2], bB[2], bC[2], bD[2];
    auto step2 = [&](int c, H2 (&b0)[2], H2 (&b1)[2], H2 (&b2)[2], H2 (&b3)[2]) {
        loadb(b2, c + 2); loada(a1, c + 1);
        __builtin_amdgcn_sched_barrier(0);
        mfma_only_h<0, 12>(acc, a0, b0);
        __builtin_amdgcn_sched_barrier(0);
        loadb(b3, c + 3); loada(a0, c + 2);
        __builtin_amdgcn_sched_barrier(0);
        mfma_only_h<0, 12>(acc, a1, b1);
        __builtin_amdgcn_sched_barrier(0);
// ... 100 lines not shown
```

dynhor_amd/csrc/workspace.h:

```cpp
#pragma once
#include "layout.h"

namespace dh {

constexpr int N_TILE_PART = 20;
constexpr int DW_G = 256;
constexpr int DW_NS = 64;
int64_t dw_slab_floats(int G);

enum : int { ABSMAX_ASAVE = 0, ABSMAX_ZBAR = 8, ABSMAX_TSAVE = 16, ABSMAX_T0AUX = 23, ABSMAX_FEATBAR = 24, ABSMAX_CZBAR = 25,
             ABSMAX_CACT = 29, ABSMAX_FEAT = 33, ABSMAX_ACT = 34, ABSMAX_CAUX = 35, ABSMAX_TAG = 36, ABSMAX_N = 37 };
constexpr unsigned ABSMAX_TAG_F16 = 0x00F16F16u;
constexpr int ABSMAX_STRIDE = 64;
constexpr int ABSMAX_FLOATS = 64 * ABSMAX_STRIDE;
enum : int { TMAX_ZBAR = 0, TMAX_FEATBAR = 8, TMAX_CZBAR = 9, TMAX_TSAVE = 13, TMAX_T0AUX = 20, TMAX_N = 21 };

struct Workspace {
    int64_t ntiles;
    float* base;
    float* absmax;
    float* tmax;
    float* act;
    float* eaux;
    float* feat;
    float* asave;
    float* cact;
    float* caux;
    float* featbar;
    float* tsave;
    float* t0aux;
    float* rsave;
    float* zbar;
    float* czbar;
    float* tpart;
    float* tred;
    float* slabs;
    float* gesave;
    int64_t infer_floats, fwd_floats, total_floats;
};

inline Workspace carve_workspace(float* base, int64_t npts) {
    Workspace w{};
    const int64_t nt = (npts + TM - 1) / TM;
    w.ntiles = nt;
    w.base = base;
    int64_t o = 0;
    auto take = [&](int64_t n) { float* p = base ? base + o : nullptr; o += n; return p; };
    w.absmax = take(ABSMAX_FLOATS);
    w.tmax = take((TMAX_N * nt + 3) / 4 * 4);
    w.act = take(8 * nt * TILE_F);
    w.eaux = take(nt * AUXT_F);
    w.feat = take(nt * TILE_F);
    w.infer_floats = o;
    w.asave = take(8 * nt * TILE_F);
    w.cact = take(4 * nt * TILE_F);
    w.caux = take(nt * AUXT_F);
    w.fwd_floats = o;
    w.featbar = take(nt * TILE_F);
    w.tsave = take(7 * nt * TILE_F);
    w.t0aux = take(nt * AUXT_F);
    w.rsave = take(8 * nt * TILE_F);
    w.zbar = take(8 * nt * TILE_F);
    w.czbar = take(4 * nt * TILE_F);
    w.tpart = take(nt * N_TILE_PART * 256);
    w.tred = take((int64_t)DW_NS * N_TILE_PART * 256);
    w.slabs = take(dw_slab_floats(DW_G));
    w.gesave = take(nt * TM * 40);
    w.total_floats = o;
    return w;
}

}
```

include/dynhor_hip.h:

```cpp
#ifndef DYNHOR_HIP_H
#define DYNHOR_HIP_H
#include <stddef.h>
#include <stdint.h>

#ifdef __cplusplus
extern "C" {
#endif

typedef enum {
    DH_OK = 0,
    DH_ERR_BAD_ARG = -1,
    DH_ERR_UNSUPPORTED = -2,
    DH_ERR_LAUNCH = -3
} dh_status;

int dh_version(void);
const char* dh_strerror(int status);

typedef enum { DH_ARITH_SPLIT_BF16 = 0, DH_ARITH_FP32_MFMA = 1, DH_ARITH_SPLIT_F16 = 2 } dh_arithmetic;
enum { DH_CHAIN_FORM_TILE = 0x100, DH_CHAIN_FORM_PAIR = 0x200 };
int dh_set_arithmetic(int mode);
int dh_get_arithmetic(void);

int64_t dh_num_params(void);
int64_t dh_packed_floats(void);
int dh_param_layout(int net, int layer, int64_t* bias_off, int64_t* g_off, int64_t* v_off, int* out_dim, int* in_dim);

int dh_packed_section(int section, int64_t* offset_floats, int64_t* n_floats);

int dh_pack_weights(const float* params, float* packed, void* stream);

int dh_sdf_nograd(const float* packed, const float* pts, int64_t npts, float* sdf, void* stream);

int dh_workspace_floats(int64_t npts, int64_t* infer_floats, int64_t* fwd_floats, int64_t* total_floats);

int dh_range_words(int64_t* act_max_off, int64_t* tag_off, float* limit);

int dh_mlp_forward(const float* packed, const float* pts, const float* dirs, int n_per_ray, int64_t npts, float* ws,
                   float* sdf, float* normals, float* color, void* stream);

int dh_sdf_forward(const float* packed, const float* pts, int64_t npts, float* ws, float* sdf, void* stream);
int dh_sdf_gradient(const float* packed, const float* pts, int64_t npts, float* ws, float* normals, int save, void* stream);
int dh_color_forward(const float* packed, const float* pts, const float* dirs, int n_per_ray, const float* normals,
                     int64_t npts, float* ws, float* color, int save, void* stream);

int dh_mlp_backward(const float* packed, const float* params, const float* pts, int64_t npts, float* ws,
                    const float* colors, const float* d_sdf, float* d_normals, const float* d_colors, float* grad_flat,
                    void* stream);

int dh_color_backward(const float* packed, const float* colors, const float* d_colors, int64_t npts, float* ws,
                      float* d_normals, void* stream);
int dh_sdf_tangent(const float* packed, const float* pts, const float* d_normals, int64_t npts, float* ws, void* stream);
int dh_sdf_backward(const float* packed, const float* d_sdf, int64_t npts, float* ws, void* stream);
int dh_color_backward_rays(const float* packed, const float* colors, const float* d_colors, const float* dirs, int n_per_ray,
                           int64_t npts, float* ws, float* d_normals, float* d_pts, float* d_dirs_pts, void* stream);
int dh_sdf_backward_rays(const float* packed, const float* d_sdf, const float* pts, const float* d_normals, int64_t npts,
                         float* ws, float* d_pts, void* stream);
int dh_weight_grads_gemm(int64_t npts, float* ws, void* stream);
int dh_weight_grads_fold(const float* packed, const float* params, int64_t npts, float* ws, float* grad_flat, void* stream);

int dh_sdf_nograd_ex(int arithmetic, const float* packed, const float* pts, int64_t npts, float* sdf, void* stream);
int dh_mlp_forward_ex(int arithmetic, const float* packed, const float* pts, const float* dirs, int n_per_ray, int64_t npts, float* ws,
                      float* sdf, float* normals, float* color, void* stream);
int dh_sdf_forward_ex(int arithmetic, const float* packed, const float* pts, int64_t npts, float* ws, float* sdf, void* stream);
int dh_sdf_gradient_ex(int arithmetic, const float* packed, const float* pts, int64_t npts, float* ws, float* normals, int save,
                       void* stream);
int dh_color_forward_ex(int arithmetic, const float* packed, const float* pts, const float* dirs, int n_per_ray, const float* normals,
                        int64_t npts, float* ws, float* color, int save, void* stream);
int dh_mlp_backward_ex(int arithmetic, const float* packed, const float* params, const float* pts, int64_t npts, float* ws,
                       const float* colors, const float* d_sdf, float* d_normals, const float* d_colors, float* grad_flat,
                       void* stream);
int dh_color_backward_ex(int arithmetic, const float* packed, const float* colors, const float* d_colors, int64_t npts, float* ws,
                         float* d_normals, void* stream);
int dh_sdf_tangent_ex(int arithmetic, const float* packed, const float* pts, const float* d_normals, int64_t npts, float* ws,
                      void* stream);
int dh_sdf_backward_ex(int arithmetic, const float* packed, const float* d_sdf, int64_t npts, float* ws, void* stream);
int dh_color_backward_rays_ex(int arithmetic, const float* packed, const float* colors, const float* d_colors, const float* dirs,
                              int n_per_ray, int64_t npts, float* ws, float* d_normals, float* d_pts, float* d_dirs_pts, void* stream);
int dh_sdf_backward_rays_ex(int arithmetic, const float* packed, const float* d_sdf, const float* pts, const float* d_normals,
                            int64_t npts, float* ws, float* d_pts, void* stream);
int dh_weight_grads_gemm_ex(int arithmetic, int64_t npts, float* ws, void* stream);
int dh_pack_weights_ex(int arithmetic, const float* params, float* packed, void* stream);

int dh_gen_rays(const uint8_t* rgb, const int8_t* label, const uint8_t* normal, const float* R, const float* T,
                const float* Kinv, int H, int W, int n_frames, int frame, const int64_t* px, const int64_t* py, int64_t B,
                float* rays, float* near, float* far, void* stream);

// ... 137 lines not shown
```

Before: 230,900 rays/s.

## Save colour-MLP ReLU sign bitmasks in forward and use them in backward

The colour forward kernel now packs the ReLU activity of the first three hidden layers into per-lane 32-bit bitmasks and writes them to a new cmask workspace region. The backward kernels apply the ReLU derivative from these bits instead of reloading the full fp32 activation tiles from cact. This cuts backward memory traffic and register ring buffers, at the cost of an extra small store in forward and a larger workspace. The change also adds a few opaque_vgpr addressing tweaks and a workspace-region query API.

```diff
diff --git a/dynhor_amd/_lib.py b/dynhor_amd/_lib.py
--- a/dynhor_amd/_lib.py
+++ b/dynhor_amd/_lib.py
@@ -24,6 +24,7 @@
     "dh_pack_weights_ex": (_i32, [_i32, _vp, _vp, _vp]),
     "dh_sdf_nograd": (_i32, [_vp, _vp, _i64, _vp, _vp]),
     "dh_workspace_floats": (_i32, [_i64, ctypes.POINTER(_i64), ctypes.POINTER(_i64), ctypes.POINTER(_i64)]),
+    "dh_workspace_region": (_i32, [_i64, _i32, ctypes.POINTER(_i64), ctypes.POINTER(_i64)]),
     "dh_range_words": (_i32, [ctypes.POINTER(_i64), ctypes.POINTER(_i64), ctypes.POINTER(_f32)]),
     "dh_mlp_forward": (_i32, [_vp, _vp, _vp, _i32, _i64, _vp, _vp, _vp, _vp, _vp]),
     "dh_sdf_forward": (_i32, [_vp, _vp, _i64, _vp, _vp, _vp]),
@@ -215,6 +216,15 @@
     return a.value, t.value, lim.value
 
 
+WS_CACT, WS_CMASK, WS_CZBAR, WS_FEATBAR, WS_TPART = 0, 1, 2, 3, 4
+
+
+def workspace_region(npts: int, region: int):
+    o, n = _i64(), _i64()
+    check(lib().dh_workspace_region(npts, int(region), ctypes.byref(o), ctypes.byref(n)))
+    return o.value, n.value
+
+
 def workspace_floats(npts: int):
     i, f, t = _i64(), _i64(), _i64()
     check(lib().dh_workspace_floats(npts, ctypes.byref(i), ctypes.byref(f), ctypes.byref(t)))
diff --git a/dynhor_amd/csrc/api.hip b/dynhor_amd/csrc/api.hip
--- a/dynhor_amd/csrc/api.hip
+++ b/dynhor_amd/csrc/api.hip
@@ -113,6 +113,25 @@
     return DH_OK;
 }
 
+int dh_workspace_region(int64_t npts, int region, int64_t* offset_floats, int64_t* n_floats) {
+    if (npts < 0 || !offset_floats || !n_floats) return DH_ERR_BAD_ARG;
+    float* const origin = reinterpret_cast<float*>(uintptr_t(16));
+    const Workspace w = carve_workspace(origin, npts);
+    const float* p = nullptr;
+    int64_t n = 0;
+    switch (region) {
+        case DH_WS_CACT: p = w.cact; n = 4 * w.ntiles * TILE_F; break;
+        case DH_WS_CMASK: p = w.cmask; n = CMASK_LAYERS * w.ntiles * CMASK_F; break;
+        case DH_WS_CZBAR: p = w.czbar; n = 4 * w.ntiles * TILE_F; break;
+        case DH_WS_FEATBAR: p = w.featbar; n = w.ntiles * TILE_F; break;
+        case DH_WS_TPART: p = w.tpart; n = w.ntiles * N_TILE_PART * 256; break;
+        default: return DH_ERR_BAD_ARG;
+    }
+    *offset_floats = p - origin;
+    *n_floats = n;
+    return DH_OK;
+}
+
 int dh_range_words(int64_t* act_max_off, int64_t* tag_off, float* limit) {
     if (!act_max_off || !tag_off || !limit) return DH_ERR_BAD_ARG;
     *act_max_off = (int64_t)ABSMAX_ACT * ABSMAX_STRIDE;
@@ -146,7 +165,7 @@
     if (npts == 0) return DH_OK;
     if (!packed || !pts || !dirs || !normals || !ws || !color || misaligned16(packed) || misaligned16(ws)) return DH_ERR_BAD_ARG;
     const Workspace w = carve_workspace(ws, npts);
-    return launch_color_fwd(packed, pts, dirs, n_per_ray, normals, w.feat, npts, color, w.cact, w.caux, save, w.absmax, DEFAULT_GRID,
+    return launch_color_fwd(packed, pts, dirs, n_per_ray, normals, w.feat, npts, color, w.cact, w.caux, w.cmask, save, w.absmax, DEFAULT_GRID,
                             arithmetic, static_cast<hipStream_t>(stream));
 }
 
@@ -164,7 +183,7 @@
     if (npts <= 0 || bad_arith_form(arithmetic)) return DH_ERR_BAD_ARG;
     if (!packed || !colors || !d_colors || !ws || !d_normals || misaligned16(packed) || misaligned16(ws)) return DH_ERR_BAD_ARG;
     const Workspace w = carve_workspace(ws, npts);
-    return launch_color_bwd(packed, colors, d_colors, npts, w.cact, w.czbar, w.featbar, d_normals, w.tpart, w.absmax, DEFAULT_GRID,
+    return launch_color_bwd(packed, colors, d_colors, npts, w.cact, w.cmask, w.czbar, w.featbar, d_normals, w.tpart, w.absmax, DEFAULT_GRID,
                             arithmetic, static_cast<hipStream_t>(stream));
 }
 
@@ -191,7 +210,7 @@
     if (!packed || !colors || !d_colors || !dirs || !ws || !d_normals || !d_pts || !d_dirs_pts || misaligned16(packed) || misaligned16(ws))
         return DH_ERR_BAD_ARG;
     const Workspace w = carve_workspace(ws, npts);
-    return launch_color_bwd_rays(packed, colors, d_colors, dirs, n_per_ray, npts, w.cact, w.czbar, w.featbar, d_normals, w.tpart,
+    return launch_color_bwd_rays(packed, colors, d_colors, dirs, n_per_ray, npts, w.cact, w.cmask, w.czbar, w.featbar, d_normals, w.tpart,
                                  d_pts, d_dirs_pts, w.absmax, DEFAULT_GRID, arithmetic, static_cast<hipStream_t>(stream));
 }
 
diff --git a/dynhor_amd/csrc/chain_pair.hip b/dynhor_amd/csrc/chain_pair.hip
--- a/dynhor_amd/csrc/chain_pair.hip
+++ b/dynhor_amd/csrc/chain_pair.hip
@@ -42,11 +42,21 @@
     const int wave, lane, tid;
     const float inv, b0, b1;
     const rsrc_t st;
+    const rsrc_t mst;
     const int loff;
+    unsigned mw[MASK_DW] = {0u, 0u, 0u, 0u};
     __device__ __forceinline__ ColFwdEpi(f32x16 (&acc_)[MT][2], _Float16* img_, HScratchP& hs_, float* lmax_, int wave_, int lane_, int tid_,
-                                         float inv_, float b0_, float b1_, rsrc_t st_, int loff_, bool)
-        : acc(acc_), hs(hs_), lmax(lmax_), wave(wave_), lane(lane_), tid(tid_), inv(inv_), b0(b0_), b1(b1_), st(st_), loff(loff_) {
+                                         float inv_, float b0_, float b1_, rsrc_t st_, rsrc_t mst_, int loff_, bool)
+        : acc(acc_), hs(hs_), lmax(lmax_), wave(wave_), lane(lane_), tid(tid_), inv(inv_), b0(b0_), b1(b1_), st(st_), mst(mst_), loff(loff_) {
         this->handoff_init(img_, wave_, lane_);
+    }
+    template <int M, int T, int R>
+    __device__ __forceinline__ void mask_in() {
+        if constexpr (SAVE && DH_COL_MASK) {
+            constexpr int q = relu_mask_dword(M, T);
+            mw[q] = relu_mask_shift_in(mw[q], acc[M][T][R]);
+            if constexpr (R == 15) mw[q] = __builtin_bitreverse32(mw[q]) >> 16;
+        }
     }
     template <int G, int SUB>
     __device__ __forceinline__ void elem() {
@@ -56,6 +66,8 @@
             constexpr int r = 4 * r4 + 2 * SUB;
             acc[m][t][r] = fmaxf(fmaf(acc[m][t][r], inv, b), 0.f);
             acc[m][t][r + 1] = fmaxf(fmaf(acc[m][t][r + 1], inv, b), 0.f);
+            if constexpr (SUB == 0) mask_in<m, t, 4 * r4>();
+            else { mask_in<m, t, 4 * r4 + 1>(); mask_in<m, t, 4 * r4 + 2>(); }
         } else {
             if constexpr (SAVE) {
                 f32x4 v;
@@ -64,6 +76,8 @@
             }
             this->m0 = fmaxf(this->m0, fmaxf(fabsf(acc[m][t][4 * r4 + 0]), fabsf(acc[m][t][4 * r4 + 1])));
             this->m1 = fmaxf(this->m1, fmaxf(fabsf(acc[m][t][4 * r4 + 2]), fabsf(acc[m][t][4 * r4 + 3])));
+            mask_in<m, t, 4 * r4 + 3>();
+            if constexpr (SAVE && DH_COL_MASK && G == 15) mask_st(mst, tid, mw);
         }
     }
     __device__ __forceinline__ void publish(float wm) { tile_max_publish(hs.sred, wave, lane, wm); }
@@ -111,7 +125,7 @@
                                                             int n_per_ray, const float* __restrict__ normals,
                                                             const float* __restrict__ feat, int64_t npts, float* __restrict__ color,
                                                             float* __restrict__ cact, float* __restrict__ caux,
-                                                            unsigned* __restrict__ absmax) {
+                                                            float* __restrict__ cmask, unsigned* __restrict__ absmax) {
     __shared__ __attribute__((aligned(16))) _Float16 simg[2][IMG_H];
     __shared__ __attribute__((aligned(16))) float saux[2][TM * LDA];
     __shared__ HScratchP hs;
@@ -220,7 +234,8 @@
                 gemm_rows_aux_h(accA, saux[0], C.aux, wave, lane, tsA.S);
             } else {
                 ColFwdEpi<SAVE> e(accB, imgB, hs, SAVE ? &hs.lmax[l - 1] : nullptr, wave, lane, tid, tsB.inv * wp, p0, p1,
-                                  tile_rsrc_if(cact + ((int64_t)(l - 1) * ntiles + tileB) * TILE_F, okB), loff, okB);
+                                  tile_rsrc_if(cact + ((int64_t)(l - 1) * ntiles + tileB) * TILE_F, okB),
+                                  mask_rsrc(cmask, l - 1, ntiles, tileB, SAVE && okB), loff, okB);
                 if (son && l == 2) e.stamp = 18;
                 pair_phase<false>(accA, imgA, W, C.main0 + (int64_t)l * COL_MAIN_STRIDE, C.main0, wave, lane, e);
                 tsB.S = e.S; tsB.inv = e.inv_S;
@@ -231,7 +246,8 @@
             acc_zero(accB);
             {
                 ColFwdEpi<SAVE> e(accA, imgA, hs, SAVE ? &hs.lmax[l] : nullptr, wave, lane, tid, tsA.inv * wl, c0, c1,
-                                  tile_rsrc(cact + ((int64_t)l * ntiles + tileA) * TILE_F), loff, true);
+                                  tile_rsrc(cact + ((int64_t)l * ntiles + tileA) * TILE_F),
+                                  mask_rsrc(cmask, l < CMASK_LAYERS ? l : 0, ntiles, tileA, SAVE && l < CMASK_LAYERS), loff, true);
                 if (son && l == 2) e.stamp = 52;
                 pair_phase<true>(accB, imgB, W, C.main0 + (int64_t)l * COL_MAIN_STRIDE, C.main0 + (int64_t)(l < 3 ? l + 1 : 3) * COL_MAIN_STRIDE, wave, lane, e, l < 3);
                 if (l == 0) gemm_rows_aux_h(accB, saux[1], C.aux, wave, lane, tsB.S);
@@ -244,7 +260,7 @@
         const float w4a = C.w4[tid], w4b = C.w4[256 + tid], w4c = C.w4[512 + tid];
         {
             ColFwdEpi<SAVE> e(accB, imgB, hs, SAVE ? &hs.lmax[3] : nullptr, wave, lane, tid, tsB.inv * winv3, bs[3][0], bs[3][1],
-                              tile_rsrc_if(cact + ((int64_t)3 * ntiles + tileB) * TILE_F, okB), loff, okB);
+                              tile_rsrc_if(cact + ((int64_t)3 * ntiles + tileB) * TILE_F, okB), mask_rsrc(cmask, 0, ntiles, tileB, false), loff, okB);
             pair_epi_alone_from<0>(e);
             tsB.S = e.S; tsB.inv = e.inv_S;
         }
@@ -502,6 +518,13 @@
     C.wabs = reinterpret_cast<const unsigned*>(packed + PACKH.wabs) + N_SDF;
     return C;
 }
+struct ColSign {
+#if DH_COL_MASK
+    unsigned w[MASK_DW];
+#else
+    rsrc_t hr;
+#endif
+};
 template <bool LAST>
 struct ColBwdEpi : PEpi<ColBwdEpi<LAST>, 4, 3, !LAST> {
     static constexpr int RING = 5;
@@ -512,19 +535,34 @@
     float* csum;
     const int wave, lane, tid;
     const float inv;
-    const rsrc_t hr, st;
+    const rsrc_t st;
     const int loff;
     const bool store;
     float cs0 = 0.f, cs1 = 0.f;
+#if DH_COL_MASK
+    unsigned mw[MASK_DW];
+#else
+    rsrc_t hr;
     f32x4 hq[RING];
+#endif
     __device__ __forceinline__ ColBwdEpi(f32x16 (&acc_)[MT][2], _Float16* img_, HScratchP& hs_, float* lmax_, unsigned* tslot_, float* csum_,
-                                         int wave_, int lane_, int tid_, float inv_, rsrc_t hr_, rsrc_t st_, int loff_, bool store_)
-        : acc(acc_), hs(hs_), lmax(lmax_), tslot(tslot_), csum(csum_), wave(wave_), lane(lane_), tid(tid_), inv(inv_), hr(hr_),
+                                         int wave_, int lane_, int tid_, float inv_, const ColSign& sign, rsrc_t st_, int loff_, bool store_)
+        : acc(acc_), hs(hs_), lmax(lmax_), tslot(tslot_), csum(csum_), wave(wave_), lane(lane_), tid(tid_), inv(inv_),
           st(st_), loff(loff_), store(store_) {
-        if constexpr (!LAST) {
-            this->handoff_init(img_, wave_, lane_);
-            DH_UNROLL for (int g = 0; g < RING; ++g) hq[g] = tile_ld(hr, loff, g);
-        }
+        static_assert(!LAST, "the last epilogue (featbar) has no ReLU behind it");
+        this->handoff_init(img_, wave_, lane_);
+#if DH_COL_MASK
+        DH_UNROLL for (int q = 0; q < MASK_DW; ++q) mw[q] = sign.w[q];
+#else
+        hr = sign.hr;
+        DH_UNROLL for (int g = 0; g < RING; ++g) hq[g] = tile_ld(hr, loff, g);
+#endif
+    }
+    __device__ __forceinline__ ColBwdEpi(f32x16 (&acc_)[MT][2], HScratchP& hs_, int wave_, int lane_, int tid_, float inv_, rsrc_t st_, int loff_,
+                                         bool store_)
+        : acc(acc_), hs(hs_), lmax(nullptr), tslot(nullptr), csum(nullptr), wave(wave_), lane(lane_), tid(tid_), inv(inv_),
+          st(st_), loff(loff_), store(store_) {
+        static_assert(LAST, "");
     }
     template <int G, int SUB>
     __device__ __forceinline__ void elem() {
@@ -535,15 +573,22 @@
                 acc[m][t][r] *= inv;
                 acc[m][t][r + 1] *= inv;
             } else {
+#if DH_COL_MASK
+                acc[m][t][r] = relu_mask_keep(mw, m, t, r, acc[m][t][r] * inv);
+                acc[m][t][r + 1] = relu_mask_keep(mw, m, t, r + 1, acc[m][t][r + 1] * inv);
+#else
                 const f32x4& h = hq[G % RING];
                 acc[m][t][r] = h[i] > 0.f ? acc[m][t][r] * inv : 0.f;
                 acc[m][t][r + 1] = h[i + 1] > 0.f ? acc[m][t][r + 1] * inv : 0.f;
+#endif
             }
         } else if constexpr (SUB == 2) {
             f32x4 v;
             v[0] = acc[m][t][4 * r4 + 0]; v[1] = acc[m][t][4 * r4 + 1]; v[2] = acc[m][t][4 * r4 + 2]; v[3] = acc[m][t][4 * r4 + 3];
             tile_st(st, loff, G, v);
+#if !DH_COL_MASK
             if constexpr (!LAST && G + RING < 16) hq[G % RING] = tile_ld(hr, loff, G + RING);
+#endif
             if constexpr (!LAST) {
                 float& cs = t ? cs1 : cs0;
                 cs += acc[m][t][4 * r4 + 0]; cs += acc[m][t][4 * r4 + 1]; cs += acc[m][t][4 * r4 + 2]; cs += acc[m][t][4 * r4 + 3];
@@ -575,7 +620,8 @@
 #define COLBWD_NREG 8
 #endif
 __global__ __launch_bounds__(256, 1) void color_bwd_p_kernel(ColBwdPPtrs C, const float* __restrict__ colors, const float* __restrict__ d_colors,
-                                                            int64_t npts, const float* __restrict__ cact, float* __restrict__ czbar,
+                                                            int64_t npts, const float* __restrict__ cact, const float* __restrict__ cmask,
+                                                            float* __restrict__ czbar,
                                                             float* __restrict__ featbar, float* __restrict__ d_normals,
                                                             float* __restrict__ tpart, unsigned* __restrict__ absmax,
                                                             unsigned* __restrict__ tmax) {
@@ -587,8 +633,8 @@
     const int loff = tile_loff(wave, lane);
     const int64_t ntiles = (npts + TM - 1) / TM, npairs = (ntiles + 1) / 2;
     if (tid < 12) hs.lmax[tid] = 0.f;
-    const float wi0 = winv_from_bits(C.wabs[0]), wi1 = winv_from_bits(C.wabs[1]), wi2 = winv_from_bits(C.wabs[2]), wi3 = winv_from_bits(C.wabs[3]);
-    auto winv = [&](int l) { return l == 0 ? wi0 : l == 1 ? wi1 : l == 2 ? wi2 : wi3; };
+    auto winv = [&](int l) { return winv_from_bits(C.wabs[l]); };
+    const float wi0 = winv(0), wi1 = winv(1);
     auto rev = [&](int l) { return l == 0 ? C.rev0 : l == 1 ? C.rev1 : l == 2 ? C.rev2 : C.rev3; };
     PW<COLBWD_NREG> W;
     _Float16* imgA = simg[0];
@@ -616,6 +662,18 @@
             for (int r = 0; r < TM; ++r) sum += scraw[which][r * 4 + j];
             if (which == 0 || okB) (which ? tpB : tpA)[PTP_COL_B4 * 256 + j] = sum;
         }
+#if DH_COL_MASK
+        unsigned mA0[MASK_DW], mA1[MASK_DW], mA2[MASK_DW], mB0[MASK_DW], mB1[MASK_DW], mB2[MASK_DW];
+        mask_ld(mA2, mask_rsrc(cmask, 2, ntiles, tileA), tid); mask_ld(mB2, mask_rsrc(cmask, 2, ntiles, tileB), tid);
+        mask_ld(mA1, mask_rsrc(cmask, 1, ntiles, tileA), tid); mask_ld(mB1, mask_rsrc(cmask, 1, ntiles, tileB), tid);
+        mask_ld(mA0, mask_rsrc(cmask, 0, ntiles, tileA), tid); mask_ld(mB0, mask_rsrc(cmask, 0, ntiles, tileB), tid);
+        auto signA = [&](int k) { ColSign s; DH_UNROLL for (int q = 0; q < MASK_DW; ++q) s.w[q] = k == 2 ? mA2[q] : k == 1 ? mA1[q] : mA0[q]; return s; };
+        auto signB = [&](int k) { ColSign s; DH_UNROLL for (int q = 0; q < MASK_DW; ++q) s.w[q] = k == 2 ? mB2[q] : k == 1 ? mB1[q] : mB0[q]; return s; };
+#else
+        (void)cmask;
+        auto signA = [&](int k) { ColSign s; s.hr = tile_rsrc(cact + ((int64_t)k * ntiles + tileA) * TILE_F); return s; };
+        auto signB = [&](int k) { ColSign s; s.hr = tile_rsrc(cact + ((int64_t)k * ntiles + tileB) * TILE_F); return s; };
+#endif
         f32x16 accA[MT][2], accB[MT][2];
         TileScale tsA, tsB;
         DH_UNROLL for (int which = 0; which < 2; ++which) {
@@ -629,9 +687,10 @@
                 float w4[3][2];
                 DH_UNROLL for (int j = 0; j < 3; ++j) { w4[j][0] = C.w4[j * 256 + col0]; w4[j][1] = C.w4[j * 256 + col1]; }
                 float dw[3][2] = {{0.f, 0.f}, {0.f, 0.f}, {0.f, 0.f}};
+                const int crow = opaque_vgpr(4 * (lane >> 5));
                 DH_UNROLL for (int m = 0; m < MT; ++m)
                     DH_UNROLL for (int r = 0; r < 16; ++r) {
-                        const f32x4 cr = *reinterpret_cast<const f32x4*>(scraw[which] + acc_row(m, r, lane) * 4);
+                        const f32x4 cr = *reinterpret_cast<const f32x4*>(scraw[which] + (crow + acc_row(m, r, 0)) * 4);
                         DH_UNROLL for (int t = 0; t < 2; ++t) {
                             const float h = acc[m][t][r];
                             DH_UNROLL for (int j = 0; j < 3; ++j) dw[j][t] = fmaf(cr[j], h, dw[j][t]);
@@ -670,8 +729,7 @@
                 pair_phase<false>(accA, imgA, W, C.rev3, C.rev3, wave, lane, e);
             } else {
                 ColBwdEpi<false> e(accB, imgB, hs, &hs.lmax[l], tmax + (TMAX_CZBAR + l) * ntiles + tileB, tpB + (PTP_COL_B0 + l) * 256, wave, lane, tid,
-                                   tsB.inv * winv(l + 1), tile_rsrc(cact + ((int64_t)l * ntiles + tileB) * TILE_F),
-                                   tile_rsrc_if(czbar + ((int64_t)l * ntiles + tileB) * TILE_F, okB), loff, okB);
+                                   tsB.inv * winv(l + 1), signB(l), tile_rsrc_if(czbar + ((int64_t)l * ntiles + tileB) * TILE_F, okB), loff, okB);
                 pair_phase<false>(accA, imgA, W, rev(l), C.rev3, wave, lane, e);
                 tsB.S = e.S; tsB.inv = e.inv_S;
             }
@@ -679,8 +737,7 @@
             acc_zero(accB);
             {
                 ColBwdEpi<false> e(accA, imgA, hs, &hs.lmax[l - 1], tmax + (TMAX_CZBAR + l - 1) * ntiles + tileA, tpA + (PTP_COL_B0 + l - 1) * 256, wave,
-                                   lane, tid, tsA.inv * winv(l), tile_rsrc(cact + ((int64_t)(l - 1) * ntiles + tileA) * TILE_F),
-                                   tile_rsrc(czbar + ((int64_t)(l - 1) * ntiles + tileA) * TILE_F), loff, true);
+                                   lane, tid, tsA.inv * winv(l), signA(l - 1), tile_rsrc(czbar + ((int64_t)(l - 1) * ntiles + tileA) * TILE_F), loff, true);
                 pair_phase<true>(accB, imgB, W, rev(l), rev(l - 1), wave, lane, e);
                 tsA.S = e.S; tsA.inv = e.inv_S;
             }
@@ -689,22 +746,20 @@
         acc_zero(accA);
         {
             ColBwdEpi<false> e(accB, imgB, hs, &hs.lmax[0], tmax + TMAX_CZBAR * ntiles + tileB, tpB + PTP_COL_B0 * 256, wave, lane, tid,
-                               tsB.inv * wi1, tile_rsrc(cact + tileB * TILE_F), tile_rsrc_if(czbar + tileB * TILE_F, okB), loff, okB);
+                               tsB.inv * wi1, signB(0), tile_rsrc_if(czbar + tileB * TILE_F, okB), loff, okB);
             pair_phase<false>(accA, imgA, W, C.rev0, C.rev0, wave, lane, e);
             tsB.S = e.S; tsB.inv = e.inv_S;
         }
         pair_barrier();
         acc_zero(accB);
         {
-            ColBwdEpi<true> e(accA, imgA, hs, nullptr, nullptr, nullptr, wave, lane, tid, tsA.inv * wi0, tile_rsrc(featbar + tileA * TILE_F),
-                              tile_rsrc(featbar + tileA * TILE_F), loff, true);
+            ColBwdEpi<true> e(accA, hs, wave, lane, tid, tsA.inv * wi0, tile_rsrc(featbar + tileA * TILE_F), loff, true);
             pair_phase<false>(accB, imgB, W, C.rev0, C.rev0, wave, lane, e);
             if (lane == 0) sfb[0][wave] = hs.sred2[wave];
         }
         pair_barrier();
         {
-            ColBwdEpi<true> e(accB, imgB, hs, nullptr, nullptr, nullptr, wave, lane, tid, tsB.inv * wi0, tile_rsrc(featbar + tileB * TILE_F),
-                              tile_rsrc_if(featbar + tileB * TILE_F, okB), loff, okB);
+            ColBwdEpi<true> e(accB, hs, wave, lane, tid, tsB.inv * wi0, tile_rsrc_if(featbar + tileB * TILE_F, okB), loff, okB);
             pair_epi_alone_from<0>(e);
             if (lane == 0) sfb[1][wave] = hs.sred2[wave];
         }
@@ -764,16 +819,16 @@
 bool pair_form_available() { return pair_cus() > 0; }
 int pair_form_cus() { return pair_cus(); }
 int launch_color_fwd_p(const float* packed, const float* pts, const float* dirs, int n_per_ray, const float* normals,
-                       const float* feat, int64_t npts, float* color, float* cact, float* caux, int save, unsigned* absmax,
+                       const float* feat, int64_t npts, float* color, float* cact, float* caux, float* cmask, int save, unsigned* absmax,
                        hipStream_t stream) {
     const int cus = pair_cus();
     if (cus <= 0) return -2;
     const int64_t ntiles = (npts + TM - 1) / TM, npairs = (ntiles + 1) / 2;
     const int g = (int)(npairs < cus ? npairs : cus);
     if (save) hipLaunchKernelGGL(color_fwd_p_kernel<true>, dim3(g), dim3(256), 0, stream, make_colp_ptrs(packed), pts, dirs, n_per_ray, normals,
-                                 feat, npts, color, cact, caux, absmax);
+                                 feat, npts, color, cact, caux, cmask, absmax);
     else hipLaunchKernelGGL(color_fwd_p_kernel<false>, dim3(g), dim3(256), 0, stream, make_colp_ptrs(packed), pts, dirs, n_per_ray, normals,
-                            feat, npts, color, cact, caux, absmax);
+                            feat, npts, color, cact, caux, cmask, absmax);
     return okp();
 }
 
@@ -795,13 +850,13 @@
 }
 
 namespace dh {
-int launch_color_bwd_p(const float* packed, const float* colors, const float* d_colors, int64_t npts, const float* cact, float* czbar,
+int launch_color_bwd_p(const float* packed, const float* colors, const float* d_colors, int64_t npts, const float* cact, const float* cmask, float* czbar,
                        float* featbar, float* d_normals, float* tpart, unsigned* absmax, unsigned* tmax, hipStream_t stream) {
     const int cus = pair_cus();
     if (cus <= 0) return -2;
     const int64_t ntiles = (npts + TM - 1) / TM, npairs = (ntiles + 1) / 2;
     const int g = (int)(npairs < cus ? npairs : cus);
-    hipLaunchKernelGGL(color_bwd_p_kernel, dim3(g), dim3(256), 0, stream, make_colbwdp_ptrs(packed), colors, d_colors, npts, cact, czbar,
+    hipLaunchKernelGGL(color_bwd_p_kernel, dim3(g), dim3(256), 0, stream, make_colbwdp_ptrs(packed), colors, d_colors, npts, cact, cmask, czbar,
                        featbar, d_normals, tpart, absmax, tmax);
     return okp();
 }
diff --git a/dynhor_amd/csrc/kernels.h b/dynhor_amd/csrc/kernels.h
--- a/dynhor_amd/csrc/kernels.h
+++ b/dynhor_amd/csrc/kernels.h
@@ -26,15 +26,15 @@
 int launch_sdf_grad(const float* packed, const float* pts, int64_t npts, const float* act, float* asave, float* normals,
                     int save, float* gesave, float* absmax, int grid, int arith, hipStream_t stream);
 int launch_color_fwd(const float* packed, const float* pts, const float* dirs, int n_per_ray, const float* normals,
-                     const float* feat, int64_t npts, float* color, float* cact, float* caux, int save, float* absmax, int grid,
+                     const float* feat, int64_t npts, float* color, float* cact, float* caux, float* cmask, int save, float* absmax, int grid,
                      int arith, hipStream_t stream);
 int launch_sdf_grad_h(const float* packed, const float* pts, int64_t npts, const float* act, float* asave, float* normals,
                       int save, float* gesave, unsigned* absmax, int grid, hipStream_t stream);
 int launch_color_fwd_h(const float* packed, const float* pts, const float* dirs, int n_per_ray, const float* normals,
-                       const float* feat, int64_t npts, float* color, float* cact, float* caux, int save, unsigned* absmax,
+                       const float* feat, int64_t npts, float* color, float* cact, float* caux, float* cmask, int save, unsigned* absmax,
                        int grid, hipStream_t stream);
 int launch_color_bwd_h(const float* packed, const float* colors, const float* d_colors, const float* dirs, int n_per_ray,
-                       int64_t npts, const float* cact, float* czbar, float* featbar, float* d_normals, float* tpart,
+                       int64_t npts, const float* cact, const float* cmask, float* czbar, float* featbar, float* d_normals, float* tpart,
                        float* d_pts, float* d_dirs_pts, unsigned* absmax, unsigned* tmax, int grid, hipStream_t st);
 int launch_sdf_tangent_h(const float* packed, const float* pts, const float* d_normals, int64_t npts, const float* act,
                          const float* asave, float* t0aux, float* tsave, float* rsave, float* tpart, unsigned* absmax, unsigned* tmax,
@@ -53,13 +53,13 @@
     return cus > 0 && (npts + TM - 1) / TM >= 2 * (int64_t)cus;
 }
 int launch_color_fwd_p(const float* packed, const float* pts, const float* dirs, int n_per_ray, const float* normals,
-                       const float* feat, int64_t npts, float* color, float* cact, float* caux, int save, unsigned* absmax,
+                       const float* feat, int64_t npts, float* color, float* cact, float* caux, float* cmask, int save, unsigned* absmax,
                        hipStream_t stream);
 
 int launch_sdf_grad_p(const float* packed, const float* pts, int64_t npts, const float* act, float* asave, float* normals, int save,
                       float* gesave, unsigned* absmax, hipStream_t stream);
 
-int launch_color_bwd_p(const float* packed, const float* colors, const float* d_colors, int64_t npts, const float* cact, float* czbar,
+int launch_color_bwd_p(const float* packed, const float* colors, const float* d_colors, int64_t npts, const float* cact, const float* cmask, float* czbar,
                        float* featbar, float* d_normals, float* tpart, unsigned* absmax, unsigned* tmax, hipStream_t stream);
 
 int launch_gen_rays(const uint8_t* rgb, const int8_t* label, const uint8_t* normal, const float* R, const float* T,
@@ -97,10 +97,10 @@
                      float delta_px, float corr_w, float* stats, float* residual_px, float* d_weights, float* pose_adj,
                      hipStream_t st);
 
-int launch_color_bwd(const float* packed, const float* colors, const float* d_colors, int64_t npts, const float* cact,
+int launch_color_bwd(const float* packed, const float* colors, const float* d_colors, int64_t npts, const float* cact, const float* cmask,
                      float* czbar, float* featbar, float* d_normals, float* tpart, float* absmax, int grid, int arith, hipStream_t st);
 int launch_color_bwd_rays(const float* packed, const float* colors, const float* d_colors, const float* dirs, int n_per_ray,
-                          int64_t npts, const float* cact, float* czbar, float* featbar, float* d_normals, float* tpart,
+                          int64_t npts, const float* cact, const float* cmask, float* czbar, float* featbar, float* d_normals, float* tpart,
                           float* d_pts, float* d_dirs_pts, float* absmax, int grid, int arith, hipStream_t st);
 int launch_sdf_bwd_rays(const float* packed, const float* d_sdf, const float* pts, const float* d_normals, int64_t npts,
                         const float* act, const float* rsave, const float* featbar, const float* gesave, float* zbar,
diff --git a/dynhor_amd/csrc/kernels_mlp.hip b/dynhor_amd/csrc/kernels_mlp.hip
--- a/dynhor_amd/csrc/kernels_mlp.hip
+++ b/dynhor_amd/csrc/kernels_mlp.hip
@@ -140,7 +140,7 @@
 template <class Core>
 __device__ __forceinline__ void color_fwd_body(const typename Core::Col& C, const float* pts, const float* dirs, int n_per_ray,
                                                const float* normals, const float* feat, int64_t npts, float* color, float* cact,
-                                               float* caux, int save) {
+                                               float* caux, float* cmask, int save) {
     __shared__ __attribute__((aligned(16))) float smain[TM * LDX];
     __shared__ __attribute__((aligned(16))) float saux[TM * LDA];
     const int tid = threadIdx.x, wave = tid >> 6, lane = tid & 63;
@@ -181,6 +181,15 @@
             const float b0 = C.bias[l][acc_col(wave, 0, lane)], b1 = C.bias[l][acc_col(wave, 1, lane)];
             acc_map(acc, [&](int, int t, int, float v) { return fmaxf(v + (t ? b1 : b0), 0.f); });
             if (save) acc_store_native(acc, cact + ((int64_t)l * ntiles + tile) * TILE_F, wave, lane);
+#if DH_COL_MASK
+            if (save && l < CMASK_LAYERS) {
+                unsigned mw[MASK_DW];
+                acc_relu_mask(acc, mw);
+                mask_store_flat(cmask + ((int64_t)l * ntiles + tile) * CMASK_F, tid, mw);
+            }
+#else
+            (void)cmask;
+#endif
             __syncthreads();
             acc_to_lds(acc, smain, wave, lane);
             __syncthreads();
@@ -197,15 +206,15 @@
                                                             int n_per_ray, const float* __restrict__ normals,
                                                             const float* __restrict__ feat, int64_t npts,
                                                             float* __restrict__ color, float* __restrict__ cact,
-                                                            float* __restrict__ caux, int save) {
-    color_fwd_body<CoreF32>(C, pts, dirs, n_per_ray, normals, feat, npts, color, cact, caux, save);
+                                                            float* __restrict__ caux, float* __restrict__ cmask, int save) {
+    color_fwd_body<CoreF32>(C, pts, dirs, n_per_ray, normals, feat, npts, color, cact, caux, cmask, save);
 }
 __global__ __launch_bounds__(256, 2) void color_fwd_s_kernel(Col16Ptrs C, const float* __restrict__ pts, const float* __restrict__ dirs,
                                                             int n_per_ray, const float* __restrict__ normals,
                                                             const float* __restrict__ feat, int64_t npts,
                                                             float* __restrict__ color, float* __restrict__ cact,
-                                                            float* __restrict__ caux, int save) {
-    color_fwd_body<CoreBf16>(C, pts, dirs, n_per_ray, normals, feat, npts, color, cact, caux, save);
+                                                            float* __restrict__ caux, float* __restrict__ cmask, int save) {
+    color_fwd_body<CoreBf16>(C, pts, dirs, n_per_ray, normals, feat, npts, color, cact, caux, cmask, save);
 }
 
 int launch_sdf_fwd_train(const float* packed, const float* pts, int64_t npts, float* sdf, float* feat, float* act,
@@ -229,21 +238,21 @@
     return ok();
 }
 int launch_color_fwd(const float* packed, const float* pts, const float* dirs, int n_per_ray, const float* normals,
-                     const float* feat, int64_t npts, float* color, float* cact, float* caux, int save, float* absmax, int grid,
+                     const float* feat, int64_t npts, float* color, float* cact, float* caux, float* cmask, int save, float* absmax, int grid,
                      int arith, hipStream_t stream) {
     const int form = arith >> 8;
     arith &= 0xff;
     if (arith == ARITH_F16) {
-        if (use_pair_form(form, npts, true)) return launch_color_fwd_p(packed, pts, dirs, n_per_ray, normals, feat, npts, color, cact, caux, save,
+        if (use_pair_form(form, npts, true)) return launch_color_fwd_p(packed, pts, dirs, n_per_ray, normals, feat, npts, color, cact, caux, cmask, save,
                                                                  reinterpret_cast<unsigned*>(absmax), stream);
-        return launch_color_fwd_h(packed, pts, dirs, n_per_ray, normals, feat, npts, color, cact, caux, save,
+        return launch_color_fwd_h(packed, pts, dirs, n_per_ray, normals, feat, npts, color, cact, caux, cmask, save,
                                   reinterpret_cast<unsigned*>(absmax), grid, stream);
     }
     const int g = grid_for(npts, grid);
     if (arith == ARITH_FP32) hipLaunchKernelGGL(color_fwd_kernel, dim3(g), dim3(256), 0, stream, make_col_ptrs(packed), pts, dirs, n_per_ray, normals,
-                                                feat, npts, color, cact, caux, save);
+                                                feat, npts, color, cact, caux, cmask, save);
     else hipLaunchKernelGGL(color_fwd_s_kernel, dim3(g), dim3(256), 0, stream, make_col16_ptrs(packed), pts, dirs, n_per_ray, normals,
-                            feat, npts, color, cact, caux, save);
+                            feat, npts, color, cact, caux, cmask, save);
     return ok();
 }
 
diff --git a/dynhor_amd/csrc/kernels_mlp_bwd.hip b/dynhor_amd/csrc/kernels_mlp_bwd.hip
--- a/dynhor_amd/csrc/kernels_mlp_bwd.hip
+++ b/dynhor_amd/csrc/kernels_mlp_bwd.hip
@@ -13,7 +13,7 @@
 
 template <class Core, bool RAYS>
 __device__ __forceinline__ void color_bwd_body(const typename Core::Col& C, const float* colors, const float* d_colors, int64_t npts,
-                                               const float* cact, float* czbar, float* featbar, float* d_normals, float* tpart,
+                                               const float* cact, const float* cmask, float* czbar, float* featbar, float* d_normals, float* tpart,
                                                const float* dirs, int n_per_ray, float* d_pts, float* d_dirs_pts) {
     __shared__ __attribute__((aligned(16))) float smain[TM * LDX];
     __shared__ __attribute__((aligned(16))) float saux[TM * LDA];
@@ -69,6 +69,16 @@
             acc_zero(acc);
             Core::rows(acc, smain, LDX, Core::K_MAIN, C.rev_main[l], wave, lane, pre);
             pre = Core::prefetch(C.rev_main[l - 1], wave, lane);
+#if DH_COL_MASK
+            {
+                unsigned mw[MASK_DW];
+                mask_load_flat(mw, cmask + ((int64_t)(l - 1) * ntiles + tile) * CMASK_F, tid);
+                DH_UNROLL for (int m = 0; m < MT; ++m)
+                    DH_UNROLL for (int t = 0; t < 2; ++t)
+                        DH_UNROLL for (int r = 0; r < 16; ++r) acc[m][t][r] = relu_mask_keep(mw, m, t, r, acc[m][t][r]);
+            }
+#else
+            (void)cmask;
             const f32x4* hp = reinterpret_cast<const f32x4*>(cact + ((int64_t)(l - 1) * ntiles + tile) * TILE_F) + (size_t)wave * MT * 8 * 64 + lane;
             DH_UNROLL for (int m = 0; m < MT; ++m) {
                 DH_UNROLL for (int t = 0; t < 2; ++t)
@@ -79,6 +89,7 @@
                     }
                 __builtin_amdgcn_sched_barrier(0);
             }
+#endif
             acc_store_native(acc, czbar + ((int64_t)(l - 1) * ntiles + tile) * TILE_F, wave, lane);
             tile_colsum(acc, tp + (TP_COL_B0 + l - 1) * 256, wave, lane);
             __syncthreads();
@@ -115,22 +126,24 @@
 template <bool RAYS>
 __global__ __launch_bounds__(256, 2) void color_bwd_kernel(ColPtrs C, const float* __restrict__ colors,
                                                             const float* __restrict__ d_colors, int64_t npts,
-                                                            const float* __restrict__ cact, float* __restrict__ czbar,
+                                                            const float* __restrict__ cact, const float* __restrict__ cmask,
+                                                            float* __restrict__ czbar,
                                                             float* __restrict__ featbar, float* __restrict__ d_normals,
                                                             float* __restrict__ tpart, const float* __restrict__ dirs,
                                                             int n_per_ray, float* __restrict__ d_pts,
                                                             float* __restrict__ d_dirs_pts) {
-    color_bwd_body<CoreF32, RAYS>(C, colors, d_colors, npts, cact, czbar, featbar, d_normals, tpart, dirs, n_per_ray, d_pts, d_dirs_pts);
+    color_bwd_body<CoreF32, RAYS>(C, colors, d_colors, npts, cact, cmask, czbar, featbar, d_normals, tpart, dirs, n_per_ray, d_pts, d_dirs_pts);
 }
 template <bool RAYS>
 __global__ __launch_bounds__(256, 2) void color_bwd_s_kernel(Col16Ptrs C, const float* __restrict__ colors,
                                                             const float* __restrict__ d_colors, int64_t npts,
-                                                            const float* __restrict__ cact, float* __restrict__ czbar,
+                                                            const float* __restrict__ cact, const float* __restrict__ cmask,
+                                                            float* __restrict__ czbar,
                                                             float* __restrict__ featbar, float* __restrict__ d_normals,
                                                             float* __restrict__ tpart, const float* __restrict__ dirs,
                                                             int n_per_ray, float* __restrict__ d_pts,
                                                             float* __restrict__ d_dirs_pts) {
-    color_bwd_body<CoreBf16, RAYS>(C, colors, d_colors, npts, cact, czbar, featbar, d_normals, tpart, dirs, n_per_ray, d_pts, d_dirs_pts);
+    color_bwd_body<CoreBf16, RAYS>(C, colors, d_colors, npts, cact, cmask, czbar, featbar, d_normals, tpart, dirs, n_per_ray, d_pts, d_dirs_pts);
 }
 
 
@@ -338,32 +351,32 @@
     sdf_bwd_body<CoreBf16, RAYS>(P, d_sdf, npts, act, rsave, featbar, zbar, tpart, pts, d_normals, gesave, d_pts);
 }
 
-int launch_color_bwd(const float* packed, const float* colors, const float* d_colors, int64_t npts, const float* cact,
+int launch_color_bwd(const float* packed, const float* colors, const float* d_colors, int64_t npts, const float* cact, const float* cmask,
                      float* czbar, float* featbar, float* d_normals, float* tpart, float* absmax, int grid, int arith, hipStream_t st) {
     const int form = arith >> 8;
     arith &= 0xff;
     if (arith == ARITH_F16) {
         unsigned* am = reinterpret_cast<unsigned*>(absmax);
-        if (use_pair_form(form, npts, false)) return launch_color_bwd_p(packed, colors, d_colors, npts, cact, czbar, featbar, d_normals, tpart, am,
+        if (use_pair_form(form, npts, false)) return launch_color_bwd_p(packed, colors, d_colors, npts, cact, cmask, czbar, featbar, d_normals, tpart, am,
                                                                  am + ABSMAX_FLOATS, st);
-        return launch_color_bwd_h(packed, colors, d_colors, nullptr, 1, npts, cact, czbar, featbar, d_normals, tpart, nullptr, nullptr, am,
+        return launch_color_bwd_h(packed, colors, d_colors, nullptr, 1, npts, cact, cmask, czbar, featbar, d_normals, tpart, nullptr, nullptr, am,
                                   am + ABSMAX_FLOATS, grid, st);
     }
     if (arith == ARITH_FP32) hipLaunchKernelGGL(color_bwd_kernel<false>, dim3(grid_for(npts, grid)), dim3(256), 0, st, make_col_ptrs(packed), colors,
-                                                d_colors, npts, cact, czbar, featbar, d_normals, tpart, nullptr, 1, nullptr, nullptr);
+                                                d_colors, npts, cact, cmask, czbar, featbar, d_normals, tpart, nullptr, 1, nullptr, nullptr);
     else hipLaunchKernelGGL(color_bwd_s_kernel<false>, dim3(grid_for(npts, grid)), dim3(256), 0, st, make_col16_ptrs(packed), colors,
-                            d_colors, npts, cact, czbar, featbar, d_normals, tpart, nullptr, 1, nullptr, nullptr);
+                            d_colors, npts, cact, cmask, czbar, featbar, d_normals, tpart, nullptr, 1, nullptr, nullptr);
     return ok();
 }
 int launch_color_bwd_rays(const float* packed, const float* colors, const float* d_colors, const float* dirs, int n_per_ray,
-                          int64_t npts, const float* cact, float* czbar, float* featbar, float* d_normals, float* tpart,
+                          int64_t npts, const float* cact, const float* cmask, float* czbar, float* featbar, float* d_normals, float* tpart,
                           float* d_pts, float* d_dirs_pts, float* absmax, int grid, int arith, hipStream_t st) {
-    if (arith == ARITH_F16) return launch_color_bwd_h(packed, colors, d_colors, dirs, n_per_ray, npts, cact, czbar, featbar, d_normals, tpart, d_pts,
+    if (arith == ARITH_F16) return launch_color_bwd_h(packed, colors, d_colors, dirs, n_per_ray, npts, cact, cmask, czbar, featbar, d_normals, tpart, d_pts,
                                                      d_dirs_pts, reinterpret_cast<unsigned*>(absmax), reinterpret_cast<unsigned*>(absmax) + ABSMAX_FLOATS, grid, st);
     if (arith == ARITH_FP32) hipLaunchKernelGGL(color_bwd_kernel<true>, dim3(grid_for(npts, grid)), dim3(256), 0, st, make_col_ptrs(packed), colors,
-                                                d_colors, npts, cact, czbar, featbar, d_normals, tpart, dirs, n_per_ray, d_pts, d_dirs_pts);
+                                                d_colors, npts, cact, cmask, czbar, featbar, d_normals, tpart, dirs, n_per_ray, d_pts, d_dirs_pts);
     else hipLaunchKernelGGL(color_bwd_s_kernel<true>, dim3(grid_for(npts, grid)), dim3(256), 0, st, make_col16_ptrs(packed), colors,
-                            d_colors, npts, cact, czbar, featbar, d_normals, tpart, dirs, n_per_ray, d_pts, d_dirs_pts);
+                            d_colors, npts, cact, cmask, czbar, featbar, d_normals, tpart, dirs, n_per_ray, d_pts, d_dirs_pts);
     return ok();
 }
 int launch_sdf_tangent(const float* packed, const float* pts, const float* d_normals, int64_t npts, const float* act,
diff --git a/dynhor_amd/csrc/kernels_mlp_h.hip b/dynhor_amd/csrc/kernels_mlp_h.hip
--- a/dynhor_amd/csrc/kernels_mlp_h.hip
+++ b/dynhor_amd/csrc/kernels_mlp_h.hip
@@ -131,13 +131,15 @@
                                                             int n_per_ray, const float* __restrict__ normals,
                                                             const float* __restrict__ feat, int64_t npts,
                                                             float* __restrict__ color, float* __restrict__ cact,
-                                                            float* __restrict__ caux, int save, unsigned* __restrict__ absmax) {
+                                                            float* __restrict__ caux, float* __restrict__ cmask, int save,
+                                                            unsigned* __restrict__ absmax) {
     __shared__ __attribute__((aligned(16))) _Float16 smain[IMG_H];
     __shared__ __attribute__((aligned(16))) float saux[TM * LDA];
     __shared__ HScratch hs;
     const int tid = threadIdx.x, wave = tid >> 6, lane = tid & 63;
     const int loff = tile_loff(wave, lane);
     const int64_t ntiles = (npts + TM - 1) / TM;
+    (void)cmask;
     hs_init(hs, tid);
     float winv[4];
     DH_UNROLL for (int l = 0; l < 4; ++l) winv[l] = winv_from_bits(C.wabs[l]);
@@ -198,6 +200,13 @@
             const float b0 = C.bias[l][acc_col(wave, 0, lane)], b1 = C.bias[l][acc_col(wave, 1, lane)];
             acc_map(acc, [&](int, int t, int, float v) { return fmaxf(fmaf(v, inv, t ? b1 : b0), 0.f); });
             if (save) acc_store_native_b(acc, tile_rsrc(cact + ((int64_t)l * ntiles + tile) * TILE_F), loff);
+#if DH_COL_MASK
+            if (save && l < CMASK_LAYERS) {
+                unsigned mw[MASK_DW];
+                acc_relu_mask(acc, mw);
+                mask_st(mask_rsrc(cmask, l, ntiles, tile), tid, mw);
+            }
+#endif
             DH_STAMP(it, l, 2);
             ts = lds_handoff(acc, smain, hs, save ? &hs.lmax[l] : nullptr, tid, wave, lane, 0.f, nullptr, nullptr, it, l);
         }
@@ -321,7 +330,8 @@
 template <bool RAYS>
 __global__ __launch_bounds__(256, 2) void color_bwd_h_kernel(ColHPtrs C, const float* __restrict__ colors,
                                                             const float* __restrict__ d_colors, int64_t npts,
-                                                            const float* __restrict__ cact, float* __restrict__ czbar,
+                                                            const float* __restrict__ cact, const float* __restrict__ cmask,
+                                                            float* __restrict__ czbar,
                                                             float* __restrict__ featbar, float* __restrict__ d_normals,
                                                             float* __restrict__ tpart, const float* __restrict__ dirs,
                                                             int n_per_ray, float* __restrict__ d_pts,
@@ -333,6 +343,7 @@
     const int tid = threadIdx.x, wave = tid >> 6, lane = tid & 63;
     const int loff = tile_loff(wave, lane);
     const int64_t ntiles = (npts + TM - 1) / TM;
+    (void)cmask;
     hs_init(hs, tid);
     for (int64_t tile = blockIdx.x; tile < ntiles; tile += gridDim.x) {
         float* tp = tpart + tile * N_TILE_PART * 256;
@@ -358,9 +369,10 @@
             float w4[3][2];
             DH_UNROLL for (int j = 0; j < 3; ++j) { w4[j][0] = C.w4[j * 256 + col0]; w4[j][1] = C.w4[j * 256 + col1]; }
             float dw[3][2] = {{0.f, 0.f}, {0.f, 0.f}, {0.f, 0.f}};
+            const int crow = opaque_vgpr(4 * (lane >> 5));
             DH_UNROLL for (int m = 0; m < MT; ++m)
                 DH_UNROLL for (int r = 0; r < 16; ++r) {
-                    const f32x4 cr = *reinterpret_cast<const f32x4*>(saux + acc_row(m, r, lane) * 4);
+                    const f32x4 cr = *reinterpret_cast<const f32x4*>(saux + (crow + acc_row(m, r, 0)) * 4);
                     DH_UNROLL for (int t = 0; t < 2; ++t) {
                         const float h = acc[m][t][r];
                         DH_UNROLL for (int j = 0; j < 3; ++j) dw[j][t] = fmaf(cr[j], h, dw[j][t]);
@@ -380,6 +392,17 @@
         TileScale ts = lds_handoff(acc, smain, hs, &hs.lmax[3], tid, wave, lane, 0.f, nullptr, tmax + (TMAX_CZBAR + 3) * ntiles + tile);
         for (int l = 3; l >= 1; --l) {
             acc_zero(acc);
+#if DH_COL_MASK
+            const rsrc_t mr = mask_rsrc(cmask, l - 1, ntiles, tile);
+            unsigned mw[MASK_DW];
+            gemm_rows_hp<false>(acc, smain, 16, C.rev[l], wave, lane, [&] { mask_ld(mw, mr, tid); });
+            const float inv = ts.inv * winv_from_bits(C.wabs[l]);
+            DH_UNROLL for (int m = 0; m < MT; ++m) {
+                DH_UNROLL for (int t = 0; t < 2; ++t)
+                    DH_UNROLL for (int r = 0; r < 16; ++r) acc[m][t][r] = relu_mask_keep(mw, m, t, r, acc[m][t][r] * inv);
+                __builtin_amdgcn_sched_barrier(0);
+            }
+#else
             const rsrc_t hr = tile_rsrc(cact + ((int64_t)(l - 1) * ntiles + tile) * TILE_F);
             Slab h0, h1;
             gemm_rows_hp<false>(acc, smain, 16, C.rev[l], wave, lane, [&] { slab_ld(h0, hr, loff, 0); });
@@ -395,6 +418,7 @@
                     }
                 __builtin_amdgcn_sched_barrier(0);
             }
+#endif
             acc_store_native_b(acc, tile_rsrc(czbar + ((int64_t)(l - 1) * ntiles + tile) * TILE_F), loff);
             tile_colsum(acc, tp + (TP_COL_B0 + l - 1) * 256, wave, lane);
             ts = lds_handoff(acc, smain, hs, &hs.lmax[l - 1], tid, wave, lane, 0.f, nullptr, tmax + (TMAX_CZBAR + l - 1) * ntiles + tile);
@@ -412,9 +436,12 @@
         DH_UNROLL for (int tt = 0; tt < AUX_NTW; ++tt) {
             const int col = aux_col(wave, tt, lane);
             if (col >= 30 && col < 33) {
+                const int row0 = opaque_vgpr(aux_row(wave, 0, lane));
+                float* dn = d_normals + (tile * TM + row0) * 3 + (col - 30);
+                const int64_t left = npts - tile * TM - row0;
                 DH_UNROLL for (int r = 0; r < 16; ++r) {
-                    const int64_t gp = tile * TM + aux_row(wave, r, lane);
-                    if (gp < npts) d_normals[gp * 3 + (col - 30)] += a2[tt][r];
+                    const int dr = aux_row(0, r, 0);
+                    if (dr < left) dn[dr * 3] += a2[tt][r];
                 }
             }
         }
@@ -423,7 +450,8 @@
             DH_UNROLL for (int tt = 0; tt < AUX_NTW; ++tt) {
                 const int col = aux_col(wave, tt, lane);
                 if (col < CAUX) {
-                    DH_UNROLL for (int r = 0; r < 16; ++r) saux[aux_row(wave, r, lane) * LDA + col] = a2[tt][r];
+                    float* dst = saux + opaque_vgpr(aux_row(wave, 0, lane)) * LDA + col;
+                    DH_UNROLL for (int r = 0; r < 16; ++r) dst[aux_row(0, r, 0) * LDA] = a2[tt][r];
                 }
             }
             __syncthreads();
@@ -684,19 +712,19 @@
     return ok();
 }
 int launch_color_fwd_h(const float* packed, const float* pts, const float* dirs, int n_per_ray, const float* normals,
-                       const float* feat, int64_t npts, float* color, float* cact, float* caux, int save, unsigned* absmax,
+                       const float* feat, int64_t npts, float* color, float* cact, float* caux, float* cmask, int save, unsigned* absmax,
                        int grid, hipStream_t stream) {
     hipLaunchKernelGGL(color_fwd_h_kernel, dim3(grid_for(npts, grid)), dim3(256), 0, stream, make_colh_ptrs(packed), pts, dirs,
-                       n_per_ray, normals, feat, npts, color, cact, caux, save, absmax);
+                       n_per_ray, normals, feat, npts, color, cact, caux, cmask, save, absmax);
     return ok();
 }
 int launch_color_bwd_h(const float* packed, const float* colors, const float* d_colors, const float* dirs, int n_per_ray,
-                       int64_t npts, const float* cact, float* czbar, float* featbar, float* d_normals, float* tpart,
+                       int64_t npts, const float* cact, const float* cmask, float* czbar, float* featbar, float* d_normals, float* tpart,
                        float* d_pts, float* d_dirs_pts, unsigned* absmax, unsigned* tmax, int grid, hipStream_t st) {
     if (d_pts) hipLaunchKernelGGL(color_bwd_h_kernel<true>, dim3(grid_for(npts, grid)), dim3(256), 0, st, make_colh_ptrs(packed), colors,
-                                  d_colors, npts, cact, czbar, featbar, d_normals, tpart, dirs, n_per_ray, d_pts, d_dirs_pts, absmax, tmax);
+                                  d_colors, npts, cact, cmask, czbar, featbar, d_normals, tpart, dirs, n_per_ray, d_pts, d_dirs_pts, absmax, tmax);
     else hipLaunchKernelGGL(color_bwd_h_kernel<false>, dim3(grid_for(npts, grid)), dim3(256), 0, st, make_colh_ptrs(packed), colors,
-                            d_colors, npts, cact, czbar, featbar, d_normals, tpart, nullptr, 1, nullptr, nullptr, absmax, tmax);
+                            d_colors, npts, cact, cmask, czbar, featbar, d_normals, tpart, nullptr, 1, nullptr, nullptr, absmax, tmax);
     return ok();
 }
 int launch_sdf_tangent_h(const float* packed, const float* pts, const float* d_normals, int64_t npts, const float* act,
diff --git a/dynhor_amd/csrc/tile.h b/dynhor_amd/csrc/tile.h
--- a/dynhor_amd/csrc/tile.h
+++ b/dynhor_amd/csrc/tile.h
@@ -88,8 +88,33 @@
 __device__ __forceinline__ int aux_row(int wave, int r, int lane) { return 32 * aux_mtile(wave) + (r & 3) + 8 * (r >> 2) + 4 * (lane >> 5); }
 __device__ __forceinline__ int aux_col(int wave, int tt, int lane) { return 32 * aux_ntile(wave, tt) + (lane & 31); }
 
+__device__ __forceinline__ int opaque_vgpr(int v) { asm volatile("" : "+v"(v)); return v; }
 __device__ __forceinline__ int acc_row(int m, int r, int lane) { return m * 32 + (r & 3) + 8 * (r >> 2) + 4 * (lane >> 5); }
 __device__ __forceinline__ int acc_col(int wave, int t, int lane) { return 64 * wave + 32 * t + (lane & 31); }
+
+constexpr int MASK_DW = 2 * MT;
+__host__ __device__ constexpr int relu_mask_dword(int m, int t) { return m * 2 + t; }
+__host__ __device__ constexpr int relu_mask_bit(int m, int t, int r) { return relu_mask_dword(m, t) * 32 + r; }
+static_assert(MT == 2 && MASK_DW == 4, "four dwords hold a lane's share of a 64-point tile");
+#ifdef __FAST_MATH__
+#error "tile.h relu_mask_shift_in needs signed zeros: do not build this library with -ffast-math"
+#endif
+__device__ __forceinline__ unsigned relu_mask_shift_in(unsigned w, float v) {
+    return __builtin_amdgcn_alignbit(w, __builtin_bit_cast(unsigned, 0.f - fmaxf(v, 0.f)), 31);
+}
+__device__ __forceinline__ void acc_relu_mask(const f32x16 (&acc)[MT][2], unsigned (&w)[MASK_DW]) {
+    DH_UNROLL for (int m = 0; m < MT; ++m)
+        DH_UNROLL for (int t = 0; t < 2; ++t) {
+            unsigned x = 0u;
+            DH_UNROLL for (int r = 15; r >= 0; --r) x = relu_mask_shift_in(x, acc[m][t][r]);
+            w[relu_mask_dword(m, t)] = x;
+        }
+}
+__device__ __forceinline__ float relu_mask_keep(const unsigned (&w)[MASK_DW], int m, int t, int r, float v) {
+    int keep;
+    asm("v_bfe_i32 %0, %1, %2, 1" : "=v"(keep) : "v"(w[relu_mask_dword(m, t)]), "n"(relu_mask_bit(m, t, r) & 31));
+    return __builtin_bit_cast(float, __builtin_bit_cast(int, v) & keep);
+}
 
 __device__ __forceinline__ void acc_to_lds(const f32x16 (&acc)[MT][2], float* xs, int wave, int lane) {
     DH_UNROLL for (int m = 0; m < MT; ++m)
@@ -123,6 +148,17 @@
             }
 }
 
+typedef unsigned mask_u32x4 __attribute__((ext_vector_type(4)));
+__device__ __forceinline__ void mask_store_flat(float* __restrict__ masks, int tid, const unsigned (&w)[MASK_DW]) {
+    mask_u32x4 v;
+    v[0] = w[0]; v[1] = w[1]; v[2] = w[2]; v[3] = w[3];
+    DH_TILE_ST(reinterpret_cast<mask_u32x4*>(masks) + tid, v);
+}
+__device__ __forceinline__ void mask_load_flat(unsigned (&w)[MASK_DW], const float* __restrict__ masks, int tid) {
+    const mask_u32x4 v = DH_TILE_LD(reinterpret_cast<const mask_u32x4*>(masks) + tid);
+    w[0] = v[0]; w[1] = v[1]; w[2] = v[2]; w[3] = v[3];
+}
+
 __device__ __forceinline__ void aux_store_native(const f32x16 (&a2)[AUX_NTW], float* __restrict__ tile, int wave, int lane) {
     f32x4* p = reinterpret_cast<f32x4*>(tile) + lane;
     DH_UNROLL for (int tt = 0; tt < AUX_NTW; ++tt)
diff --git a/dynhor_amd/csrc/tile16h.h b/dynhor_amd/csrc/tile16h.h
--- a/dynhor_amd/csrc/tile16h.h
+++ b/dynhor_amd/csrc/tile16h.h
@@ -183,6 +183,18 @@
                 acc[m][t][4 * r4 + 0] = v[0]; acc[m][t][4 * r4 + 1] = v[1]; acc[m][t][4 * r4 + 2] = v[2]; acc[m][t][4 * r4 + 3] = v[3];
             }
 }
+__device__ __forceinline__ rsrc_t mask_rsrc(const float* cmask, int64_t layer, int64_t ntiles, int64_t tile, bool on = true) {
+    return __builtin_amdgcn_make_buffer_rsrc(const_cast<float*>(cmask + (layer * ntiles + tile) * CMASK_F), 0, on ? CMASK_F * 4 : 0, 0x00020000);
+}
+__device__ __forceinline__ void mask_st(rsrc_t r, int tid, const unsigned (&w)[MASK_DW]) {
+    u32x4 v;
+    v[0] = w[0]; v[1] = w[1]; v[2] = w[2]; v[3] = w[3];
+    __builtin_amdgcn_raw_buffer_store_b128(v, r, tid * 16, 0, 2);
+}
+__device__ __forceinline__ void mask_ld(unsigned (&w)[MASK_DW], rsrc_t r, int tid) {
+    const u32x4 v = __builtin_amdgcn_raw_buffer_load_b128(r, tid * 16, 0, 2);
+    w[0] = v[0]; w[1] = v[1]; w[2] = v[2]; w[3] = v[3];
+}
 struct Slab { f32x4 v[8]; };
 __device__ __forceinline__ void slab_ld(Slab& s, rsrc_t r, int loff, int m) {
     DH_UNROLL for (int i = 0; i < 8; ++i) s.v[i] = tile_ld(r, loff, m * 8 + i);
diff --git a/dynhor_amd/csrc/workspace.h b/dynhor_amd/csrc/workspace.h
--- a/dynhor_amd/csrc/workspace.h
+++ b/dynhor_amd/csrc/workspace.h
@@ -2,6 +2,12 @@
 #include "layout.h"
 
 namespace dh {
+
+#ifndef DH_COL_MASK
+#define DH_COL_MASK 1
+#endif
+constexpr int CMASK_LAYERS = 3;
+constexpr int CMASK_F = 256 * 4;
 
 constexpr int N_TILE_PART = 20;
 constexpr int DW_G = 256;
@@ -26,6 +32,7 @@
     float* asave;
     float* cact;
     float* caux;
+    float* cmask;
     float* featbar;
     float* tsave;
     float* t0aux;
@@ -55,6 +62,7 @@
     w.asave = take(8 * nt * TILE_F);
     w.cact = take(4 * nt * TILE_F);
     w.caux = take(nt * AUXT_F);
+    w.cmask = take(CMASK_LAYERS * nt * CMASK_F);
     w.fwd_floats = o;
     w.featbar = take(nt * TILE_F);
     w.tsave = take(7 * nt * TILE_F);
diff --git a/include/dynhor_hip.h b/include/dynhor_hip.h
--- a/include/dynhor_hip.h
+++ b/include/dynhor_hip.h
@@ -33,6 +33,9 @@
 int dh_sdf_nograd(const float* packed, const float* pts, int64_t npts, float* sdf, void* stream);
 
 int dh_workspace_floats(int64_t npts, int64_t* infer_floats, int64_t* fwd_floats, int64_t* total_floats);
+
+enum { DH_WS_CACT = 0, DH_WS_CMASK = 1, DH_WS_CZBAR = 2, DH_WS_FEATBAR = 3, DH_WS_TPART = 4 };
+int dh_workspace_region(int64_t npts, int region, int64_t* offset_floats, int64_t* n_floats);
 
 int dh_range_words(int64_t* act_max_off, int64_t* tag_off, float* limit);
 
```

After: 236,100 rays/s (median of 6 runs). About the same (+2.3%).
